# eblerjana/pangenie

Hardware: AMD Instinct MI355X
Metric: genotyped variants/sec (whole node) at H haplotypes; HBM GB/s vs roofline (higher is better)
Workload: dtype f64

## Files before the change

### include/pangenie_hmm.h

```cpp
#ifndef PANGENIE_HMM_H
#define PANGENIE_HMM_H

#include <stddef.h>
#include <stdint.h>

#ifdef __cplusplus
extern "C" {
#endif

#define PG_OK 0
#define PG_ERR_INVALID (-1)
#define PG_ERR_NO_PATHS (-2)
#define PG_ERR_UNSUPPORTED (-3)
#define PG_ERR_DEVICE (-4)
#define PG_ERR_NOMEM (-5)

typedef struct pg_contig_batch {
    uint32_t n_variants;
    uint32_t n_paths;
    const uint64_t* variant_pos;
    const uint16_t* coverage;
    const uint32_t* kmer_off;
    const uint16_t* kmer_count;
    const uint32_t* allele_off;
    const uint16_t* allele_id;
    const uint8_t*  allele_flags;
    const uint16_t* allele_kmer_off;
    const uint32_t* allele_kmer_mask;
    const uint16_t* path_allele;
} pg_contig_batch;

typedef struct pg_hmm_params {
    long double effective_N;
    double recombrate;
    int32_t uniform;
    int32_t run_genotyping;
    int32_t run_phasing;
    int32_t reserved;
} pg_hmm_params;
#define PG_CALL_ANNOUNCED 1

typedef struct pg_contig_result {
    double*   lik;
    int32_t*  lik_exp;
    uint8_t*  kept;
    uint8_t*  allele_present;
    uint16_t* n_kmers;
    uint16_t* coverage;
    uint32_t  n_columns;
    uint32_t  reserved;
    uint16_t* haplotype_1;
    uint16_t* haplotype_2;
} pg_contig_result;

int pg_hmm_geno_offsets(const pg_contig_batch* batch, uint64_t* geno_off);

typedef struct pg_table pg_table;
pg_table* pg_table_create(uint16_t cov_min, uint16_t cov_max, uint16_t count_max,
                          long double regularization);
pg_table* pg_table_create_default(void);
int  pg_table_modify(pg_table* t, uint16_t coverage, uint16_t count,
                     long double p0, long double p1, long double p2);
int  pg_table_get(const pg_table* t, uint16_t coverage, uint16_t count,
                  long double out3[3]);
void pg_table_destroy(pg_table* t);

int pg_hmm_device_count(void);
const char* pg_hmm_version(void);
int pg_hmm_genotype_contig(const pg_contig_batch* batch, const pg_table* table,
                           const pg_hmm_params* params, int device,
                           pg_contig_result* out, char* err, size_t errlen);
void pg_hmm_announce(int device);
void pg_hmm_retract(int device);
int  pg_hmm_coalesce_stats(uint64_t out3[3]);

typedef struct pg_job pg_job;
pg_job* pg_job_create(int device, uint32_t n_contigs, const pg_contig_batch* batches,
                      const pg_table* table, const pg_hmm_params* params,
                      char* err, size_t errlen);
int  pg_job_run(pg_job* job, void* stream, char* err, size_t errlen);
int  pg_job_fetch(pg_job* job, uint32_t contig, pg_contig_result* out, char* err, size_t errlen);
int  pg_job_fetch_all(pg_job* job, pg_contig_result* outs, char* err, size_t errlen);
int  pg_job_device_results(pg_job* job, uint32_t contig, void** d_lik, uint64_t* n_lik,
                           void** d_lik_exp, uint64_t* n_variants);
#define PG_N_KERNEL_CLASSES 6
int  pg_job_kernel_ms(const pg_job* job, double ms[PG_N_KERNEL_CLASSES]);
const char* pg_job_kernel_name(int cls);
int  pg_job_profile_counters(pg_job* job, uint32_t contig, uint64_t out64[64]);
uint64_t pg_job_device_bytes(const pg_job* job);
int  pg_job_sweep_mode(const pg_job* job, uint32_t* chunk_cols);
uint32_t pg_job_triangle_chains(const pg_job* job);
double pg_job_index_ms(const pg_job* job);
size_t pg_job_plan(const pg_job* job, char* out, size_t len);
int pg_sparse_segment(uint32_t n_columns, uint32_t chunk_cols, uint32_t chunk, uint32_t role, uint32_t j, uint32_t out[3]);
int pg_sparse_stored_by_chain(uint32_t n_columns, uint32_t role, uint32_t column);
int pg_sparse_chunk_segment(uint32_t n_columns, uint32_t chunk_cols, uint32_t chunk, uint32_t role, uint32_t j, uint32_t out[3]);
int pg_sparse_chunk_stored_by_chain(uint32_t n_columns, uint32_t role, uint32_t column);
int pg_sparse_piece_range(uint32_t n_columns, uint32_t chunk_cols, uint32_t piece_chunks, uint32_t piece, uint32_t role, uint32_t out[2]);
int pg_prep_parts(uint32_t n_columns, uint32_t chunk_cols, uint32_t piece_chunks, uint32_t n_pieces, uint32_t early,
                  const uint32_t* col_variant, uint32_t n_variants, uint32_t out_cols[2], uint32_t out_vars[2]);
uint32_t pg_prep_part_member(uint32_t part, uint32_t lo, uint32_t hi, uint32_t n, uint32_t u);
double pg_job_viterbi_ms(const pg_job* job);
void pg_job_destroy(pg_job* job);

int  pg_job_panel_sizes(const pg_job* job, uint32_t contig, uint32_t* n_variants, uint32_t* n_paths,
                        uint64_t* sum_kmers, uint64_t* sum_alleles);
int  pg_job_fetch_panel(pg_job* job, uint32_t contig, uint32_t* kmer_off, uint16_t* kmer_count,
                        uint32_t* allele_off, uint16_t* allele_id, uint8_t* allele_flags,
                        uint16_t* allele_kmer_off, uint32_t* allele_kmer_mask, uint16_t* path_allele,
                        char* err, size_t errlen);

int  pg_job_new(int device, uint32_t n_contigs, const pg_contig_batch* batches,
                const pg_table* table, const pg_hmm_params* params,
                pg_job** out, char* err, size_t errlen);
uint32_t pg_job_n_chains(const pg_job* job);

typedef struct pg_sample_counts {
    const uint16_t* const* kmer_count;
    const uint16_t* const* coverage;
} pg_sample_counts;
int  pg_cohort_new(int device, uint32_t n_contigs, const pg_contig_batch* index,
                   uint32_t n_samples, const pg_sample_counts* samples,
                   const pg_table* table, const pg_hmm_params* params,
                   pg_job** out, char* err, size_t errlen);

int  pg_job_upload(pg_job* job, const pg_contig_batch* batches, const pg_sample_counts* samples,
                   char* err, size_t errlen);
int  pg_job_upload_run(pg_job* job, const pg_contig_batch* batches, const pg_sample_counts* samples, char* err, size_t errlen);
int  pg_job_upload_begin(pg_job* job, const pg_sample_counts* samples, char* err, size_t errlen);
int  pg_job_upload_end(pg_job* job, char* err, size_t errlen);
int  pg_job_host_seconds(const pg_job* job, double out4[4]);
int  pg_job_upload_bytes(const pg_job* job, uint64_t out2[2]);
int  pg_job_packed_results(pg_job* job, void** d_lik, void** d_lik_exp, uint64_t* n_lik_total);
void pg_hmm_release_cache(void);

typedef struct pg_comm pg_comm;
int  pg_comm_unique_id(uint8_t id128[128], char* err, size_t errlen);
int  pg_comm_init(const uint8_t id128[128], int world, int rank, int device,
                  pg_comm** out, char* err, size_t errlen);
int  pg_comm_init_all(int n_devices, const int* devices, pg_comm** out_comms, char* err, size_t errlen);
int  pg_comm_rank(const pg_comm* comm);
int  pg_comm_world(const pg_comm* comm);
void pg_comm_destroy(pg_comm* comm);
int  pg_hmm_gather(pg_comm* comm, pg_job* job, int root, const uint64_t* n_lik_per_rank,
                   void* d_lik_all, void* d_exp_all, char* err, size_t errlen);
int  pg_hmm_gather_all(int n_local, pg_comm* const* comms, pg_job* const* jobs, int root,
                       const uint64_t* n_lik_per_rank, void* d_lik_all, void* d_exp_all,
                       char* err, size_t errlen);
int  pg_hmm_gather_to_host(int n_local, pg_comm* const* comms, pg_job* const* jobs, int root,
                           const uint64_t* n_lik_per_rank, double* h_lik_all, int32_t* h_exp_all,
                           char* err, size_t errlen);

int pg_emission_table(const pg_contig_batch* batch, const pg_table* table, uint32_t v,
                      int device, long double* out_AxA, int32_t* all_zeros,
                      char* err, size_t errlen);
int pg_transition_probs(uint64_t from_pos, uint64_t to_pos, double recombrate,
                        uint32_t nr_paths, int uniform, long double effective_N,
                        int device, double out3[3], char* err, size_t errlen);

typedef struct pg_call {
    uint16_t allele_1, allele_2;
    uint16_t gq;
    uint16_t flags;
} pg_call;
#define PG_CALL_OK 0
#define PG_CALL_NONE 1
#define PG_CALL_NOT_UNIQUE 2
#define PG_CALL_DEFERRED 3
int  pg_job_calls(pg_job* job, char* err, size_t errlen);
int  pg_job_fetch_calls(pg_job* job, uint32_t chain, pg_call* out, char* err, size_t errlen);
int  pg_job_fetch_calls_all(pg_job* job, pg_call* const* outs, char* err, size_t errlen);
int  pg_job_device_calls(pg_job* job, uint32_t chain, void** d_calls, uint64_t* n);
double pg_job_calls_ms(const pg_job* job);
int  pg_calls_from_bins(int device, uint32_t n_variants, const uint32_t* allele_off, const uint16_t* allele_id,
                        const uint8_t* kept, const uint8_t* allele_present, const double* lik,
                        const int32_t* lik_exp, pg_call* out);

typedef struct pg_record_plan {
    uint32_t n_variants;
    uint32_t n_records;
    const uint32_t* rec_off;
    const uint32_t* map_off;
    const uint16_t* map;
    const uint16_t* n_alleles;
    const uint32_t* vcf_off;
    const uint16_t* vcf_index;
} pg_record_plan;
#define PG_CALL_EMPTY 0x100
int  pg_job_record_plan(pg_job* job, uint32_t index_contig, const pg_record_plan* plan, char* err, size_t errlen);
int  pg_job_record_plan_strided(pg_job* job, uint32_t contig, uint32_t n_contigs, const pg_record_plan* plan, char* err, size_t errlen);
int  pg_job_record_calls(pg_job* job, char* err, size_t errlen);
int  pg_job_fetch_record_calls(pg_job* job, uint32_t chain, pg_call* out, char* err, size_t errlen);
int  pg_job_fetch_record_calls_all(pg_job* job, pg_call* const* outs, char* err, size_t errlen);
int  pg_job_device_record_calls(pg_job* job, uint32_t chain, void** d_calls, uint64_t* n);
double pg_job_record_calls_ms(const pg_job* job);
int  pg_record_calls_from_bins(int device, uint32_t n_variants, const uint32_t* allele_off, const uint16_t* allele_id,
                               const uint8_t* kept, const uint8_t* allele_present, const double* lik,
                               const int32_t* lik_exp, const pg_record_plan* plan, pg_call* out);

#ifndef PG_GL_DEFINED
#define PG_GL_DEFINED
typedef struct pg_gl { int16_t mant; int16_t exp10; } pg_gl;
#define PG_GL_NEG_INF  (-32768)
#define PG_GL_DEFERRED (-32767)
#endif
int  pg_record_gl_offsets(const pg_record_plan* plan, uint64_t* gl_off);
int  pg_job_record_gl(pg_job* job, char* err, size_t errlen);
int  pg_job_fetch_record_gl(pg_job* job, uint32_t chain, pg_gl* out, char* err, size_t errlen);
int  pg_job_fetch_record_gl_all(pg_job* job, pg_gl* const* outs, char* err, size_t errlen);
int  pg_job_device_record_gl(pg_job* job, uint32_t chain, void** d_gl, uint64_t* n);
double pg_job_record_gl_ms(const pg_job* job);
int  pg_job_record_first(pg_job* job, uint64_t* calls_first, uint64_t* gl_first, char* err, size_t errlen);
int  pg_job_fetch_record_calls_packed(pg_job* job, pg_call* out, uint64_t n, char* err, size_t errlen);
int  pg_job_fetch_record_gl_packed(pg_job* job, pg_gl* out, uint64_t n, char* err, size_t errlen);
int  pg_record_gl_from_bins(int device, uint32_t n_variants, const uint32_t* allele_off, const uint16_t* allele_id,
                            const uint8_t* kept, const uint8_t* allele_present, const double* lik,
                            const int32_t* lik_exp, const pg_record_plan* plan, pg_gl* out);
int  pg_gl_from_values(int device, uint64_t n, const uint64_t* m, const int32_t* e, pg_gl* out);
int  pg_gl_text(pg_gl value, char* buf, size_t len);

#ifdef __cplusplus
}
#endif
#endif
```

### pangenie_amd/_lib.py

```python
from __future__ import annotations

import ctypes as C

import numpy as np
import os
from pathlib import Path

ROOT = Path(__file__).resolve().parent.parent
HIP_LIB_PATH = ROOT / "pangenie_amd" / "csrc" / "libpangenie_hmm.so"

PG_OK = 0
PG_ERR_INVALID = -1
PG_ERR_NO_PATHS = -2
PG_ERR_UNSUPPORTED = -3
PG_ERR_DEVICE = -4
PG_ERR_NOMEM = -5
PG_N_KERNEL_CLASSES = 6

u8p = C.POINTER(C.c_uint8)
u16p = C.POINTER(C.c_uint16)
u32p = C.POINTER(C.c_uint32)
u64p = C.POINTER(C.c_uint64)
i32p = C.POINTER(C.c_int32)
f64p = C.POINTER(C.c_double)
ldp = C.POINTER(C.c_longdouble)


def c_ld(x) -> C.c_longdouble:
    v = np.longdouble(x) if isinstance(x, str) else x
    return C.c_longdouble.from_buffer_copy(np.array([v], dtype=np.longdouble).tobytes())


def ld_out(n: int):
    a = np.zeros(n, dtype=np.longdouble)
    return a, a.ctypes.data_as(ldp)


class PgContigBatch(C.Structure):
    _fields_ = [
        ("n_variants", C.c_uint32),
        ("n_paths", C.c_uint32),
        ("variant_pos", u64p),
        ("coverage", u16p),
        ("kmer_off", u32p),
        ("kmer_count", u16p),
        ("allele_off", u32p),
        ("allele_id", u16p),
        ("allele_flags", u8p),
        ("allele_kmer_off", u16p),
        ("allele_kmer_mask", u32p),
        ("path_allele", u16p),
    ]


class PgHmmParams(C.Structure):
    _fields_ = [
        ("effective_N", C.c_longdouble),
        ("recombrate", C.c_double),
        ("uniform", C.c_int32),
        ("run_genotyping", C.c_int32),
        ("run_phasing", C.c_int32),
        ("reserved", C.c_int32),
    ]


class PgContigResult(C.Structure):
    _fields_ = [
        ("lik", f64p),
        ("lik_exp", i32p),
        ("kept", u8p),
        ("allele_present", u8p),
        ("n_kmers", u16p),
        ("coverage", u16p),
        ("n_columns", C.c_uint32),
        ("reserved", C.c_uint32),
        ("haplotype_1", u16p),
        ("haplotype_2", u16p),
    ]


class PgSampleCounts(C.Structure):
    _fields_ = [
        ("kmer_count", C.POINTER(u16p)),
        ("coverage", C.POINTER(u16p)),
    ]


class PgGl(C.Structure):
    _fields_ = [("mant", C.c_int16), ("exp10", C.c_int16)]


PG_CALL_ANNOUNCED = 1


class HipExtensionMissing(RuntimeError):
    pass


_hip = None


def _bind_hip(lib):
    ld = C.c_longdouble
    lib.pg_hmm_geno_offsets.argtypes = [C.POINTER(PgContigBatch), u64p]
    lib.pg_hmm_geno_offsets.restype = C.c_int
    lib.pg_table_create.argtypes = [C.c_uint16, C.c_uint16, C.c_uint16, ld]
    lib.pg_table_create.restype = C.c_void_p
    lib.pg_table_create_default.argtypes = []
    lib.pg_table_create_default.restype = C.c_void_p
    lib.pg_table_modify.argtypes = [C.c_void_p, C.c_uint16, C.c_uint16, ld, ld, ld]
    lib.pg_table_modify.restype = C.c_int
    lib.pg_table_get.argtypes = [C.c_void_p, C.c_uint16, C.c_uint16, ldp]
    lib.pg_table_get.restype = C.c_int
    lib.pg_table_destroy.argtypes = [C.c_void_p]
    lib.pg_table_destroy.restype = None
    lib.pg_hmm_device_count.argtypes = []
    lib.pg_hmm_device_count.restype = C.c_int
    lib.pg_hmm_version.argtypes = []
    lib.pg_hmm_version.restype = C.c_char_p
    lib.pg_hmm_genotype_contig.argtypes = [
        C.POINTER(PgContigBatch), C.c_void_p, C.POINTER(PgHmmParams), C.c_int,
        C.POINTER(PgContigResult), C.c_char_p, C.c_size_t]
    lib.pg_hmm_genotype_contig.restype = C.c_int
    lib.pg_job_create.argtypes = [
        C.c_int, C.c_uint32, C.POINTER(PgContigBatch), C.c_void_p,
        C.POINTER(PgHmmParams), C.c_char_p, C.c_size_t]
    lib.pg_job_create.restype = C.c_void_p
    lib.pg_job_run.argtypes = [C.c_void_p, C.c_void_p, C.c_char_p, C.c_size_t]
    lib.pg_job_run.restype = C.c_int
    lib.pg_job_fetch.argtypes = [C.c_void_p, C.c_uint32, C.POINTER(PgContigResult),
                                 C.c_char_p, C.c_size_t]
    lib.pg_job_fetch.restype = C.c_int
    lib.pg_job_device_results.argtypes = [C.c_void_p, C.c_uint32, C.POINTER(C.c_void_p),
                                          u64p, C.POINTER(C.c_void_p), u64p]
    lib.pg_job_device_results.restype = C.c_int
    lib.pg_job_index_ms.argtypes = [C.c_void_p]
    lib.pg_job_index_ms.restype = C.c_double
    lib.pg_job_plan.argtypes = [C.c_void_p, C.c_char_p, C.c_size_t]
    lib.pg_job_plan.restype = C.c_size_t
    lib.pg_sparse_segment.argtypes = [C.c_uint32, C.c_uint32, C.c_uint32, C.c_uint32, C.c_uint32, u32p]
    lib.pg_sparse_segment.restype = C.c_int
    lib.pg_sparse_stored_by_chain.argtypes = [C.c_uint32, C.c_uint32, C.c_uint32]
    lib.pg_sparse_stored_by_chain.restype = C.c_int
    lib.pg_sparse_chunk_segment.argtypes = [C.c_uint32, C.c_uint32, C.c_uint32, C.c_uint32, C.c_uint32, u32p]
    lib.pg_sparse_chunk_segment.restype = C.c_int
    lib.pg_sparse_chunk_stored_by_chain.argtypes = [C.c_uint32, C.c_uint32, C.c_uint32]
    lib.pg_sparse_chunk_stored_by_chain.restype = C.c_int
    lib.pg_sparse_piece_range.argtypes = [C.c_uint32, C.c_uint32, C.c_uint32, C.c_uint32, C.c_uint32, u32p]
    lib.pg_sparse_piece_range.restype = C.c_int
    lib.pg_prep_parts.argtypes = [C.c_uint32, C.c_uint32, C.c_uint32, C.c_uint32, C.c_uint32, u32p, C.c_uint32, u32p, u32p]
    lib.pg_prep_parts.restype = C.c_int
    lib.pg_prep_part_member.argtypes = [C.c_uint32] * 5
    lib.pg_prep_part_member.restype = C.c_uint32
    lib.pg_job_kernel_ms.argtypes = [C.c_void_p, f64p]
    lib.pg_job_kernel_ms.restype = C.c_int
    lib.pg_job_kernel_name.argtypes = [C.c_int]
    lib.pg_job_kernel_name.restype = C.c_char_p
    lib.pg_job_profile_counters.argtypes = [C.c_void_p, C.c_uint32, u64p]
    lib.pg_job_profile_counters.restype = C.c_int
    lib.pg_job_viterbi_ms.argtypes = [C.c_void_p]
    lib.pg_job_viterbi_ms.restype = C.c_double
    lib.pg_job_device_bytes.argtypes = [C.c_void_p]
    lib.pg_job_device_bytes.restype = C.c_uint64
    lib.pg_job_sweep_mode.argtypes = [C.c_void_p, C.POINTER(C.c_uint32)]
    lib.pg_job_sweep_mode.restype = C.c_int
    lib.pg_job_triangle_chains.argtypes = [C.c_void_p]
    lib.pg_job_triangle_chains.restype = C.c_uint32
    lib.pg_job_destroy.argtypes = [C.c_void_p]
    lib.pg_job_destroy.restype = None
    lib.pg_job_new.argtypes = [C.c_int, C.c_uint32, C.POINTER(PgContigBatch), C.c_void_p, C.POINTER(PgHmmParams),
                               C.POINTER(C.c_void_p), C.c_char_p, C.c_size_t]
    lib.pg_job_new.restype = C.c_int
    lib.pg_cohort_new.argtypes = [C.c_int, C.c_uint32, C.POINTER(PgContigBatch), C.c_uint32, C.POINTER(PgSampleCounts),
                                  C.c_void_p, C.POINTER(PgHmmParams), C.POINTER(C.c_void_p), C.c_char_p, C.c_size_t]
    lib.pg_cohort_new.restype = C.c_int
    lib.pg_job_n_chains.argtypes = [C.c_void_p]
    lib.pg_job_n_chains.restype = C.c_uint32
    lib.pg_job_upload.argtypes = [C.c_void_p, C.POINTER(PgContigBatch), C.POINTER(PgSampleCounts), C.c_char_p, C.c_size_t]
    lib.pg_job_upload.restype = C.c_int
    lib.pg_job_upload_run.argtypes = [C.c_void_p, C.POINTER(PgContigBatch), C.POINTER(PgSampleCounts), C.c_char_p, C.c_size_t]
    lib.pg_job_upload_run.restype = C.c_int
    lib.pg_job_upload_begin.argtypes = [C.c_void_p, C.POINTER(PgSampleCounts), C.c_char_p, C.c_size_t]
    lib.pg_job_upload_begin.restype = C.c_int
    lib.pg_job_upload_end.argtypes = [C.c_void_p, C.c_char_p, C.c_size_t]
    lib.pg_job_upload_end.restype = C.c_int
    lib.pg_job_host_seconds.argtypes = [C.c_void_p, f64p]
    lib.pg_job_host_seconds.restype = C.c_int
    lib.pg_job_upload_bytes.argtypes = [C.c_void_p, u64p]
    lib.pg_job_upload_bytes.restype = C.c_int
    lib.pg_job_packed_results.argtypes = [C.c_void_p, C.POINTER(C.c_void_p), C.POINTER(C.c_void_p), u64p]
    lib.pg_job_packed_results.restype = C.c_int
    lib.pg_hmm_release_cache.argtypes = []
    lib.pg_hmm_release_cache.restype = None
    lib.pg_comm_unique_id.argtypes = [u8p, C.c_char_p, C.c_size_t]
    lib.pg_comm_unique_id.restype = C.c_int
    lib.pg_comm_init.argtypes = [u8p, C.c_int, C.c_int, C.c_int, C.POINTER(C.c_void_p), C.c_char_p, C.c_size_t]
    lib.pg_comm_init.restype = C.c_int
    lib.pg_comm_init_all.argtypes = [C.c_int, C.POINTER(C.c_int), C.POINTER(C.c_void_p), C.c_char_p, C.c_size_t]
    lib.pg_comm_init_all.restype = C.c_int
    lib.pg_comm_rank.argtypes = [C.c_void_p]
    lib.pg_comm_rank.restype = C.c_int
    lib.pg_comm_world.argtypes = [C.c_void_p]
    lib.pg_comm_world.restype = C.c_int
    lib.pg_comm_destroy.argtypes = [C.c_void_p]
    lib.pg_comm_destroy.restype = None
    lib.pg_hmm_gather.argtypes = [C.c_void_p, C.c_void_p, C.c_int, u64p, C.c_void_p, C.c_void_p, C.c_char_p, C.c_size_t]
    lib.pg_hmm_gather.restype = C.c_int
    lib.pg_hmm_gather_all.argtypes = [C.c_int, C.POINTER(C.c_void_p), C.POINTER(C.c_void_p), C.c_int, u64p, C.c_void_p, C.c_void_p,
                                      C.c_char_p, C.c_size_t]
    lib.pg_hmm_gather_all.restype = C.c_int
    lib.pg_emission_table.argtypes = [C.POINTER(PgContigBatch), C.c_void_p, C.c_uint32, C.c_int,
                                      ldp, i32p, C.c_char_p, C.c_size_t]
    lib.pg_emission_table.restype = C.c_int
    lib.pg_transition_probs.argtypes = [C.c_uint64, C.c_uint64, C.c_double, C.c_uint32, C.c_int,
                                        ld, C.c_int, f64p, C.c_char_p, C.c_size_t]
    lib.pg_transition_probs.restype = C.c_int
    lib.pg_job_fetch_all.argtypes = [C.c_void_p, C.POINTER(PgContigResult), C.c_char_p, C.c_size_t]
    lib.pg_job_fetch_all.restype = C.c_int
    lib.pg_job_panel_sizes.argtypes = [C.c_void_p, C.c_uint32, C.POINTER(C.c_uint32), C.POINTER(C.c_uint32), u64p, u64p]
    lib.pg_job_panel_sizes.restype = C.c_int
    lib.pg_job_fetch_panel.argtypes = [C.c_void_p, C.c_uint32, u32p, u16p, u32p, u16p, u8p, u16p, u32p, u16p, C.c_char_p, C.c_size_t]
    lib.pg_job_fetch_panel.restype = C.c_int
    lib.pg_hmm_announce.argtypes = [C.c_int]
    lib.pg_hmm_announce.restype = None
    lib.pg_hmm_retract.argtypes = [C.c_int]
    lib.pg_hmm_retract.restype = None
    lib.pg_hmm_coalesce_stats.argtypes = [u64p]
    lib.pg_hmm_coalesce_stats.restype = C.c_int
    lib.pg_job_calls.argtypes = [C.c_void_p, C.c_char_p, C.c_size_t]
    lib.pg_job_calls.restype = C.c_int
    lib.pg_job_fetch_calls.argtypes = [C.c_void_p, C.c_uint32, C.c_void_p, C.c_char_p, C.c_size_t]
    lib.pg_job_fetch_calls.restype = C.c_int
    lib.pg_job_fetch_calls_all.argtypes = [C.c_void_p, C.POINTER(C.c_void_p), C.c_char_p, C.c_size_t]
    lib.pg_job_fetch_calls_all.restype = C.c_int
    lib.pg_job_device_calls.argtypes = [C.c_void_p, C.c_uint32, C.POINTER(C.c_void_p), u64p]
    lib.pg_job_device_calls.restype = C.c_int
    lib.pg_job_calls_ms.argtypes = [C.c_void_p]
    lib.pg_job_calls_ms.restype = C.c_double
    lib.pg_calls_from_bins.argtypes = [C.c_int, C.c_uint32, u32p, u16p, u8p, u8p, f64p, i32p, C.c_void_p]
    lib.pg_calls_from_bins.restype = C.c_int
    lib.pg_job_record_plan.argtypes = [C.c_void_p, C.c_uint32, C.c_void_p, C.c_char_p, C.c_size_t]
    lib.pg_job_record_plan.restype = C.c_int
    lib.pg_job_record_calls.argtypes = [C.c_void_p, C.c_char_p, C.c_size_t]
    lib.pg_job_record_calls.restype = C.c_int
    lib.pg_job_fetch_record_calls.argtypes = [C.c_void_p, C.c_uint32, C.c_void_p, C.c_char_p, C.c_size_t]
    lib.pg_job_fetch_record_calls.restype = C.c_int
    lib.pg_job_fetch_record_calls_all.argtypes = [C.c_void_p, C.POINTER(C.c_void_p), C.c_char_p, C.c_size_t]
    lib.pg_job_fetch_record_calls_all.restype = C.c_int
    lib.pg_job_device_record_calls.argtypes = [C.c_void_p, C.c_uint32, C.POINTER(C.c_void_p), u64p]
    lib.pg_job_device_record_calls.restype = C.c_int
    lib.pg_job_record_calls_ms.argtypes = [C.c_void_p]
    lib.pg_job_record_calls_ms.restype = C.c_double
    lib.pg_record_calls_from_bins.argtypes = [C.c_int, C.c_uint32, u32p, u16p, u8p, u8p, f64p, i32p, C.c_void_p, C.c_void_p]
    lib.pg_record_calls_from_bins.restype = C.c_int
    lib.pg_record_gl_offsets.argtypes = [C.c_void_p, u64p]
    lib.pg_record_gl_offsets.restype = C.c_int
    lib.pg_job_record_gl.argtypes = [C.c_void_p, C.c_char_p, C.c_size_t]
    lib.pg_job_record_gl.restype = C.c_int
    lib.pg_job_fetch_record_gl.argtypes = [C.c_void_p, C.c_uint32, C.c_void_p, C.c_char_p, C.c_size_t]
    lib.pg_job_fetch_record_gl.restype = C.c_int
    lib.pg_job_fetch_record_gl_all.argtypes = [C.c_void_p, C.POINTER(C.c_void_p), C.c_char_p, C.c_size_t]
    lib.pg_job_fetch_record_gl_all.restype = C.c_int
    lib.pg_job_device_record_gl.argtypes = [C.c_void_p, C.c_uint32, C.POINTER(C.c_void_p), u64p]
    lib.pg_job_device_record_gl.restype = C.c_int
    lib.pg_job_record_gl_ms.argtypes = [C.c_void_p]
    lib.pg_job_record_gl_ms.restype = C.c_double
    lib.pg_record_gl_from_bins.argtypes = [C.c_int, C.c_uint32, u32p, u16p, u8p, u8p, f64p, i32p, C.c_void_p, C.c_void_p]
    lib.pg_record_gl_from_bins.restype = C.c_int
    lib.pg_job_record_plan_strided.argtypes = [C.c_void_p, C.c_uint32, C.c_uint32, C.c_void_p, C.c_char_p, C.c_size_t]
    lib.pg_job_record_plan_strided.restype = C.c_int
    lib.pg_job_record_first.argtypes = [C.c_void_p, u64p, u64p, C.c_char_p, C.c_size_t]
    lib.pg_job_record_first.restype = C.c_int
    lib.pg_job_fetch_record_calls_packed.argtypes = [C.c_void_p, C.c_void_p, C.c_uint64, C.c_char_p, C.c_size_t]
    lib.pg_job_fetch_record_calls_packed.restype = C.c_int
    lib.pg_job_fetch_record_gl_packed.argtypes = [C.c_void_p, C.c_void_p, C.c_uint64, C.c_char_p, C.c_size_t]
    lib.pg_job_fetch_record_gl_packed.restype = C.c_int
    lib.pg_gl_from_values.argtypes = [C.c_int, C.c_uint64, u64p, i32p, C.c_void_p]
    lib.pg_gl_from_values.restype = C.c_int
    lib.pg_gl_text.argtypes = [PgGl, C.c_char_p, C.c_size_t]
    lib.pg_gl_text.restype = C.c_int
    return lib


HIP_ABI_SYMBOLS = [
    "pg_hmm_geno_offsets", "pg_table_create", "pg_table_create_default", "pg_table_modify",
    "pg_table_get", "pg_table_destroy", "pg_hmm_device_count", "pg_hmm_version",
    "pg_hmm_genotype_contig", "pg_job_create", "pg_job_run", "pg_job_fetch",
    "pg_job_device_results", "pg_job_profile_counters", "pg_job_kernel_ms", "pg_job_index_ms", "pg_job_plan", "pg_job_kernel_name", "pg_job_device_bytes", "pg_job_sweep_mode",
    "pg_job_destroy", "pg_emission_table", "pg_transition_probs",
    "pg_job_new", "pg_cohort_new", "pg_job_n_chains", "pg_job_upload", "pg_job_upload_run", "pg_job_upload_begin", "pg_job_upload_end", "pg_job_host_seconds", "pg_job_upload_bytes",
    "pg_job_packed_results", "pg_hmm_release_cache", "pg_job_triangle_chains", "pg_job_viterbi_ms",
    "pg_comm_unique_id", "pg_comm_init", "pg_comm_init_all", "pg_comm_rank", "pg_comm_world", "pg_comm_destroy",
    "pg_hmm_gather", "pg_hmm_gather_all", "pg_hmm_gather_to_host",
    "pg_hmm_announce", "pg_hmm_retract", "pg_hmm_coalesce_stats", "pg_job_fetch_all", "pg_job_panel_sizes", "pg_job_fetch_panel",
    "pg_job_calls", "pg_job_fetch_calls", "pg_job_fetch_calls_all", "pg_job_device_calls", "pg_job_calls_ms", "pg_calls_from_bins",
    "pg_job_record_plan", "pg_job_record_calls", "pg_job_fetch_record_calls", "pg_job_fetch_record_calls_all", "pg_job_device_record_calls",
    "pg_job_record_calls_ms", "pg_record_calls_from_bins",
    "pg_record_gl_offsets", "pg_job_record_gl", "pg_job_fetch_record_gl", "pg_job_fetch_record_gl_all", "pg_job_device_record_gl",
    "pg_job_record_gl_ms", "pg_record_gl_from_bins", "pg_gl_from_values", "pg_gl_text",
    "pg_job_record_plan_strided", "pg_job_record_first", "pg_job_fetch_record_calls_packed", "pg_job_fetch_record_gl_packed",
    "pg_sparse_segment", "pg_sparse_stored_by_chain", "pg_sparse_chunk_segment", "pg_sparse_chunk_stored_by_chain", "pg_sparse_piece_range",
    "pg_prep_parts", "pg_prep_part_member",
]


def load_hip():
    global _hip
    if _hip is None:
        path = Path(os.environ.get("PANGENIE_HMM_LIB", HIP_LIB_PATH))
        if not path.exists():
            raise HipExtensionMissing(
                f"{path} is missing: run `python -c 'import __graft_entry__ as g; g.build()'` "
                "(hipcc --offload-arch=gfx950). There is no CPU fallback.")
        _hip = _bind_hip(C.CDLL(str(path), mode=os.RTLD_GLOBAL if hasattr(os, "RTLD_GLOBAL") else 0))
    return _hip
```

### pangenie_amd/csrc/pg_device.h

```cpp
#pragma once
#include <stddef.h>
#include <stdint.h>

#define PG_AMAX 5
#define PG_ESTRIDE (PG_AMAX + 1)
#define PG_ETAB (PG_ESTRIDE * PG_ESTRIDE)
#define PG_MAX_ALLELES_PER_VARIANT 256
#define PG_MAX_PATHS 1024
#define PG_PHANTOM 255

#define PG_REC_C0 0
#define PG_REC_C1 8
#define PG_REC_C2 16
#define PG_REC_KAPPA 24
#define PG_REC_VARIANT 32
#define PG_REC_EXP 36
#define PG_REC_NLOCAL 40
#define PG_REC_FLAGS 41
#define PG_REC_LOCAL_SLOT 48
#define PG_REC_BITS1 64
#define PG_REC_E 80
#define PG_REC_ALLELES (80 + 8 * PG_ETAB)
#define PG_REC_FLAG_ALLZERO 1
#define PG_REC_FLAG_WIDE 2
#define PG_REC_WIDE_IDX 44
#define PG_REC_AUX 60

#define PG_WIDE_MAX 254
#define PG_WIDE_NONE 0xFFFFFFFFu
static inline uint64_t pg_wide_entry_bytes(uint32_t n_local) {
    const uint64_t s = (uint64_t)n_local + 1;
    return (s * s * 20 + (uint64_t)n_local * 2 + 15) & ~(uint64_t)15;
}
#define PG_WIDE_OFF_PM(S) ((size_t)(S) * (S) * 8)
#define PG_WIDE_OFF_PE(S) ((size_t)(S) * (S) * 16)
#define PG_WIDE_OFF_SLOT(S) ((size_t)(S) * (S) * 20)

#ifndef PG_SCRATCH_BUFS
#define PG_SCRATCH_BUFS 3u
#endif
#define PG_SCR_BUF(c) ((c) % PG_SCRATCH_BUFS)
#define PG_SYNC_NEXT 16u
#define PG_SYNC_DONE 17u
#define PG_SYNC_READY 32u
#define PG_SYNC_WORDS 48u

#define PG_BIAS_F 400
#define PG_BIAS_B 400

static inline uint32_t pg_pair_count(uint32_t pair_n) { return ((pair_n * (pair_n + 1) / 2) + 1u) & ~1u; }
static inline uint32_t pg_pair_bytes(uint32_t pair_n) { return pg_pair_count(pair_n) * 12u; }

static inline uint32_t pg_rec_bytes(uint32_t hp) { return (PG_REC_ALLELES + hp + 63u) & ~63u; }

#define PG_DEVERR_ALLELE_NOT_FOUND 1u
#define PG_DEVERR_TOO_MANY_ALLELES 2u
#define PG_DEVERR_TOO_MANY_LOCAL 4u
#define PG_DEVERR_SYNC_TIMEOUT 16u
#define PG_DEVERR_WIDE_FUSED 8u

struct DevTable {
    uint32_t cov_min, cov_max, count_max;
    uint32_t pad;
    double reg;
    const double* mant;
    const int32_t* expo;
    const unsigned char* packed;
};

#define PG_IXPD_BYTES 32u
#define PG_IXREC_BYTES 64u
#define PG_IXBIN_BYTES 32u
#define PG_SREC1_BYTES 64u
#define PG_SREC2_BYTES 128u
#define PG_CPREC_BYTES 192u
#define PG_COL_NONE 0xFFFFFFFFu
#define PG_IXPD_U0 0x100u
#define PG_IXPD_U1 0x200u
#define PG_IXPD_HAS0 0x400u
#define PG_IXPD_HAS1 0x800u
#define PG_SREC_FLAG_ALLZERO 1u
#define PG_SREC_FLAG_WIDE 2u
#define PG_SREC_FLAG_PRECISE 4u
struct IxBin {
    uint32_t g0, v, aux;
    uint16_t A;
    uint8_t nl, flags;
    uint16_t ls[5];
    uint8_t cnt[5];
    uint8_t pad;
};

struct DevContig {
    uint32_t V, H, HP, RB;
    uint32_t T;
    uint32_t pad0;
    double dist_scale;
    int32_t uniform;
    uint32_t debug;
    uint32_t part_slots;
    uint32_t pair_n;
    const uint64_t* pos;
    const uint16_t* cov;
    const uint32_t* kmer_off;
    const uint16_t* kmer_count;
    const uint32_t* allele_off;
    const uint16_t* allele_id;
    const uint8_t*  allele_flags;
    const uint16_t* allele_koff;
    const uint32_t* allele_kmask;
    const uint16_t* path_allele;
    const uint64_t* geno_off;
    uint8_t*  vrec;
    uint8_t*  kept;
    uint8_t*  allele_present;
    uint32_t* n_cols;
    uint32_t* col_variant;
    uint8_t*  colrec;
    double*   fwd;
    double*   part;
    double*   fscale;
    double*   bscale;
    double*   bsum;
    uint8_t*  fwd_fallback;
    double*   scratch;
    uint32_t* sync;
    uint32_t  chunk_cols;
    uint32_t  col_stride;
    uint8_t*  wide;
    const uint32_t* wide_idx;
    uint8_t*  vpair;
    double*   frec;
    uint32_t  prep_fast;
    uint32_t  n_prep_m4, n_prep_w;
    uint32_t  n_prep_b;
    const uint32_t* prep_m4;
    const uint32_t* prep_w;
    const uint32_t* prep_b;
    uint32_t  lean;
    uint32_t  tri;
    uint32_t  leanx2;
    uint32_t  widef;
    uint32_t  small;
    uint32_t  leanx;
    uint32_t  cls4;
    uint32_t  smallx;
    uint32_t  split;
    const uint32_t* col_of;
    const unsigned char* ix_pd;
    const unsigned char* ix_rec;
    const unsigned char* ix_bin;
    unsigned char* cprec;
    uint32_t* ix_err;
    const uint32_t* ix_big;
    uint32_t n_ix_big;
    uint32_t sparse;
    uint32_t sparse2;
    uint32_t ckpt_slots;
    double*  ckpt;
    uint32_t* wcols;
    uint32_t* n_wcols;
    unsigned char* aux;
    const uint32_t* aux_idx;
    uint32_t  live;
    double*   xbuf;
    uint32_t* err;
    unsigned long long* prof;
    double*   vit_tq;
    uint16_t* vit_back;
    uint32_t* vit_best;
    uint16_t* hap1;
    uint16_t* hap2;
    double*   lik;
    int32_t*  lik_exp;
};

#define PG_LEAN_SPARSE 64u
#ifdef __HIP__
#define PG_HD __attribute__((host)) __attribute__((device))
#else
#define PG_HD
#endif
PG_HD inline uint32_t pg_sparse_segments(uint32_t C, uint32_t role) {
    const uint32_t mid = C / 2u;
    if (role == 0u) return mid ? (mid - 1u) / PG_LEAN_SPARSE : 0u;
    return C ? (C - 1u - mid) / PG_LEAN_SPARSE : 0u;
}
PG_HD inline uint32_t pg_sparse_checkpoint(uint32_t C, uint32_t role, uint32_t m) {
    const uint32_t mid = C / 2u;
    return role == 0u ? mid - 1u - m * PG_LEAN_SPARSE : mid + m * PG_LEAN_SPARSE;
}
PG_HD inline bool pg_sparse_stored(uint32_t C, uint32_t role, uint32_t c) {
    const uint32_t mid = C / 2u;
    if (role == 0u) return c >= mid || (mid - 1u - c) % PG_LEAN_SPARSE == 0u || c < (mid - 1u) % PG_LEAN_SPARSE;
    return c < mid || (c - mid) % PG_LEAN_SPARSE == 0u || c > mid + pg_sparse_segments(C, 1u) * PG_LEAN_SPARSE;
}
#define PG_PIECE_CHUNKS_DEFAULT 4u
PG_HD inline bool pg_sparse_piece(uint32_t C, uint32_t role, uint32_t piece_cols, uint32_t g, uint32_t out[2]) {
    const unsigned long long mid = C / 2u, half = role == 0u ? mid : C - mid;
    const unsigned long long d0 = (unsigned long long)g * piece_cols;
    if (piece_cols == 0u || piece_cols % PG_LEAN_SPARSE != 0u || d0 >= half) return false;
    const unsigned long long d1 = half - d0 > piece_cols ? d0 + piece_cols : half;
    if (role == 0u) { out[0] = (uint32_t)(mid - d1); out[1] = (uint32_t)(mid - 1u - d0); }
    else { out[0] = (uint32_t)(mid + d0); out[1] = (uint32_t)(mid + d1 - 1u); }
    return true;
}
#define PG_PREP_EARLY_PIECES_DEFAULT 2u
PG_HD inline uint32_t pg_prep_band(uint32_t n_pieces, uint32_t E, uint32_t piece_cols) {
    const unsigned long long W = (unsigned long long)(n_pieces - E) * piece_cols;
    return W > 0xFFFFFFC0ull ? 0xFFFFFFC0u : (uint32_t)W;
}
PG_HD inline void pg_prep_middle(uint32_t C, uint32_t W, uint32_t out[2]) {
    const uint32_t mid = C / 2u;
    out[0] = mid - (mid < W ? mid : W);
    out[1] = mid + (C - mid < W ? C - mid : W);
}
PG_HD inline void pg_prep_middle_variants(const uint32_t* col_variant, uint32_t C, uint32_t V, uint32_t W, uint32_t out[2]) {
    uint32_t cr[2];
    pg_prep_middle(C, W, cr);
    out[0] = cr[0] == 0u ? 0u : col_variant[cr[0]];
    out[1] = cr[1] >= C ? V : col_variant[cr[1]];
}
PG_HD inline uint32_t pg_prep_part_item(uint32_t part, uint32_t lo, uint32_t hi, uint32_t N, uint32_t u) {
    if (part == 2u) return u < hi - lo ? lo + u : N;
    return u < lo ? u : (u < N - (hi - lo) ? u + (hi - lo) : N);
}

PG_HD inline uint32_t pg_sparse2_slots(uint32_t V) { return (V / 2u + 1u) / PG_LEAN_SPARSE + 2u; }
PG_HD inline bool pg_sparse2_segment(uint32_t C, uint32_t role, unsigned long long m, uint32_t out[3]) {
    if (C < 2u) return false;
    const unsigned long long mid = C / 2u, d = m * PG_LEAN_SPARSE;
    if (role == 0u) {
        const unsigned long long ck = mid - 1u + d;
        if (ck + 1u >= C) return false;
        out[0] = (uint32_t)ck; out[1] = (uint32_t)ck + 1u; out[2] = (uint32_t)(C - 1u - ck > PG_LEAN_SPARSE ? ck + PG_LEAN_SPARSE : C - 1u);
    } else {
        if (d >= mid) return false;
        const unsigned long long ck = mid - d;
        out[0] = (uint32_t)ck; out[1] = (uint32_t)(ck > PG_LEAN_SPARSE ? ck - PG_LEAN_SPARSE : 0u); out[2] = (uint32_t)ck - 1u;
    }
    return true;
}
PG_HD inline bool pg_sparse2_stored(uint32_t C, uint32_t role, uint32_t c) {
    const uint32_t mid = C / 2u;
    if (C < 2u) return false;
    if (role == 0u) return c >= mid && c < C && (c - (mid - 1u)) % PG_LEAN_SPARSE == 0u;
    return c < mid && (mid - c) % PG_LEAN_SPARSE == 0u;
}

struct pg_job;
extern "C" {
__attribute__((visibility("hidden"))) int pgi_job_fill_begin(struct pg_job* job, uint32_t sample, int device, uint32_t n_contigs, const uint32_t* n_variants,
                                                            const uint32_t* const* kmer_off, void* stream, uint16_t** d_kmer_count, uint16_t** d_coverage,
                                                            char* err, size_t errlen);
__attribute__((visibility("hidden"))) int pgi_job_fill_end(struct pg_job* job, uint32_t sample, uint32_t n_contigs, const uint16_t* const* coverage, void* stream,
                                                          char* err, size_t errlen);
}
```

### pangenie_amd/csrc/pg_experiments.h

```cpp
#pragma once

#ifndef PG_EXP
#define PG_EXP 0
#endif
static constexpr unsigned kExp = PG_EXP;
#ifdef PG_CHAIN_PROF
static constexpr bool kChainProf = true;
#else
static constexpr bool kChainProf = false;
#endif

#ifndef PG_LEAN_EXP
#define PG_LEAN_EXP 0
#endif
static constexpr unsigned kLeanExp = PG_LEAN_EXP;
#ifdef PG_LEAN_DPPSUM
static constexpr bool kLeanDppSum = true;
#else
static constexpr bool kLeanDppSum = false;
#endif

#ifdef PG_POST_GENERIC
static constexpr bool kPostGeneric = true;
#else
static constexpr bool kPostGeneric = false;
#endif

#ifndef PG_PERSIST_EXP
#define PG_PERSIST_EXP 0
#endif
static constexpr unsigned kPersistExp = PG_PERSIST_EXP;

#ifndef PG_LEAN_PRETOTAL
#define PG_LEAN_PRETOTAL 0
#endif
static constexpr bool kLeanPreTotal = PG_LEAN_PRETOTAL != 0;

#ifdef PG_NT_STORES
static constexpr bool kNtStores = true;
#else
static constexpr bool kNtStores = false;
#endif
#ifdef PG_NT_POST
static constexpr bool kNtPost = true;
#else
static constexpr bool kNtPost = false;
#endif

#ifndef PG_LX_EXP
#define PG_LX_EXP 0
#endif
static constexpr unsigned kLxExp = PG_LX_EXP;

#ifndef PG_LEANP_EXP
#define PG_LEANP_EXP 0
#endif
static constexpr unsigned kLeanpExp = PG_LEANP_EXP;

#ifdef PG_LEAN_TIMELINE
static constexpr bool kLeanTimeline = true;
#else
static constexpr bool kLeanTimeline = false;
#endif
struct LeanTimeline {
    unsigned long long t[10], acc[10];
    DEVI void init() { if constexpr (kLeanTimeline) { for (int i = 0; i < 10; ++i) { t[i] = 0; acc[i] = 0; } } }
    template <int I>
    DEVI void mark(double dep) {
        if constexpr (kLeanTimeline) {
            __builtin_amdgcn_sched_barrier(0);
            asm volatile("" :: "v"(dep));
            t[I] = __builtin_amdgcn_s_memtime();
            __builtin_amdgcn_sched_barrier(0);
        }
    }
    template <int N>
    DEVI void fold() {
        if constexpr (kLeanTimeline) {
#pragma unroll
            for (int i = 0; i < N; ++i) acc[i] += t[i + 1] - t[i];
            acc[9] += 1;
        }
    }
    DEVI void write(unsigned long long* o) const {
        if constexpr (kLeanTimeline) { for (int i = 0; i < 9; ++i) o[i] = acc[i]; o[15] = acc[9]; }
    }
};

#ifndef PG_X_EXP
#define PG_X_EXP 0
#endif
static constexpr unsigned kXExp = PG_X_EXP;

#ifdef PG_VIT_TIMELINE
static constexpr bool kVitTimeline = true;
#else
static constexpr bool kVitTimeline = false;
#endif
#ifndef PG_VIT_EXP
#define PG_VIT_EXP 0
#endif
static constexpr unsigned kVitExp = PG_VIT_EXP;
struct VitTimeline {
    unsigned long long t[13], acc[13];
    DEVI void init() { if constexpr (kVitTimeline) { for (int i = 0; i < 13; ++i) { t[i] = 0; acc[i] = 0; } } }
    template <int I>
    DEVI void mark(double dep) {
        if constexpr (kVitTimeline) {
            __builtin_amdgcn_sched_barrier(0);
            asm volatile("" :: "v"(dep));
            t[I] = __builtin_amdgcn_s_memtime();
            __builtin_amdgcn_sched_barrier(0);
        }
    }
    template <int I>
    DEVI void mark_u(unsigned dep) {
        if constexpr (kVitTimeline) {
            __builtin_amdgcn_sched_barrier(0);
            asm volatile("" :: "v"(dep));
            t[I] = __builtin_amdgcn_s_memtime();
            __builtin_amdgcn_sched_barrier(0);
        }
    }
    template <int N>
    DEVI void fold() {
        if constexpr (kVitTimeline) {
#pragma unroll
            for (int i = 0; i < N; ++i) acc[i] += t[i + 1] - t[i];
            acc[12] += 1;
        }
    }
    DEVI void write(unsigned long long* o) const {
        if constexpr (kVitTimeline) { for (int i = 0; i < 12; ++i) o[i] = acc[i]; o[15] = acc[12]; }
    }
};
```

### pangenie_amd/csrc/pg_kernels.hip

```cpp
#include <hip/hip_runtime.h>
#include <math.h>
#include <stdint.h>
#include <stdlib.h>

#include <type_traits>

#include "pg_device.h"
#include "pg_devmath.h"
#include "pg_launch.h"

#define DEVI __device__ __forceinline__
typedef double v2f64 __attribute__((ext_vector_type(2)));
#include "pg_experiments.h"

template <int CTRL, int ROW_MASK, bool BOUND>
DEVI double dpp_f64(double v) {
    int lo = __double2loint(v), hi = __double2hiint(v);
    lo = __builtin_amdgcn_update_dpp(0, lo, CTRL, ROW_MASK, 0xF, BOUND);
    hi = __builtin_amdgcn_update_dpp(0, hi, CTRL, ROW_MASK, 0xF, BOUND);
    return __hiloint2double(hi, lo);
}

DEVI double readlane_f64(double v, int src_lane ) {
    int lo = __builtin_amdgcn_readlane(__double2loint(v), src_lane);
// ... 2132 lines not shown
    constexpr int KP = (PHASE == 2 && !RING) ? R - Cfg::PARK : R;
    v2f64* const park = (v2f64*)ring + p.tid;
    auto y_get = [&](int k, v2f64& q) __attribute__((always_inline)) -> double {
        if (k < KP) return y[k < KP ? k : 0];
        if (!(k & 1)) q = park[(size_t)((k - KP) >> 1) * Cfg::T];
        return (k & 1) ? q.y : q.x;
    };
    auto y_put = [&](int k, v2f64& q, double val) __attribute__((always_inline)) {
        if (k < KP) y[k < KP ? k : 0] = val;
        else if (k & 1) { q.y = val; park[(size_t)((k - KP) >> 1) * Cfg::T] = q; }
        else q.x = val;
    };
    double Sy = 0.0;
    unsigned long long tq = 0;
    if (!Cfg::LOADER && p.wave == 0) {
        rec_stage(t0 + 1, rec_load(t0 + 1));
        rec_stage(t0, rec_load(t0));
        rec_stage(t0 - 1, rec_load(t0 - 1));
        tq = rec_load(t0 - 2);
    }
    if constexpr (PHASE == 1) {
        const double B0 = ldexp(1.0, PG_BIAS_B);
#pragma unroll
        for (int k = 0; k < R; ++k) y[k] = (p.j < H && p.i0 + k < H) ? B0 : 0.0;
        Sy = (double)H * (double)H * B0;
        store_col(top, y);
        if (p.tid == 0) { bscale[top] = 1.0; bsum[top] = Sy; }
    } else {
        if (tri) load_col_tri(resume, y);
        else load_col(top + 1, y);
        Sy = bsum[top + 1];
        if constexpr (PHASE == 2 && !RING) {
            load_col(top, vA);
            if constexpr (VBUF == 2) load_col(top - 1, vB);
        }
    }
    if constexpr (KP < R) {
#pragma unroll
        for (int k = KP; k < R; k += 2) park[(size_t)((k - KP) >> 1) * Cfg::T] = v2f64{y[k], y[k + 1]};
    }
    lds_barrier();
    RecInfo cur = decode_record<Cfg::UNI>(sh.rec[(uint32_t)(t0 + 1) & 7u], p.j, p.i0, full, dc.wide);
    const bool prof = kChainProf && (dc.debug & 8u) != 0;
    const unsigned long long t_begin = prof ? __builtin_amdgcn_s_memtime() : 0;

    auto step = [&](int64_t t, double (&v)[NV]) {
        if (__builtin_expect(!(Sy > 0.0) || !(Sy < INFINITY), 0)) {
            v2f64 uq = v2f64{0.0, 0.0};
#pragma unroll
            for (int k = 0; k < R; ++k) y_put(k, uq, (p.j < H && p.i0 + k < H) ? unif : 0.0);
            Sy = 1.0;
        }
        double vt[RING ? R : 1];
        if constexpr (RING) ring_get(t, vt);
        const RecInfo nxt = decode_record<Cfg::UNI>(sh.rec[(uint32_t)t & 7u], p.j, p.i0, full, dc.wide);
        const unsigned char* rec1 = sh.rec[(uint32_t)(t + 1) & 7u];
        int es = exponent_of(Sy) - PG_BIAS_B;
        es = es < -900 ? -900 : es;
        const double m = ldexp(Sy, -es - PG_BIAS_B);
        if (p.tid == 0) bscale[t] = m;
        const double k0 = ldexp(cur.c0, -es), k1 = ldexp(cur.c1, -es), k2 = ldexp(cur.c2, -es);
        const double kap = ldexp(cur.kappa, -es);
        const bool fast = cur.fast;
        FastE fe = cur.fe;
        if (Cfg::UNI) fe.rowbits = __builtin_amdgcn_readfirstlane(fe.rowbits);
        const double feA = fe.eA, feB = fe.eB;
        double w[KEEPW ? R : 1];
        double part = 0.0;
        v2f64 yq = v2f64{0.0, 0.0};
        if (fast) {
#pragma unroll
            for (int k = 0; k < R; ++k) {
                const double yk = y_get(k, yq);
                const double wk = (kExp & 16u) ? yk : yk * (((fe.rowbits >> k) & 1u) ? +feB : +feA);
                if constexpr (KEEPW) w[k] = wk;
                part += (kExp & 16u) ? (k == 0 ? wk : 0.0) : wk;
            }
        } else if (cur.em.wide) {
#pragma unroll
            for (int k = 0; k < R; ++k) {
                const double wk = y_get(k, yq) * emission_wide(rec1, p.i0 + k, cur.em);
                if constexpr (KEEPW) w[k] = wk;
                part += wk;
                if constexpr (R > 16) { if ((k & 7) == 7) __builtin_amdgcn_sched_barrier(0); }
            }
        } else {
#pragma unroll
            for (int k = 0; k < R; ++k) {
                const double wk = y_get(k, yq) * emission_narrow(rec1, p.i0 + k, cur.em);
                if constexpr (KEEPW) w[k] = wk;
                part += wk;
                if constexpr (R > 16) { if ((k & 7) == 7) __builtin_amdgcn_sched_barrier(0); }
            }
        }
        const uint32_t pb = (uint32_t)t & 1u;
        write_colsums<HP, R>(sh, pb, p, part);
        if (!Cfg::LOADER && p.wave == 0) {
            rec_stage(t - 2, tq);
            tq = rec_load(t - 3);
        }
        lds_barrier();
        double Cj, Crow, Call;
        read_colsums<HP, R>(sh, pb, p, Cj, Crow, Call);
        const double urow = k1 * Crow, ucol = k1 * Cj;
        double ui[R > 16 ? 1 : R];
        if constexpr (R <= 16) { publish_u<HP, R>(sh, p, urow, ucol); fetch_u<HP, R>(sh, p, urow, ui); }
        constexpr bool UDPP = R > 16 && PHASE != 2;
        double urep[2] = {0.0, 0.0};
        if constexpr (UDPP) u_rows_setup<HP, R>(sh, pb, p, k1, urep);
        __builtin_amdgcn_sched_barrier(0);
        const double Sw = total_sum<HP>(Call);
        const double uj = fma(k2, Sw, ucol);
        auto beta_loop = [&](auto kind_c) {
            constexpr int KIND = decltype(kind_c)::value;
#pragma unroll
            for (int k = 0; k < R; ++k) {
                double wk;
                if constexpr (KEEPW) wk = w[k];
                else {
                    const double yk = y_get(k, yq);
                    if constexpr (KIND == 1) wk = yk * (((fe.rowbits >> k) & 1u) ? +feB : +feA);
                    else if constexpr (KIND == 2) wk = yk * emission_wide(rec1, p.i0 + k, cur.em);
                    else wk = yk * emission_narrow(rec1, p.i0 + k, cur.em);
                }
                double uik;
                if constexpr (R <= 16) uik = ui[k];
                else if constexpr (UDPP) uik = u_of_row(urep, k);
                else uik = readlane_f64(urow, __builtin_amdgcn_readfirstlane((int)((p.i0 + k) & 63u)));
                const double yn = (kExp & 16u) ? (k == 0 ? wk + uik + uj : wk) : fma(k0, wk, uik + uj);
                y_put(k, yq, yn);
                if constexpr (PHASE == 2 && !RING) v[k] *= yn;
                if constexpr (STORE) { if (k & 1) { store_pair(t, k, y[k - 1], y[k]); __builtin_amdgcn_sched_barrier(0); } }
                else if constexpr (R > 16) { if ((k & 7) == 7) __builtin_amdgcn_sched_barrier(0); }
            }
        };
        if (KEEPW || fast) beta_loop(std::integral_constant<int, 1>{});
        else if (cur.em.wide) beta_loop(std::integral_constant<int, 2>{});
        else beta_loop(std::integral_constant<int, 0>{});
        Sy = kap * Sw;
        if constexpr (STORE) {
            if (p.tid == 0) bsum[t] = Sy;
        } else {
            if constexpr (RING) {
#pragma unroll
                for (int k = 0; k < R; ++k) vt[k] *= y[k];
                posterior<HP, R>(sh, part_out, part_slots, nxt, (uint32_t)t, p, vt);
            } else {
                posterior<HP, R>(sh, part_out, part_slots, nxt, (uint32_t)t, p, v);
                load_col(t - VBUF, v);
            }
        }
        cur = nxt;
    };

    if constexpr (R <= 16) {
        static_assert(PHASE != 2 || RING, "loader configurations read partner columns from the LDS ring");
        double w[R];
        auto rowbits_of = [&](const RecInfo& ri) -> uint32_t {
            return Cfg::UNI ? (uint32_t)__builtin_amdgcn_readfirstlane(ri.fe.rowbits) : ri.fe.rowbits;
        };
        {
            if (!(Sy > 0.0)) {
#pragma unroll
                for (int k = 0; k < R; ++k) y[k] = (p.j < H && p.i0 + k < H) ? unif : 0.0;
                Sy = 1.0;
            }
            const unsigned char* rec1 = sh.rec[(uint32_t)(t0 + 1) & 7u];
            const uint32_t rb1 = rowbits_of(cur);
            double part = 0.0;
            if (cur.fast) {
#pragma unroll
                for (int k = 0; k < R; ++k) { w[k] = y[k] * (((rb1 >> k) & 1u) ? cur.fe.eB : cur.fe.eA); part += w[k]; }
            } else {
#pragma unroll
                for (int k = 0; k < R; ++k) { w[k] = y[k] * emission_at(rec1, p.i0 + k, cur.em); part += w[k]; }
            }
            write_colsums<HP, R>(sh, (uint32_t)t0 & 1u, p, part);
        }
        for (int64_t t = t0; t >= bot; --t) {
            int es = exponent_of(Sy) - PG_BIAS_B;
            es = es < -900 ? -900 : es;
            const double m = ldexp(Sy, -es - PG_BIAS_B);
            if (Cfg::NW == 1 || p.tid == 0) bscale[t] = m;
            const double k0 = ldexp(cur.c0, -es), k1 = ldexp(cur.c1, -es), k2 = ldexp(cur.c2, -es);
            const double kap = ldexp(cur.kappa, -es);
            double vt[RING ? R : 1];
            if constexpr (RING) ring_get(t, vt);
            const RecInfo nxt = decode_record<Cfg::UNI>(sh.rec[(uint32_t)t & 7u], p.j, p.i0, full, dc.wide);
            const unsigned char* rec0 = sh.rec[(uint32_t)t & 7u];
            const uint32_t rb0 = rowbits_of(nxt);
            if (!Cfg::LOADER && p.wave == 0) {
                rec_stage(t - 2, tq);
                tq = rec_load(t - 3);
            }
            lds_barrier();
            double Cj, Crow, Call;
            read_colsums<HP, R>(sh, (uint32_t)t & 1u, p, Cj, Crow, Call);
            const double urow = k1 * Crow, ucol = k1 * Cj;
            publish_u<HP, R>(sh, p, urow, ucol);
            double ui[R];
            fetch_u<HP, R>(sh, p, urow, ui);
            __builtin_amdgcn_sched_barrier(0);
            const double Sw = total_sum<HP>(Call);
            const double uj = fma(k2, Sw, ucol);
            const double Snew = kap * Sw;
            double part = 0.0;
            if (__builtin_expect(!(Snew > 0.0), 0)) {
#pragma unroll
                for (int k = 0; k < R; ++k) {
                    y[k] = 0.0;
                    const double bu = (p.j < H && p.i0 + k < H) ? unif : 0.0;
                    w[k] = bu * (nxt.fast ? (((rb0 >> k) & 1u) ? nxt.fe.eB : nxt.fe.eA) : emission_at(rec0, p.i0 + k, nxt.em));
                    part += w[k];
                }
                if constexpr (STORE) store_col(t, y);
            } else if (nxt.fast) {
#pragma unroll
                for (int k = 0; k < R; ++k) {
                    y[k] = (kExp & 16u) ? w[k] : fma(k0, w[k], ui[k] + uj);
                    if constexpr (STORE) { if (k & 1) { store_pair(t, k, y[k - 1], y[k]); __builtin_amdgcn_sched_barrier(0); } }
                    w[k] = (kExp & 16u) ? y[k] : y[k] * (((rb0 >> k) & 1u) ? nxt.fe.eB : nxt.fe.eA);
                    part += (kExp & 16u) ? (k == 0 ? w[0] + ui[k] + uj : 0.0) : w[k];
                }
            } else {
#pragma unroll
                for (int k = 0; k < R; ++k) {
                    y[k] = fma(k0, w[k], ui[k] + uj);
                    if constexpr (STORE) { if (k & 1) { store_pair(t, k, y[k - 1], y[k]); __builtin_amdgcn_sched_barrier(0); } }
                    w[k] = y[k] * emission_at(rec0, p.i0 + k, nxt.em);
                    part += w[k];
                }
            }
            write_colsums<HP, R>(sh, (uint32_t)(t - 1) & 1u, p, part);
            if constexpr (STORE) { if (Cfg::NW == 1 || p.tid == 0) bsum[t] = Snew; }
            else if (widef_col(rec0, nxt)) store_aux(rec0, y);
            else {
#pragma unroll
                for (int k = 0; k < R; ++k) vt[k] *= y[k];
                posterior<HP, R>(sh, part_out, part_slots, nxt, (uint32_t)t, p, vt);
            }
            Sy = Snew > 0.0 ? Snew : 1.0;
            cur = nxt;
        }
    } else
    for (int64_t t = t0; t >= bot; t -= 2) {
        if constexpr (PHASE == 2 && VBUF == 2 && !RING) {
            step(t, vA);
            if (t - 1 >= bot) step(t - 1, vB);
        } else {
            step(t, vA);
            if (t - 1 >= bot) step(t - 1, vA);
        }
    }
    if (prof && p.tid == 0) {
        unsigned long long* o = dc.prof + (PHASE == 1 ? 16 : 24);
        o[0] = __builtin_amdgcn_s_memtime() - t_begin; o[1] = 0; o[2] = (unsigned long long)(t0 - bot + 1);
    }
    if constexpr (PHASE == 2) lds_barrier();
}

template <int HP, int R, int VBUF, bool KEEPW, int PHASE>
#ifndef PG_HP32_WAVES
#define PG_HP32_WAVES 4
#endif
#ifndef PG_HP32_WAVES_P2
#define PG_HP32_WAVES_P2 3
#endif
__global__ __launch_bounds__((ChainCfg<HP, R, sweep_has_loader<HP, PHASE>()>::TT), (HP == 32 ? (PHASE == 2 ? PG_HP32_WAVES_P2 : PG_HP32_WAVES) : 1)) void k_sweep(const DevContig* __restrict__ contigs, uint32_t chunk) {
    __shared__ ChainShared<HP, R> sh;
    extern __shared__ __attribute__((aligned(16))) unsigned char dyn_ring[];
    const DevContig& dc = contigs[blockIdx.x];
    if (dc.HP != (uint32_t)HP) return;
    if (dc.split) return;
    if (PHASE != 2 && (dc.lean || dc.small || dc.smallx || dc.leanx)) return;
    if (PHASE == 2 && dc.leanx2) return;
    const uint32_t C = (uint32_t)__builtin_amdgcn_readfirstlane((int)*dc.n_cols);
    if (C == 0) return;
    if (PHASE == 2 && dc.tri == 2u && C >= 2) return;
    if (PHASE == 2 && (dc.small == 2u || dc.smallx == 2u) && C >= 2) return;
    if constexpr (PHASE == 2 && HP == 64 && ChainCfg<HP, R>::LOADER) {
        if (threadIdx.x == 0) *(v2f64*)(dyn_ring + (uint32_t)kTriSlots * kTriSlotB) = v2f64{0.0, 0.0};
    }
    if (PHASE == 1 && HP == 64 && dc.tri) return;
    if (blockIdx.y == 0) forward_body<HP, R, PHASE>(dc, sh, C, dyn_ring, chunk);
    else backward_body<HP, R, VBUF, KEEPW, PHASE>(dc, sh, C, dyn_ring, chunk);
}
__global__ __launch_bounds__((ChainCfg<64, 16, sweep_has_loader<64, 1>()>::TT), 1) void k_sweep_tri1(const DevContig* __restrict__ contigs) {
    __shared__ ChainShared<64, 16> sh;
    const DevContig& dc = contigs[blockIdx.x];
    if (dc.HP != 64u || dc.split || dc.lean || dc.leanx || !dc.tri) return;
    const uint32_t C = (uint32_t)__builtin_amdgcn_readfirstlane((int)*dc.n_cols);
    if (C == 0) return;
    if (blockIdx.y == 0) forward_body<64, 16, 1, true>(dc, sh, C, nullptr, 0);
    else backward_body<64, 16, 1, true, 1, true>(dc, sh, C, nullptr, 0);
}

#define PG_LEAN_BLOCK 64
template <int R>
struct LeanShared {
    static constexpr int NW = 64 / R;
    double psum[2][NW][64];
    double ptot[2][NW] __attribute__((aligned(32)));
    double u[NW][64] __attribute__((aligned(16)));
    double rec[2][PG_LEAN_BLOCK][8] __attribute__((aligned(16)));
    double scal[2][64];
    v2f64 tab[2][PG_LEAN_BLOCK][4][2];
    unsigned char comb[2][PG_LEAN_BLOCK][NW][R / 2] __attribute__((aligned(8)));
};
struct FRec {
    double c0, c1, c2, kappa, E00, E01, E11;
    unsigned long long bits1;
};
typedef double v4f64 __attribute__((ext_vector_type(4)));
struct LeanRecs {
    const GAS char* base;
    int64_t origin, C;
    int dir;
    uint32_t tid;
    DEVI v2f64 fetch(uint32_t block) const {
        int64_t c = origin + (int64_t)dir * ((int64_t)block * PG_LEAN_BLOCK + ((tid & 255u) >> 2));
        c = c < 0 ? 0 : (c >= C ? C - 1 : c);
        return *(const GAS v2f64*)(base + (size_t)c * 64u + (tid & 3u) * 16u);
    }
    template <class SH>
    DEVI void park(SH& sh, uint32_t block, v2f64 piece) const {
        if (tid < 256u) ((v2f64*)&sh.rec[block & 1u][0][0])[tid] = piece;
    }
};
template <class SH>
DEVI FRec read_frec(const SH& sh, uint32_t rel ) {
    const double* q = sh.rec[(rel / PG_LEAN_BLOCK) & 1u][rel % PG_LEAN_BLOCK];
    FRec r;
    r.c0 = q[0]; r.c1 = q[1]; r.c2 = q[2]; r.kappa = q[3]; r.E00 = q[4]; r.E01 = q[5]; r.E11 = q[6];
    r.bits1 = (unsigned long long)__double_as_longlong(q[7]);
    return r;
}

DEVI double wave_total_mfma(double v) {
    const v4f64 z = {0.0, 0.0, 0.0, 0.0};
    const v4f64 a = __builtin_amdgcn_mfma_f64_16x16x4f64(v, 1.0, z, 0, 0, 0);
    const double u = (a[0] + a[1]) + (a[2] + a[3]);
    const v4f64 b = __builtin_amdgcn_mfma_f64_16x16x4f64(u, 1.0, z, 0, 0, 0);
    return b[0];
}
DEVI double sel_by_bit(uint32_t bits , int k, double if0, double if1) {
    const uint32_t m = (uint32_t)(((int32_t)(bits << (31 - k))) >> 31);
    const uint32_t lo = ((uint32_t)__double2loint(if1) & m) | ((uint32_t)__double2loint(if0) & ~m);
    const uint32_t hi = ((uint32_t)__double2hiint(if1) & m) | ((uint32_t)__double2hiint(if0) & ~m);
    return __hiloint2double((int)hi, (int)lo);
}

struct ColScalars {
    double* row;
    unsigned long long valid = 0ull;
    DEVI void put(uint32_t , uint64_t t , double v ) {
        row[t & 63u] = v;
        valid |= 1ull << (t & 63u);
    }
    DEVI void flush(gdouble* arr, uint32_t lane, uint64_t t_any ) {
        if ((valid >> lane) & 1ull) arr[(t_any & ~(uint64_t)63u) + lane] = row[lane];
        valid = 0ull;
    }
};

template <int R>
DEVI void lean_u_rows(double urep, double (&ui)[R]) {
    static_assert(R == 16, "one DPP row of 16 lanes = the wave's 16 rows");
    ui[0] = row_bcast_f64<0>(urep);   ui[1] = row_bcast_f64<1>(urep);   ui[2] = row_bcast_f64<2>(urep);   ui[3] = row_bcast_f64<3>(urep);
    ui[4] = row_bcast_f64<4>(urep);   ui[5] = row_bcast_f64<5>(urep);   ui[6] = row_bcast_f64<6>(urep);   ui[7] = row_bcast_f64<7>(urep);
    ui[8] = row_bcast_f64<8>(urep);   ui[9] = row_bcast_f64<9>(urep);   ui[10] = row_bcast_f64<10>(urep); ui[11] = row_bcast_f64<11>(urep);
    ui[12] = row_bcast_f64<12>(urep); ui[13] = row_bcast_f64<13>(urep); ui[14] = row_bcast_f64<14>(urep); ui[15] = row_bcast_f64<15>(urep);
}
template <int K>
DEVI double fmac_row_bcast(double acc, double u, double s) {
    asm("v_fmac_f64_dpp %0, %1, %2 row_newbcast:%3 row_mask:0xf bank_mask:0xf" : "+v"(acc) : "v"(u), "v"(s), "n"(K));
    return acc;
}
DEVI void pin_here(double& v) { asm volatile("" : "+v"(v)); }
DEVI void lean_fence() { __builtin_amdgcn_sched_barrier(0); }
DEVI double dpp_source(double v) {
    double r;
    asm("v_mov_b64 %0, %1\n\ts_nop 1" : "=v"(r) : "v"(v));
    return r;
}
template <int K>
DEVI unsigned long long row_mask64(unsigned long long bits ) {
    unsigned long long m;
    asm("s_bfe_i64 %0, %1, %2" : "=s"(m) : "s"(bits), "n"((1 << 16) | K) : "scc");
    return m;
}
DEVI double sel_by_mask(double if0, double if1, unsigned long long m ) {
    uint32_t lo, hi;
    asm("v_cndmask_b32_e64 %0, %1, %2, %3" : "=v"(lo) : "v"(__double2loint(if0)), "v"(__double2loint(if1)), "s"(m));
    asm("v_cndmask_b32_e64 %0, %1, %2, %3" : "=v"(hi) : "v"(__double2hiint(if0)), "v"(__double2hiint(if1)), "s"(m));
    return __hiloint2double((int)hi, (int)lo);
}
template <int K, int N, class F>
DEVI void static_for(F&& f) {
    if constexpr (K < N) { f(std::integral_constant<int, K>{}); static_for<K + 1, N>(f); }
}
template <int SEL>
DEVI uint32_t add_byte(uint32_t bytes, uint32_t base) {
    uint32_t r;
    if constexpr (SEL == 0) asm("v_add_u32_sdwa %0, %1, %2 dst_sel:DWORD dst_unused:UNUSED_PAD src0_sel:BYTE_0 src1_sel:DWORD" : "=v"(r) : "v"(bytes), "v"(base));
    else if constexpr (SEL == 1) asm("v_add_u32_sdwa %0, %1, %2 dst_sel:DWORD dst_unused:UNUSED_PAD src0_sel:BYTE_1 src1_sel:DWORD" : "=v"(r) : "v"(bytes), "v"(base));
    else if constexpr (SEL == 2) asm("v_add_u32_sdwa %0, %1, %2 dst_sel:DWORD dst_unused:UNUSED_PAD src0_sel:BYTE_2 src1_sel:DWORD" : "=v"(r) : "v"(bytes), "v"(base));
    else asm("v_add_u32_sdwa %0, %1, %2 dst_sel:DWORD dst_unused:UNUSED_PAD src0_sel:BYTE_3 src1_sel:DWORD" : "=v"(r) : "v"(bytes), "v"(base));
    return r;
}
template <class SH>
DEVI void lean_expand(SH& sh, uint32_t block , uint32_t tid) {
    static_assert(sizeof(sh.comb[0][0]) == 32, "four waves of eight row pairs");
    if (tid >= 256u) return;
    const uint32_t b = block & 1u;
    {
        const uint32_t r = tid >> 2, c = tid & 3u;
        const double* rc = sh.rec[b][r];
        const double E00 = rc[4], E01 = rc[5], E11 = rc[6];
        sh.tab[b][r][c][0] = v2f64{(c & 1u) ? E01 : E00, (c & 2u) ? E01 : E00};
        sh.tab[b][r][c][1] = v2f64{(c & 1u) ? E11 : E01, (c & 2u) ? E11 : E01};
    }
    {
        const uint32_t r = tid >> 2, w = tid & 3u;
        const unsigned long long bits = (unsigned long long)__double_as_longlong(sh.rec[b][r][7]);
        const uint32_t b16 = (uint32_t)(bits >> (16u * w)) & 0xFFFFu;
        auto spread = [](uint32_t v8) { return ((v8 & 3u) | (((v8 >> 2) & 3u) << 8) | (((v8 >> 4) & 3u) << 16) | (((v8 >> 6) & 3u) << 24)) << 5; };
        typedef uint32_t u32x2 __attribute__((ext_vector_type(2)));
        *(u32x2*)&sh.comb[b][r][w][0] = u32x2{spread(b16 & 0xFFu), spread(b16 >> 8)};
    }
}
struct LeanPairs { uint32_t tbase, cd0, cd1; };
typedef uint32_t u32x2 __attribute__((ext_vector_type(2)));
template <class SH>
DEVI u32x2 lean_pair_bytes(const SH& sh, uint32_t rel , uint32_t wave ) {
    return *(const u32x2*)&sh.comb[(rel / PG_LEAN_BLOCK) & 1u][rel % PG_LEAN_BLOCK][wave][0];
}
template <class SH>
DEVI LeanPairs lean_pairs(const SH& sh, uint32_t rel , u32x2 cd, uint32_t aj ) {
    return LeanPairs{(uint32_t)(uintptr_t)(LAS const unsigned char*)&sh.tab[(rel / PG_LEAN_BLOCK) & 1u][rel % PG_LEAN_BLOCK][0][0] + aj * 16u, cd.x, cd.y};
}
template <class SH>
DEVI LeanPairs lean_pairs(const SH& sh, uint32_t rel, uint32_t wave, uint32_t aj) { return lean_pairs(sh, rel, lean_pair_bytes(sh, rel, wave), aj); }
template <int P>
DEVI v2f64 lean_pair(const LeanPairs& lp) {
    return *(LAS const v2f64*)(uintptr_t)add_byte<(P & 3)>(P < 4 ? lp.cd0 : lp.cd1, lp.tbase);
}
template <int R>
DEVI void lean_pairs_all(const LeanPairs& lp, double (&e)[R]) {
    static_for<0, R / 2>([&](auto pc) __attribute__((always_inline)) { constexpr int q = decltype(pc)::value; const v2f64 t = lean_pair<q>(lp); e[2 * q] = t.x; e[2 * q + 1] = t.y; });
}
template <int R>
DEVI double lean_colsum(const LeanShared<R>& sh, uint32_t pb, uint32_t lane) {
    if constexpr (R == 16)
        return (sh.psum[pb][0][lane] + sh.psum[pb][1][lane]) + (sh.psum[pb][2][lane] + sh.psum[pb][3][lane]);
    else
        return ((sh.psum[pb][0][lane] + sh.psum[pb][1][lane]) + (sh.psum[pb][2][lane] + sh.psum[pb][3][lane])) +
               ((sh.psum[pb][4][lane] + sh.psum[pb][5][lane]) + (sh.psum[pb][6][lane] + sh.psum[pb][7][lane]));
}



#define PG_SYNC_TIMEOUT_TICKS 1000000000ull
#ifndef PG_POLL_SLEEPS
#define PG_POLL_SLEEPS 2
#endif
DEVI bool chunk_spin(uint32_t* flag, uint32_t want, uint32_t* err) {
    bool ok = __hip_atomic_load(flag, __ATOMIC_RELAXED, __HIP_MEMORY_SCOPE_AGENT) >= want;
    if (!ok) {
        const unsigned long long t0 = wall_clock64();
        for (uint32_t it = 0;; ++it) {
#pragma unroll
            for (int z = 0; z < PG_POLL_SLEEPS; ++z) __builtin_amdgcn_s_sleep(127);
            if (__hip_atomic_load(flag, __ATOMIC_RELAXED, __HIP_MEMORY_SCOPE_AGENT) >= want) { ok = true; break; }
            if ((it & 63u) == 63u) {
                if (__hip_atomic_load(err, __ATOMIC_RELAXED, __HIP_MEMORY_SCOPE_AGENT) & PG_DEVERR_SYNC_TIMEOUT) break;
                if (wall_clock64() - t0 > PG_SYNC_TIMEOUT_TICKS) { atomicOr(err, PG_DEVERR_SYNC_TIMEOUT); break; }
            }
        }
    }
    if (ok) __builtin_amdgcn_fence(__ATOMIC_ACQUIRE, "agent");
    return ok;
}
DEVI void chunk_publish(uint32_t* flag, uint32_t value) {
    __builtin_amdgcn_fence(__ATOMIC_RELEASE, "agent");
    __syncthreads();
    if (threadIdx.x == 0) __hip_atomic_store(flag, value, __ATOMIC_RELEASE, __HIP_MEMORY_SCOPE_AGENT);
}
DEVI void chunk_wait_buffer(uint32_t* flag, uint32_t want, uint32_t* err) {
    if (threadIdx.x == 0 && !(kPersistExp & 2u)) (void)chunk_spin(flag, want, err);
    __syncthreads();
}

DEVI void lean_store(gdouble2* p, v2f64 v) {
    if constexpr (kNtStores) __builtin_nontemporal_store(v, p);
    else *p = v;
}
template <int R>
DEVI void lean_put_sums(LeanShared<R>& sh, uint32_t pb, uint32_t wave, uint32_t lane, double part) {
    sh.psum[pb][wave][lane] = part;
    if constexpr (kLeanPreTotal) {
        double v = part;
        v += dpp_f64<0x111, 0xF, true>(v);
        v += dpp_f64<0x112, 0xF, true>(v);
        v += dpp_f64<0x114, 0xF, true>(v);
        v += dpp_f64<0x118, 0xF, true>(v);
        v += dpp_f64<0x142, 0xA, false>(v);
        v += dpp_f64<0x143, 0xC, false>(v);
        if (lane == 63u) sh.ptot[pb][wave] = v;
    }
}
template <int R>
DEVI double lean_total(const LeanShared<R>& sh, uint32_t pb) {
    static_assert(R == 16, "four waves");
    const v2f64 a = *(const v2f64*)&sh.ptot[pb][0], b = *(const v2f64*)&sh.ptot[pb][2];
    return (a.x + a.y) + (b.x + b.y);
}

template <int PHASE, int R, bool TRI, bool SPARSE = false>
DEVI void lean_forward(const DevContig& dc, LeanShared<R>& sh, uint32_t C, uint32_t chunk) {
    static_assert(!SPARSE || ((PHASE == 1 || PHASE == 3) && !TRI), "sparse stores: phases 1 and 3 of full-column lean chains");
    constexpr int HP = 64;
    constexpr uint32_t RMASK = (1u << R) - 1u;
    const uint32_t mid = C / 2, K = dc.chunk_cols;
    uint32_t lo = PHASE == 1 ? 0u : mid, hi = PHASE == 1 ? mid : C;
    if constexpr (PHASE == 3) {
        const unsigned long long l = (unsigned long long)mid + (unsigned long long)chunk * K;
        if (l >= C) return;
        lo = (uint32_t)l;
        hi = C - lo > K ? lo + K : C;
    }
    if constexpr (SPARSE && PHASE == 1) if (chunk) {
        uint32_t pc[2];
        if (!pg_sparse_piece(C, 0u, (chunk >> 16) * K, chunk & 0xFFFFu, pc)) return;
        lo = pc[0]; hi = pc[1] + 1u;
    }
    bool seg2 = false;
    if constexpr (PHASE == 5) {
        lo = chunk + 1u; hi = chunk + PG_LEAN_SPARSE;
        seg2 = lo >= mid;
        if (seg2) hi = C - lo > PG_LEAN_SPARSE ? lo + PG_LEAN_SPARSE : C;
    }
    if (lo >= hi) return;
    const uint32_t first = lo == 0 ? 1u : lo;
    const uint32_t tid = threadIdx.x, lane = tid & 63u;
    const uint32_t wave = __builtin_amdgcn_readfirstlane(tid >> 6);
    const uint32_t i0 = wave * R;
    const size_t colsz = TRI ? (size_t)dc.col_stride : (size_t)HP * HP;
    const double unif = 1.0 / 4096.0;
    LeanRecs recs{(const GAS char*)dc.frec, (int64_t)first - 1, (int64_t)C, +1, tid};
    recs.park(sh, 0, recs.fetch(0));
    v2f64 piece = recs.fetch(1);
    lds_barrier();
    lean_expand(sh, 0, tid);
    lds_barrier();
    gdouble* fwd = (gdouble*)dc.fwd;
    gdouble* fscale = (gdouble*)dc.fscale;
    gu8* fallback = (gu8*)dc.fwd_fallback;
    gdouble* wr = fwd;
    gcdouble* resume = (gcdouble*)(fwd + (size_t)(lo > 0 ? lo - 1 : 0) * colsz);
    if constexpr (PHASE == 3) {
        gdouble* scr = (gdouble*)dc.scratch;
        wr = scr + (size_t)(PG_SCR_BUF(chunk) * 2u) * K * colsz - (size_t)lo * colsz;
        if constexpr (SPARSE) { if (chunk > 0) resume = (gcdouble*)dc.ckpt + (size_t)(lo - mid) / PG_LEAN_SPARSE * colsz; }
        else if (chunk > 0) resume = (gcdouble*)(scr + ((size_t)(PG_SCR_BUF(chunk - 1u) * 2u) * K + (K - 1u)) * colsz);
    }
    if constexpr (PHASE == 4) wr = (gdouble*)dc.scratch - (size_t)lo * colsz;
    bool boundary = false;
    if constexpr (PHASE == 5) if (seg2) {
        const uint32_t m = (lo - mid) / PG_LEAN_SPARSE, ci = (lo - mid) / K;
        if (m) resume = (gcdouble*)dc.ckpt + (size_t)m * colsz;
        wr = (gdouble*)dc.scratch + (size_t)(PG_SCR_BUF(ci) * 2u) * K * colsz - ((size_t)mid + (size_t)ci * K) * colsz;
        boundary = (lo - mid) % K == 0u;
    }
    const size_t toff = (size_t)(i0 >> 1) * HP + lane;
    auto emis = [&](const FRec& r, double& eA, double& eB) {
        const bool aj = (r.bits1 >> lane) & 1ull;
        eA = aj ? r.E01 : r.E00;
        eB = aj ? r.E11 : r.E01;
    };
    double tfa[TRI ? R / 2 : 1], tfb[TRI ? R / 2 : 1];
    uint32_t tskip = 0, tunit[TRI ? R / 2 : 1];
    uint32_t rskip = 0;
    if constexpr (PHASE == 5) {
#pragma unroll
        for (int q = 0; q < R / 2; ++q) rskip |= (lane < ((i0 + 2u * (uint32_t)q) & ~7u) ? 1u : 0u) << q;
    }
    if constexpr (TRI) {
#pragma unroll
        for (int q = 0; q < R / 2; ++q) {
            const uint32_t r0 = i0 + 2u * (uint32_t)q;
            tfa[q] = lane < r0 ? 0.0 : (lane == r0 ? 0.5 : 1.0);
            tfb[q] = lane <= r0 ? 0.0 : (lane == r0 + 1u ? 0.5 : 1.0);
            const bool off_q = lane < (r0 & ~7u);
            tskip |= (off_q ? 1u : 0u) << q;
            tunit[q] = off_q ? 0u : tri_unit_of(r0 >> 1, lane);
        }
    }
    auto put_pair = [&](gdouble2* dst, int q, double a, double b) __attribute__((always_inline)) {
        if constexpr (TRI) {
            if (!((tskip >> q) & 1u)) lean_store((dst - toff) + tunit[q], v2f64{a * tfa[q], b * tfb[q]});
        } else if constexpr (PHASE == 5) {
            if (!((rskip >> q) & 1u)) lean_store(dst + (size_t)q * HP, v2f64{a, b});
        } else {
            lean_store(dst + (size_t)q * HP, v2f64{a, b});
        }
    };
    auto col_at = [&](uint32_t c) __attribute__((always_inline)) -> gdouble* {
        if constexpr (SPARSE && PHASE == 3) return (gdouble*)dc.ckpt + (size_t)((c - (mid - 1u)) / PG_LEAN_SPARSE) * colsz;
        else return wr + (size_t)c * colsz;
    };
    auto store_col = [&](uint32_t c, const double (&v)[R]) {
        gdouble2* dst = (gdouble2*)col_at(c) + toff;
#pragma unroll
        for (int k = 0; k < R; k += 2) put_pair(dst, k >> 1, v[k], v[k + 1]);
    };
    auto flag_uniform = [&](uint32_t cprev) {
        bool stored = cprev >= lo;
        if constexpr (SPARSE && PHASE == 1) stored = pg_sparse_stored(C, 0u, cprev);
        if constexpr (SPARSE && PHASE == 3) stored = stored && pg_sparse2_stored(C, 0u, cprev);
        if (stored) {
            double xu[R];
#pragma unroll
            for (int k = 0; k < R; ++k) xu[k] = unif;
            store_col(cprev, xu);
        }
        if constexpr (PHASE != 5) if (wave == 0) fallback[cprev] = 1;
    };

    uint32_t noscal = ~0u;
    if constexpr (PHASE == 5) if (seg2 && pg_sparse2_stored(C, 0u, hi - 1u)) noscal = hi - 1u;
    ColScalars fsc{&sh.scal[0][0]};
    double x[R];
    {
        const FRec r0 = read_frec(sh, 0);
        double eA, eB;
        emis(r0, eA, eB);
        const uint32_t rb = (uint32_t)__builtin_amdgcn_readfirstlane((int)((uint32_t)(r0.bits1 >> i0) & RMASK));
        double part = 0.0;
        if (lo == 0) {
            const double P0 = ldexp(1.0, PG_BIAS_F);
            double pz[R];
#pragma unroll
            for (int k = 0; k < R; ++k) { pz[k] = P0; x[k] = sel_by_bit(rb, k, eA, eB) * P0; part += x[k]; }
            store_col(0, pz);
            if (wave == 0) fscale[0] = 1.0;
        } else {
            gcdouble2* src = (gcdouble2*)resume + toff;
#pragma unroll
            for (int k = 0; k < R; k += 2) { const v2f64 t = src[(size_t)(k >> 1) * HP]; x[k] = t.x; x[k + 1] = t.y; }
            if (!fallback[lo - 1]) {
#pragma unroll
                for (int k = 0; k < R; ++k) { const double e = sel_by_bit(rb, k, eA, eB); part = fma(e, x[k], part); x[k] *= e; }
            } else if ((PHASE == 5 && !boundary) || (SPARSE && PHASE == 1)) {
#pragma unroll
                for (int k = 0; k < R; ++k) x[k] = 0.0;
            } else {
#pragma unroll
                for (int k = 0; k < R; ++k) part += x[k];
            }
        }
        lean_put_sums<R>(sh, (first - 1) & 1u, wave, lane, part);
    }
    double ec[R];
    {
        const FRec r1 = read_frec(sh, 1);
        lean_pairs_all<R>(lean_pairs(sh, 1, wave, (uint32_t)((r1.bits1 >> lane) & 1ull)), ec);
    }
    LeanTimeline tl;
    tl.init();
    auto step = [&](auto store_c, uint32_t t, const FRec& cur, FRec& nxt) __attribute__((always_inline)) {
        constexpr bool STORE = decltype(store_c)::value;
        const uint32_t n = t - first;
        tl.template mark<0>(0.0);
        nxt = read_frec(sh, n + 2u);
        const u32x2 cdn = lean_pair_bytes(sh, n + 2u, wave);
        if (((n + 4u) % PG_LEAN_BLOCK) == 0u) {
            const uint32_t blk = (n + 4u) / PG_LEAN_BLOCK;
            recs.park(sh, blk, piece);
            piece = recs.fetch(blk + 1u);
        } else if (((n + 3u) % PG_LEAN_BLOCK) == 0u) {
            lean_expand(sh, (n + 3u) / PG_LEAN_BLOCK, tid);
        }
        const uint32_t pb = (t - 1) & 1u;
        double pc[64 / R], pr[64 / R];
#pragma unroll
        for (int q = 0; q < 64 / R; ++q) { pc[q] = sh.psum[pb][q][lane]; pr[q] = sh.psum[pb][q][i0 + (lane & 15u)]; }
        const double Spre = kLeanPreTotal ? lean_total<R>(sh, pb) : 0.0;
        const double Cj = (pc[0] + pc[1]) + (pc[2] + pc[3]);
        tl.template mark<1>(Cj);
        const v4f64 zz = {0.0, 0.0, 0.0, 0.0};
        const v4f64 ma = (kLeanDppSum || kLeanPreTotal) ? zz : __builtin_amdgcn_mfma_f64_16x16x4f64(Cj, 1.0, zz, 0, 0, 0);
        lean_fence();
        const double ucol = cur.c1 * Cj;
        const double urep = dpp_source(cur.c1 * ((pr[0] + pr[1]) + (pr[2] + pr[3])));
        const LeanPairs lp = lean_pairs(sh, n + 2u, cdn, (uint32_t)((nxt.bits1 >> lane) & 1ull));
        const double msum = (ma[0] + ma[1]) + (ma[2] + ma[3]);
        tl.template mark<2>(msum);
        lean_fence();
        const v4f64 mb = (kLeanDppSum || kLeanPreTotal) ? zz : __builtin_amdgcn_mfma_f64_16x16x4f64(msum, 1.0, zz, 0, 0, 0);
        if constexpr (!kLeanPreTotal) asm volatile("" :: "v"(mb));
        lean_fence();
        double S = (kLeanExp & 4) ? 64.0 * Cj : (kLeanPreTotal ? Spre : (kLeanDppSum ? wave_sum(Cj) : mb[0]));
        tl.template mark<3>(S);
        double uj = fma(cur.c2, S, ucol);
        double c0 = cur.c0;
        if (__builtin_expect(!(S > 0.0), 0)) {
            flag_uniform(t - 1);
            const double Cu = 64.0 * unif;
            S = 1.0;
            uj = fma(cur.c0, unif, fma(cur.c2, 1.0, 2.0 * cur.c1 * Cu));
            c0 = 0.0;
        }
        int es = exponent_of(S) - PG_BIAS_F;
        es = es < -900 ? -900 : es;
        const double m = ldexp(S, -es - PG_BIAS_F);
        const double sc = ldexp(1.0, -es), c0s = ldexp(c0, -es), ujs = ldexp(uj, -es);
        tl.template mark<4>(c0s + ujs + sc);
        gdouble2* dst = (gdouble2*)col_at(t) + toff;
        double part = 0.0, pprev = 0.0;
        static_for<0, R>([&](auto kc) __attribute__((always_inline)) {
            constexpr int k = decltype(kc)::value;
            const double pk = fmac_row_bcast<k>(fma(c0s, x[k], ujs), urep, sc);
            part = fma(ec[k], pk, part);
            x[k] = ec[k] * pk;
            pin_here(x[k]);
            if constexpr (k == 1) tl.template mark<5>(x[1]);
            if constexpr (k & 1) {
                if constexpr (STORE) { if (!(kLeanExp & 1)) put_pair(dst, k >> 1, pprev, pk); }
                const v2f64 t2 = (kLeanExp & 2) ? v2f64{0.5, 0.5} : lean_pair<(k >> 1)>(lp);
                ec[k - 1] = t2.x; ec[k] = t2.y;
                __builtin_amdgcn_sched_barrier(0);
            } else pprev = pk;
        });
        tl.template mark<6>(part);
        lean_put_sums<R>(sh, t & 1u, wave, lane, part);
        if constexpr (SPARSE) {
            if constexpr (STORE) if (wave == 0) fscale[t] = m;
        } else if (wave == 0) {
            if (PHASE != 5 || t != noscal) fsc.put(lane, t, m);
            if ((t & 63u) == 63u) fsc.flush(fscale, lane, t);
        }
        tl.template mark<7>(0.0);
        lds_barrier();
        tl.template mark<8>(0.0);
        tl.template fold<8>();
    };
    FRec ra = read_frec(sh, 1), rb2;
    constexpr std::true_type kStore{};
    constexpr std::false_type kNoStore{};
    __builtin_amdgcn_s_waitcnt(0x0F70);
    lds_barrier();
    uint32_t t = first;
    if constexpr (PHASE == 4) {
        const uint32_t post_groups = 2u * (uint32_t)K;
        gdouble* scr = (gdouble*)dc.scratch;
        uint32_t q = 0, cend = hi - lo > K ? lo + K : hi;
        for (;;) {
            for (; t + 1 < cend; t += 2) {
                step(kStore, t, ra, rb2);
                step(kStore, t + 1, rb2, ra);
            }
            if (t < cend) { step(kStore, t, ra, rb2); ++t; }
            if (wave == 0 && fsc.valid) fsc.flush(fscale, lane, cend - 1);
            {
                const double Cj = lean_colsum<R>(sh, (cend - 1) & 1u, lane);
                if (!(wave_total_mfma(Cj) > 0.0)) flag_uniform(cend - 1);
            }
            chunk_publish(dc.sync + 0, q + 1u);
            if (cend >= hi) break;
            ++q;
            lo = cend;
            cend = hi - lo > K ? lo + K : hi;
            wr = scr + (size_t)(PG_SCR_BUF(q) * 2u) * K * colsz - (size_t)lo * colsz;
            if (q >= PG_SCRATCH_BUFS) chunk_wait_buffer(dc.sync + PG_SYNC_DONE + PG_SCR_BUF(q), (q / PG_SCRATCH_BUFS) * post_groups, dc.err);
        }
        return;
    }
    if constexpr (SPARSE) {
        if constexpr (PHASE == 1) {
            const uint32_t ck0 = (hi - 1u) % PG_LEAN_SPARSE;
            for (; t + 1 <= ck0; t += 2) {
                step(kStore, t, ra, rb2);
                step(kStore, t + 1, rb2, ra);
            }
            if (t <= ck0) { step(kStore, t, ra, rb2); ra = rb2; ++t; }
        }
        while (hi - t >= PG_LEAN_SPARSE) {
            for (uint32_t g = 0; g + 1u < PG_LEAN_SPARSE / 2u; ++g, t += 2) {
                step(kNoStore, t, ra, rb2);
                step(kNoStore, t + 1, rb2, ra);
            }
            step(kNoStore, t, ra, rb2);
            step(kStore, t + 1, rb2, ra);
            t += 2;
        }
        if constexpr (PHASE == 3) {
            for (; t + 1 < hi; t += 2) {
                step(kNoStore, t, ra, rb2);
                step(kNoStore, t + 1, rb2, ra);
            }
            if (t < hi) step(kNoStore, t, ra, rb2);
        }
    } else {
        for (; t + 1 < hi; t += 2) {
            step(kStore, t, ra, rb2);
            step(kStore, t + 1, rb2, ra);
        }
        if (t < hi) step(kStore, t, ra, rb2);
    }
    if constexpr (!SPARSE) if (wave == 0 && fsc.valid) fsc.flush(fscale, lane, hi - 1);
    if (kLeanTimeline && tid == 0) tl.write(dc.prof + 32);
    {
        const uint32_t pb = (hi - 1) & 1u;
        const double Cj = lean_colsum<R>(sh, pb, lane);
        if (!(wave_total_mfma(Cj) > 0.0)) flag_uniform(hi - 1);
    }
}

template <int PHASE, int R, bool TRI, bool SPARSE = false>
DEVI void lean_backward(const DevContig& dc, LeanShared<R>& sh, uint32_t C, uint32_t chunk) {
    static_assert(!SPARSE || ((PHASE == 1 || PHASE == 3) && !TRI), "sparse stores: phases 1 and 3 of full-column lean chains");
    constexpr int HP = 64;
    constexpr uint32_t RMASK = (1u << R) - 1u;
    const int64_t mid = C / 2, K = dc.chunk_cols;
    int64_t top = PHASE == 1 ? (int64_t)C - 1 : mid - 1;
    int64_t bot = PHASE == 1 ? mid : 0;
    if constexpr (PHASE == 3) {
        top = mid - 1 - (int64_t)chunk * K;
        if (top < 0) return;
        bot = top - K + 1 > 0 ? top - K + 1 : 0;
    }
    bool seg2 = false;
    if constexpr (PHASE == 5) {
        top = (int64_t)chunk - 1; bot = (int64_t)chunk - (int64_t)(PG_LEAN_SPARSE - 1u);
        seg2 = (int64_t)chunk <= mid;
        if (seg2) bot = top + 1 > (int64_t)PG_LEAN_SPARSE ? top + 1 - (int64_t)PG_LEAN_SPARSE : 0;
    }
    bool resumed = PHASE != 1;
    if constexpr (SPARSE && PHASE == 1) if (chunk) {
        uint32_t pc[2];
        if (!pg_sparse_piece(C, 1u, (chunk >> 16) * dc.chunk_cols, chunk & 0xFFFFu, pc)) return;
        bot = pc[0]; top = pc[1];
        resumed = top != (int64_t)C - 1;
    }
    if (top < bot) return;
    const int64_t t0 = resumed ? top : top - 1;
    const uint32_t tid = threadIdx.x, lane = tid & 63u;
    const uint32_t wave = __builtin_amdgcn_readfirstlane(tid >> 6);
    const uint32_t i0 = wave * R;
    const size_t colsz = TRI ? (size_t)dc.col_stride : (size_t)HP * HP;
    const double unif = 1.0 / 4096.0;
    LeanRecs recs{(const GAS char*)dc.frec, t0 + 1, (int64_t)C, -1, tid};
    recs.park(sh, 0, recs.fetch(0));
    v2f64 piece = recs.fetch(1);
    lds_barrier();
    lean_expand(sh, 0, tid);
    lds_barrier();
    gdouble* cols = (gdouble*)dc.fwd;
    gdouble* bscale = (gdouble*)dc.bscale;
    gdouble* bsum = (gdouble*)dc.bsum;
    gdouble* wr = cols;
    gcdouble* resume = (gcdouble*)(cols + (size_t)(top + 1 < (int64_t)C ? top + 1 : top) * colsz);
    if constexpr (PHASE == 3) {
        gdouble* scr = (gdouble*)dc.scratch;
        wr = scr + (size_t)(PG_SCR_BUF(chunk) * 2u + 1u) * (size_t)K * colsz - (size_t)bot * colsz;
        if constexpr (SPARSE) { if (chunk > 0) resume = (gcdouble*)dc.ckpt + ((size_t)dc.ckpt_slots + (size_t)(mid - 1 - top) / PG_LEAN_SPARSE) * colsz; }
        else if (chunk > 0) resume = (gcdouble*)(scr + (size_t)(PG_SCR_BUF(chunk - 1u) * 2u + 1u) * (size_t)K * colsz);
    }
    if constexpr (PHASE == 5) if (seg2) {
        const size_t m = (size_t)(mid - 1 - top) / PG_LEAN_SPARSE;
        const int64_t ci = (mid - 1 - top) / K, ctop = mid - 1 - ci * K;
        if (m) resume = (gcdouble*)dc.ckpt + ((size_t)dc.ckpt_slots + m) * colsz;
        wr = (gdouble*)dc.scratch + (size_t)(PG_SCR_BUF((uint32_t)ci) * 2u + 1u) * (size_t)K * colsz - (size_t)(ctop - K + 1 > 0 ? ctop - K + 1 : 0) * colsz;
    }
    int64_t cbot = bot;
    if constexpr (PHASE == 4) {
        cbot = top - K + 1 > 0 ? top - K + 1 : 0;
        wr = (gdouble*)dc.scratch + (size_t)K * colsz - (size_t)cbot * colsz;
    }
    const size_t toff = (size_t)(i0 >> 1) * HP + lane;
    auto emis = [&](const FRec& r, double& eA, double& eB) {
        const bool aj = (r.bits1 >> lane) & 1ull;
        eA = aj ? r.E01 : r.E00;
        eB = aj ? r.E11 : r.E01;
    };
    double tfa[TRI ? R / 2 : 1], tfb[TRI ? R / 2 : 1];
    uint32_t tskip = 0, tunit[TRI ? R / 2 : 1];
    uint32_t rskip = 0;
    if constexpr (PHASE == 5) {
#pragma unroll
        for (int q = 0; q < R / 2; ++q) rskip |= (lane < ((i0 + 2u * (uint32_t)q) & ~7u) ? 1u : 0u) << q;
    }
    if constexpr (TRI) {
#pragma unroll
        for (int q = 0; q < R / 2; ++q) {
            const uint32_t r0 = i0 + 2u * (uint32_t)q;
            tfa[q] = lane < r0 ? 0.0 : (lane == r0 ? 0.5 : 1.0);
            tfb[q] = lane <= r0 ? 0.0 : (lane == r0 + 1u ? 0.5 : 1.0);
            const bool off_q = lane < (r0 & ~7u);
            tskip |= (off_q ? 1u : 0u) << q;
            tunit[q] = off_q ? 0u : tri_unit_of(r0 >> 1, lane);
        }
    }
    auto put_pair = [&](gdouble2* dst, int q, double a, double b) __attribute__((always_inline)) {
        if constexpr (TRI) {
            if (!((tskip >> q) & 1u)) lean_store((dst - toff) + tunit[q], v2f64{a * tfa[q], b * tfb[q]});
        } else if constexpr (PHASE == 5) {
            if (!((rskip >> q) & 1u)) lean_store(dst + (size_t)q * HP, v2f64{a, b});
        } else {
            lean_store(dst + (size_t)q * HP, v2f64{a, b});
        }
    };
    auto col_at = [&](int64_t c) __attribute__((always_inline)) -> gdouble* {
        if constexpr (SPARSE && PHASE == 3) return (gdouble*)dc.ckpt + ((size_t)dc.ckpt_slots + (size_t)(mid - c) / PG_LEAN_SPARSE) * colsz;
        else return wr + (size_t)c * colsz;
    };
    auto store_col = [&](int64_t c, const double (&v)[R]) {
        gdouble2* dst = (gdouble2*)col_at(c) + toff;
#pragma unroll
        for (int k = 0; k < R; k += 2) put_pair(dst, k >> 1, v[k], v[k + 1]);
    };

    int64_t noscal = -1;
    if constexpr (PHASE == 5) if (seg2 && pg_sparse2_stored(C, 1u, (uint32_t)bot)) noscal = bot;
    ColScalars bsc{&sh.scal[0][0]}, bsm{&sh.scal[1][0]};
    double w[R], Sy;
    FRec cur = read_frec(sh, 0);
    {
        double y[R];
        if (!resumed) {
            const double B0 = ldexp(1.0, PG_BIAS_B);
#pragma unroll
            for (int k = 0; k < R; ++k) y[k] = B0;
            Sy = 4096.0 * B0;
            store_col(top, y);
            if (wave == 0) { bscale[top] = 1.0; bsum[top] = Sy; }
        } else {
            gcdouble2* src = (gcdouble2*)resume + toff;
#pragma unroll
            for (int k = 0; k < R; k += 2) { const v2f64 t = src[(size_t)(k >> 1) * HP]; y[k] = t.x; y[k + 1] = t.y; }
            Sy = bsum[top + 1];
            if (!(Sy > 0.0)) {
#pragma unroll
                for (int k = 0; k < R; ++k) y[k] = unif;
                Sy = 1.0;
            }
        }
        double eA, eB;
        emis(cur, eA, eB);
        const uint32_t rb = (uint32_t)__builtin_amdgcn_readfirstlane((int)((uint32_t)(cur.bits1 >> i0) & RMASK));
        double part = 0.0;
#pragma unroll
        for (int k = 0; k < R; ++k) { const double e = sel_by_bit(rb, k, eA, eB); part = fma(e, y[k], part); w[k] = y[k] * e; }
        lean_put_sums<R>(sh, (uint32_t)t0 & 1u, wave, lane, part);
    }
    double ec[R];
    {
        const FRec r1 = read_frec(sh, 1);
        lean_pairs_all<R>(lean_pairs(sh, 1, wave, (uint32_t)((r1.bits1 >> lane) & 1ull)), ec);
    }
    double one = 1.0;
    asm volatile("" : "+v"(one));
    LeanTimeline tl;
    tl.init();
    auto step = [&](auto store_c, int64_t t, const FRec& cur, FRec& nxt) __attribute__((always_inline)) {
        constexpr bool STORE = decltype(store_c)::value;
        const uint32_t n = (uint32_t)(t0 - t);
        tl.template mark<0>(0.0);
        if (((n + 4u) % PG_LEAN_BLOCK) == 0u) {
            const uint32_t blk = (n + 4u) / PG_LEAN_BLOCK;
            recs.park(sh, blk, piece);
            piece = recs.fetch(blk + 1u);
        } else if (((n + 3u) % PG_LEAN_BLOCK) == 0u) {
            lean_expand(sh, (n + 3u) / PG_LEAN_BLOCK, tid);
        }
        int es = exponent_of(Sy) - PG_BIAS_B;
        es = es < -900 ? -900 : es;
        const double m = ldexp(Sy, -es - PG_BIAS_B);
        if constexpr (SPARSE) {
            if constexpr (STORE) if (wave == 1) { asm volatile("" ::: "memory"); bscale[t] = m; }
        } else if (wave == 1 && (PHASE != 5 || t != noscal)) { asm volatile("" ::: "memory"); bsc.put(lane, (uint64_t)t, m); }
        double k0 = ldexp(cur.c0, -es), k1 = ldexp(cur.c1, -es), k2 = ldexp(cur.c2, -es), kap = ldexp(cur.kappa, -es);
        pin_here(k0); pin_here(k1); pin_here(k2); pin_here(kap);
        tl.template mark<1>(k0 + kap);
        lds_barrier();
        tl.template mark<2>(0.0);
        const uint32_t pb = (uint32_t)t & 1u;
        double pc[64 / R], pr[64 / R];
#pragma unroll
        for (int q = 0; q < 64 / R; ++q) { pc[q] = sh.psum[pb][q][lane]; pr[q] = sh.psum[pb][q][i0 + (lane & 15u)]; }
        const double Spre = kLeanPreTotal ? lean_total<R>(sh, pb) : 0.0;
        lean_fence();
        nxt = read_frec(sh, n + 1u);
        const unsigned long long bits_n = (unsigned long long)__double_as_longlong(sh.rec[((n + 2u) / PG_LEAN_BLOCK) & 1u][(n + 2u) % PG_LEAN_BLOCK][7]);
        const u32x2 cdn = lean_pair_bytes(sh, n + 2u, wave);
        lean_fence();
        const double Cj = (pc[0] + pc[1]) + (pc[2] + pc[3]);
        tl.template mark<3>(Cj);
        const v4f64 zz = {0.0, 0.0, 0.0, 0.0};
        const v4f64 ma = (kLeanDppSum || kLeanPreTotal) ? zz : __builtin_amdgcn_mfma_f64_16x16x4f64(Cj, 1.0, zz, 0, 0, 0);
        lean_fence();
        const double ucol = k1 * Cj;
        const double urep = dpp_source(k1 * ((pr[0] + pr[1]) + (pr[2] + pr[3])));
        const LeanPairs lp = lean_pairs(sh, n + 2u, cdn, (uint32_t)((bits_n >> lane) & 1ull));
        const double msum = (ma[0] + ma[1]) + (ma[2] + ma[3]);
        tl.template mark<4>(msum);
        lean_fence();
        const v4f64 mb = (kLeanDppSum || kLeanPreTotal) ? zz : __builtin_amdgcn_mfma_f64_16x16x4f64(msum, 1.0, zz, 0, 0, 0);
        if constexpr (!kLeanPreTotal) asm volatile("" :: "v"(mb));
        lean_fence();
        const double Sw = (kLeanExp & 4) ? 64.0 * Cj : (kLeanPreTotal ? Spre : (kLeanDppSum ? wave_sum(Cj) : mb[0]));
        tl.template mark<5>(Sw);
        const double uj = fma(k2, Sw, ucol);
        const double Snew = kap * Sw;
        Sy = Snew;
        gdouble2* dst = (gdouble2*)col_at(t) + toff;
        double part = 0.0, yprev = 0.0;
        const bool zero = !(Snew > 0.0);
        static_for<0, R>([&](auto kc) __attribute__((always_inline)) {
            constexpr int k = decltype(kc)::value;
            const double yk = fmac_row_bcast<k>(fma(k0, w[k], uj), urep, one);
            part = fma(ec[k], yk, part);
            w[k] = ec[k] * yk;
            pin_here(w[k]);
            if constexpr (k == 1) tl.template mark<6>(w[1]);
            if constexpr (k & 1) {
                if constexpr (STORE) { if (!(kLeanExp & 1)) put_pair(dst, k >> 1, yprev, yk); }
                const v2f64 t2 = (kLeanExp & 2) ? v2f64{0.5, 0.5} : lean_pair<(k >> 1)>(lp);
                ec[k - 1] = t2.x; ec[k] = t2.y;
                __builtin_amdgcn_sched_barrier(0);
            } else yprev = yk;
        });
        if (__builtin_expect(zero, 0)) {
            double et[R];
            lean_pairs_all<R>(lean_pairs(sh, n + 1u, wave, (uint32_t)((nxt.bits1 >> lane) & 1ull)), et);
            part = 0.0;
#pragma unroll
            for (int k = 0; k < R; ++k) { w[k] = unif * et[k]; part += w[k]; }
            Sy = 1.0;
        }
        tl.template mark<7>(part);
        lean_put_sums<R>(sh, (uint32_t)(t - 1) & 1u, wave, lane, part);
        if constexpr (SPARSE) {
            if constexpr (STORE) if (wave == 2) { asm volatile("" ::: "memory"); bsum[t] = Snew; }
        } else if constexpr (PHASE != 5) {
            if (wave == 2) { asm volatile("" ::: "memory"); bsm.put(lane, (uint64_t)t, Snew); }
            if (((uint64_t)t & 63u) == 0u) {
                if (wave == 1) bsc.flush(bscale, lane, (uint64_t)t);
                if (wave == 2) bsm.flush(bsum, lane, (uint64_t)t);
            }
        } else {
            if (wave == 1 && ((uint64_t)t & 63u) == 0u) bsc.flush(bscale, lane, (uint64_t)t);
        }
        tl.template mark<8>(0.0);
        tl.template fold<8>();
    };
    FRec rb2;
    constexpr std::true_type kStore{};
    constexpr std::false_type kNoStore{};
    int64_t t = t0;
    __builtin_amdgcn_s_waitcnt(0x0F70);
    if constexpr (PHASE == 4) {
        const uint32_t post_groups = 2u * (uint32_t)K;
        gdouble* scr = (gdouble*)dc.scratch;
        uint32_t q = 0;
        for (;;) {
            for (; t - 1 >= cbot; t -= 2) {
                step(kStore, t, cur, rb2);
                step(kStore, t - 1, rb2, cur);
            }
            if (t >= cbot) { step(kStore, t, cur, rb2); --t; }
            if (wave == 1 && bsc.valid) bsc.flush(bscale, lane, (uint64_t)cbot);
            if (wave == 2 && bsm.valid) bsm.flush(bsum, lane, (uint64_t)cbot);
            chunk_publish(dc.sync + 1, q + 1u);
            if (cbot == 0) break;
            ++q;
            const int64_t ntop = cbot - 1;
            cbot = ntop - K + 1 > 0 ? ntop - K + 1 : 0;
            wr = scr + (size_t)(PG_SCR_BUF(q) * 2u + 1u) * (size_t)K * colsz - (size_t)cbot * colsz;
            if (q >= PG_SCRATCH_BUFS) chunk_wait_buffer(dc.sync + PG_SYNC_DONE + PG_SCR_BUF(q), (q / PG_SCRATCH_BUFS) * post_groups, dc.err);
        }
        return;
    }
    if constexpr (SPARSE) {
        if constexpr (PHASE == 1) {
            const int64_t ckh = mid + (int64_t)pg_sparse_segments(C, 1u) * (int64_t)PG_LEAN_SPARSE;
            for (; t - 1 >= ckh; t -= 2) {
                step(kStore, t, cur, rb2);
                step(kStore, t - 1, rb2, cur);
            }
            if (t >= ckh) { step(kStore, t, cur, rb2); cur = rb2; --t; }
        }
        while (t - bot >= (int64_t)PG_LEAN_SPARSE - 1) {
            for (uint32_t g = 0; g + 1u < PG_LEAN_SPARSE / 2u; ++g, t -= 2) {
                step(kNoStore, t, cur, rb2);
                step(kNoStore, t - 1, rb2, cur);
            }
            step(kNoStore, t, cur, rb2);
            step(kStore, t - 1, rb2, cur);
            t -= 2;
        }
        if constexpr (PHASE == 3) {
            for (; t - 1 >= bot; t -= 2) {
                step(kNoStore, t, cur, rb2);
                step(kNoStore, t - 1, rb2, cur);
            }
            if (t >= bot) step(kNoStore, t, cur, rb2);
        }
    } else {
        for (; t - 1 >= bot; t -= 2) {
            step(kStore, t, cur, rb2);
            step(kStore, t - 1, rb2, cur);
        }
        if (t >= bot) step(kStore, t, cur, rb2);
    }
    if constexpr (!SPARSE) {
        if (wave == 1 && bsc.valid) bsc.flush(bscale, lane, (uint64_t)bot);
        if (PHASE != 5 && wave == 2 && bsm.valid) bsm.flush(bsum, lane, (uint64_t)bot);
    }
    if (kLeanTimeline && tid == 0) tl.write(dc.prof + 48);
}

template <int R>
struct LeanShared2 {
    LeanShared<R> a;
    v2f64 ppart[2][64 / R][64];
};
template <int R>
struct LeanTri {
    uint32_t sbase[R / 2];
    uint32_t lane16, valid;
    DEVI void setup(uint32_t i0 , uint32_t lane) {
        valid = 0;
        lane16 = lane * 16u;
#pragma unroll
        for (int q = 0; q < R / 2; ++q) {
            const uint32_t rp = (i0 >> 1) + (uint32_t)q, g = rp >> 2;
            sbase[q] = (uint32_t)__builtin_amdgcn_readfirstlane((int)((256u * g - 16u * g * (g - 1u) + (rp & 3u) * (64u - 8u * g) - 8u * g) * 16u));
            valid |= (lane >= 8u * g ? 1u : 0u) << q;
        }
    }
    DEVI void load(gcdouble* col , double (&v)[R]) const {
#pragma unroll
        for (int q = 0; q < R / 2; ++q)
            if ((valid >> q) & 1u) {
                const GAS char* cb = (const GAS char*)col + (int32_t)sbase[q];
                const v2f64 t = *(const GAS v2f64*)(cb + lane16);
                v[2 * q] = t.x; v[2 * q + 1] = t.y;
            }
    }
};
template <int R>
DEVI void lean_load_mirrored(gcdouble* col, uint32_t i0, uint32_t lane, double (&v)[R]) {
#pragma unroll
    for (int k = 0; k < R; ++k) {
        const uint32_t i = i0 + (uint32_t)k, a = i <= lane ? i : lane, b = i <= lane ? lane : i;
        const double val = col[(size_t)tri_unit_of(a >> 1, b) * 2 + (a & 1u)];
        v[k] = a == b ? 2.0 * val : val;
    }
}
template <int R>
DEVI void lean2_flush_partials(const LeanShared2<R>& sh, uint32_t pb, gdouble* part, size_t c, uint32_t wave, uint32_t lane,
                               unsigned long long bits1 ) {
    static_assert(64 / R == 4, "one class per wave");
    v2f64 t = sh.ppart[pb][0][lane];
#pragma unroll
    for (int w = 1; w < 64 / R; ++w) { const v2f64 o = sh.ppart[pb][w][lane]; t.x += o.x; t.y += o.y; }
    const bool aj = (bits1 >> lane) & 1ull;
    const double mine = (wave & 2u) ? t.y : t.x;
    const double s = wave_sum(aj == ((wave & 1u) != 0u) ? mine : 0.0);
    if (lane == 0) part[c * 4u + wave] = s;
}

template <int R>
DEVI void lean2_forward(const DevContig& dc, LeanShared2<R>& sh2, uint32_t C) {
    constexpr int HP = 64;
    constexpr uint32_t RMASK = (1u << R) - 1u;
    LeanShared<R>& sh = sh2.a;
    const uint32_t mid = C / 2, lo = mid, hi = C, first = lo;
    const uint32_t tid = threadIdx.x, lane = tid & 63u;
    const uint32_t wave = __builtin_amdgcn_readfirstlane(tid >> 6);
    const uint32_t i0 = wave * R;
    const size_t colsz = dc.col_stride;
    const double unif = 1.0 / 4096.0;
    LeanRecs recs{(const GAS char*)dc.frec, (int64_t)first - 1, (int64_t)C, +1, tid};
    recs.park(sh, 0, recs.fetch(0));
    v2f64 piece = recs.fetch(1);
    lds_barrier();
    lean_expand(sh, 0, tid);
    gcdouble* cols = (gcdouble*)dc.fwd;
    gdouble* fscale = (gdouble*)dc.fscale;
    gu8* fallback = (gu8*)dc.fwd_fallback;
    gdouble* part = (gdouble*)dc.part;
    auto emis = [&](const FRec& r, double& eA, double& eB) {
        const bool aj = (r.bits1 >> lane) & 1ull;
        eA = aj ? r.E01 : r.E00;
        eB = aj ? r.E11 : r.E01;
    };
    LeanTri<R> tri;
    tri.setup(i0, lane);
    double b0[R], b1[R], b2[R];
#pragma unroll
    for (int k = 0; k < R; ++k) { b0[k] = 0.0; b1[k] = 0.0; b2[k] = 0.0; }
    tri.load(cols + (size_t)lo * colsz, b0);
    if (lo + 1 < C) tri.load(cols + (size_t)(lo + 1) * colsz, b1);

    ColScalars fsc{&sh.scal[0][0]};
    double x[R];
    {
        const FRec r0 = read_frec(sh, 0);
        double eA, eB;
        emis(r0, eA, eB);
        const uint32_t rb = (uint32_t)__builtin_amdgcn_readfirstlane((int)((uint32_t)(r0.bits1 >> i0) & RMASK));
        lean_load_mirrored<R>(cols + (size_t)(lo - 1) * colsz, i0, lane, x);
        if (!fallback[lo - 1]) {
#pragma unroll
            for (int k = 0; k < R; ++k) x[k] *= sel_by_bit(rb, k, eA, eB);
        }
        double part0 = 0.0;
#pragma unroll
        for (int k = 0; k < R; ++k) part0 += x[k];
        sh.psum[(first - 1) & 1u][wave][lane] = part0;
    }
    unsigned long long pbits = 0;
    lds_barrier();
    unsigned long long cbits = read_frec(sh, 1).bits1;
    u32x2 ccd = lean_pair_bytes(sh, 1, wave);
    auto step = [&](uint32_t t, const double (&ba)[R], double (&bc)[R]) __attribute__((always_inline)) {
        const uint32_t n = t - first;
        const double* rq = sh.rec[((n + 1u) / PG_LEAN_BLOCK) & 1u][(n + 1u) % PG_LEAN_BLOCK];
        const double rc0 = rq[0], rc1 = rq[1], rc2 = rq[2];
        const unsigned long long nbits = (unsigned long long)__double_as_longlong(sh.rec[((n + 2u) / PG_LEAN_BLOCK) & 1u][(n + 2u) % PG_LEAN_BLOCK][7]);
        const u32x2 ncd = lean_pair_bytes(sh, n + 2u, wave);
        if (((n + 4u) % PG_LEAN_BLOCK) == 0u) {
            const uint32_t blk = (n + 4u) / PG_LEAN_BLOCK;
            recs.park(sh, blk, piece);
            piece = recs.fetch(blk + 1u);
        } else if (((n + 3u) % PG_LEAN_BLOCK) == 0u) {
            lean_expand(sh, (n + 3u) / PG_LEAN_BLOCK, tid);
        }
        if (t + 2 < C) tri.load(cols + (size_t)(t + 2) * colsz, bc);
        if (t > first) lean2_flush_partials<R>(sh2, (t - 1) & 1u, part, (size_t)(t - 1), wave, lane, pbits);
        const uint32_t pb = (t - 1) & 1u;
        const double Cj = lean_colsum<R>(sh, pb, lane);
        const double ucol = rc1 * Cj;
        const double urep = dpp_source(rc1 * lean_colsum<R>(sh, pb, i0 + (lane & 15u)));
        const LeanPairs lp = lean_pairs(sh, n + 1u, ccd, (uint32_t)((cbits >> lane) & 1ull));
        const v4f64 zz = {0.0, 0.0, 0.0, 0.0};
        const v4f64 ma = __builtin_amdgcn_mfma_f64_16x16x4f64(Cj, 1.0, zz, 0, 0, 0);
        double S = __builtin_amdgcn_mfma_f64_16x16x4f64((ma[0] + ma[1]) + (ma[2] + ma[3]), 1.0, zz, 0, 0, 0)[0];
        double uj = fma(rc2, S, ucol);
        double c0 = rc0;
        if (__builtin_expect(!(S > 0.0), 0)) {
            if (wave == 0) fallback[t - 1] = 1;
            const double Cu = 64.0 * unif;
            S = 1.0;
            uj = fma(rc0, unif, fma(rc2, 1.0, 2.0 * rc1 * Cu));
            c0 = 0.0;
        }
        int es = exponent_of(S) - PG_BIAS_F;
        es = es < -900 ? -900 : es;
        const double m = ldexp(S, -es - PG_BIAS_F);
        const double sc = ldexp(1.0, -es), c0s = ldexp(c0, -es), ujs = ldexp(uj, -es);
        double part0 = 0.0, acc0 = 0.0, acc1 = 0.0;
        const uint32_t rb = (uint32_t)__builtin_amdgcn_readfirstlane((int)((uint32_t)(cbits >> i0) & RMASK));
        v2f64 en = lean_pair<0>(lp);
        static_for<0, R / 2>([&](auto pc) __attribute__((always_inline)) {
            constexpr int q = decltype(pc)::value, k = 2 * q;
            const v2f64 e = en;
            if constexpr (q + 1 < R / 2) en = lean_pair<q + 1>(lp);
            const double pa = fmac_row_bcast<k>(fma(c0s, x[k], ujs), urep, sc);
            const double pb2 = fmac_row_bcast<k + 1>(fma(c0s, x[k + 1], ujs), urep, sc);
            x[k] = pa * e.x;
            part0 += x[k];
            x[k + 1] = pb2 * e.y;
            part0 += x[k + 1];
            const double pra = pa * ba[k], prb = pb2 * ba[k + 1];
            const bool bita = (rb >> k) & 1u, bitb = (rb >> (k + 1)) & 1u;
            acc1 = fma(pra, bita ? 1.0 : 0.0, acc1);
            acc0 = fma(pra, bita ? 0.0 : 1.0, acc0);
            acc1 = fma(prb, bitb ? 1.0 : 0.0, acc1);
            acc0 = fma(prb, bitb ? 0.0 : 1.0, acc0);
        });
        sh.psum[t & 1u][wave][lane] = part0;
        sh2.ppart[t & 1u][wave][lane] = v2f64{acc0, acc1};
        if (wave == 0) {
            fsc.put(lane, t, m);
            if ((t & 63u) == 63u) fsc.flush(fscale, lane, t);
        }
        pbits = cbits; cbits = nbits; ccd = ncd;
        lds_barrier();
    };
    {
        uint32_t t = first;
        for (; t + 2 < hi; t += 3) {
            step(t, b0, b2);
            step(t + 1, b1, b0);
            step(t + 2, b2, b1);
        }
        if (t < hi) step(t, b0, b2);
        if (t + 1 < hi) step(t + 1, b1, b0);
    }
    lean2_flush_partials<R>(sh2, (hi - 1) & 1u, part, (size_t)(hi - 1), wave, lane, pbits);
    if (wave == 0 && fsc.valid) fsc.flush(fscale, lane, hi - 1);
    {
        const double Cj = lean_colsum<R>(sh, (hi - 1) & 1u, lane);
        if (!(wave_total_mfma(Cj) > 0.0) && wave == 0) fallback[hi - 1] = 1;
    }
}

template <int R>
DEVI void lean2_backward(const DevContig& dc, LeanShared2<R>& sh2, uint32_t C) {
    constexpr int HP = 64;
    constexpr uint32_t RMASK = (1u << R) - 1u;
    LeanShared<R>& sh = sh2.a;
    const int64_t mid = C / 2, top = mid - 1, bot = 0, t0 = top;
    const uint32_t tid = threadIdx.x, lane = tid & 63u;
    const uint32_t wave = __builtin_amdgcn_readfirstlane(tid >> 6);
    const uint32_t i0 = wave * R;
    const size_t colsz = dc.col_stride;
    const double unif = 1.0 / 4096.0;
    LeanRecs recs{(const GAS char*)dc.frec, t0 + 1, (int64_t)C, -1, tid};
    recs.park(sh, 0, recs.fetch(0));
    v2f64 piece = recs.fetch(1);
    lds_barrier();
    lean_expand(sh, 0, tid);
    gcdouble* cols = (gcdouble*)dc.fwd;
    gdouble* bscale = (gdouble*)dc.bscale;
    gcdouble* bsum = (gcdouble*)dc.bsum;
    gdouble* part = (gdouble*)dc.part;
    auto emis = [&](const FRec& r, double& eA, double& eB) {
        const bool aj = (r.bits1 >> lane) & 1ull;
        eA = aj ? r.E01 : r.E00;
        eB = aj ? r.E11 : r.E01;
    };
    LeanTri<R> tri;
    tri.setup(i0, lane);
    double b0[R], b1[R], b2[R];
#pragma unroll
    for (int k = 0; k < R; ++k) { b0[k] = 0.0; b1[k] = 0.0; b2[k] = 0.0; }
    tri.load(cols + (size_t)t0 * colsz, b0);
    if (t0 - 1 >= 0) tri.load(cols + (size_t)(t0 - 1) * colsz, b1);

    ColScalars bsc{&sh.scal[0][0]};
    double w[R], Sy;
    FRec cur = read_frec(sh, 0);
    {
        double y[R];
        lean_load_mirrored<R>(cols + (size_t)(top + 1) * colsz, i0, lane, y);
        Sy = bsum[top + 1];
        if (!(Sy > 0.0)) {
#pragma unroll
            for (int k = 0; k < R; ++k) y[k] = unif;
            Sy = 1.0;
        }
        double eA, eB;
        emis(cur, eA, eB);
        const uint32_t rb = (uint32_t)__builtin_amdgcn_readfirstlane((int)((uint32_t)(cur.bits1 >> i0) & RMASK));
        double part0 = 0.0;
#pragma unroll
        for (int k = 0; k < R; ++k) { w[k] = y[k] * sel_by_bit(rb, k, eA, eB); part0 += w[k]; }
        sh.psum[(uint32_t)t0 & 1u][wave][lane] = part0;
    }
    double one = 1.0;
    asm volatile("" : "+v"(one));
    lds_barrier();
    double kc0 = cur.c0, kc1 = cur.c1, kc2 = cur.c2, kck = cur.kappa;
    unsigned long long pbits = cur.bits1;
    unsigned long long cbits = read_frec(sh, 1).bits1;
    u32x2 ccd = lean_pair_bytes(sh, 1, wave);
    auto step = [&](int64_t t, const double (&ba)[R], double (&bc)[R]) __attribute__((always_inline)) {
        const uint32_t n = (uint32_t)(t0 - t);
        if (((n + 4u) % PG_LEAN_BLOCK) == 0u) {
            const uint32_t blk = (n + 4u) / PG_LEAN_BLOCK;
            recs.park(sh, blk, piece);
            piece = recs.fetch(blk + 1u);
        } else if (((n + 3u) % PG_LEAN_BLOCK) == 0u) {
            lean_expand(sh, (n + 3u) / PG_LEAN_BLOCK, tid);
        }
        if (t - 2 >= 0) tri.load(cols + (size_t)(t - 2) * colsz, bc);
        int es = exponent_of(Sy) - PG_BIAS_B;
        es = es < -900 ? -900 : es;
        const double m = ldexp(Sy, -es - PG_BIAS_B);
        if (wave == 0) bsc.put(lane, (uint64_t)t, m);
        const double k0 = ldexp(kc0, -es), k1 = ldexp(kc1, -es), k2 = ldexp(kc2, -es), kap = ldexp(kck, -es);
        lds_barrier();
        const double* rq = sh.rec[((n + 1u) / PG_LEAN_BLOCK) & 1u][(n + 1u) % PG_LEAN_BLOCK];
        const double nc0 = rq[0], nc1 = rq[1], nc2 = rq[2], nck = rq[3];
        const unsigned long long nbits = (unsigned long long)__double_as_longlong(sh.rec[((n + 2u) / PG_LEAN_BLOCK) & 1u][(n + 2u) % PG_LEAN_BLOCK][7]);
        const u32x2 ncd = lean_pair_bytes(sh, n + 2u, wave);
        if (t < t0) lean2_flush_partials<R>(sh2, (uint32_t)(t + 1) & 1u, part, (size_t)(t + 1), wave, lane, pbits);
        const double Cj = lean_colsum<R>(sh, (uint32_t)t & 1u, lane);
        const double ucol = k1 * Cj;
        const double urep = dpp_source(k1 * lean_colsum<R>(sh, (uint32_t)t & 1u, i0 + (lane & 15u)));
        const LeanPairs lp = lean_pairs(sh, n + 1u, ccd, (uint32_t)((cbits >> lane) & 1ull));
        const v4f64 zz = {0.0, 0.0, 0.0, 0.0};
        const v4f64 ma = __builtin_amdgcn_mfma_f64_16x16x4f64(Cj, 1.0, zz, 0, 0, 0);
        const double Sw = __builtin_amdgcn_mfma_f64_16x16x4f64((ma[0] + ma[1]) + (ma[2] + ma[3]), 1.0, zz, 0, 0, 0)[0];
        const double uj = fma(k2, Sw, ucol);
        const double Snew = kap * Sw;
        double part0 = 0.0, acc0 = 0.0, acc1 = 0.0;
        if (__builtin_expect(!(Snew > 0.0), 0)) {
            double et[R];
            lean_pairs_all<R>(lp, et);
#pragma unroll
            for (int k = 0; k < R; ++k) { w[k] = unif * et[k]; part0 += w[k]; }
        } else {
            const uint32_t rb = (uint32_t)__builtin_amdgcn_readfirstlane((int)((uint32_t)(cbits >> i0) & RMASK));
            v2f64 en = lean_pair<0>(lp);
            static_for<0, R / 2>([&](auto pc) __attribute__((always_inline)) {
                constexpr int q = decltype(pc)::value, k = 2 * q;
                const v2f64 e = en;
                if constexpr (q + 1 < R / 2) en = lean_pair<q + 1>(lp);
                const double ya = fmac_row_bcast<k>(fma(k0, w[k], uj), urep, one);
                const double yb = fmac_row_bcast<k + 1>(fma(k0, w[k + 1], uj), urep, one);
                w[k] = ya * e.x;
                part0 += w[k];
                w[k + 1] = yb * e.y;
                part0 += w[k + 1];
                const double pra = ba[k] * ya, prb = ba[k + 1] * yb;
                const bool bita = (rb >> k) & 1u, bitb = (rb >> (k + 1)) & 1u;
                acc1 = fma(pra, bita ? 1.0 : 0.0, acc1);
                acc0 = fma(pra, bita ? 0.0 : 1.0, acc0);
                acc1 = fma(prb, bitb ? 1.0 : 0.0, acc1);
                acc0 = fma(prb, bitb ? 0.0 : 1.0, acc0);
            });
        }
        sh.psum[(uint32_t)(t - 1) & 1u][wave][lane] = part0;
        sh2.ppart[(uint32_t)t & 1u][wave][lane] = v2f64{acc0, acc1};
        if (wave == 0 && ((uint64_t)t & 63u) == 0u) bsc.flush(bscale, lane, (uint64_t)t);
        Sy = Snew > 0.0 ? Snew : 1.0;
        kc0 = nc0; kc1 = nc1; kc2 = nc2; kck = nck;
        pbits = cbits; cbits = nbits; ccd = ncd;
    };
    {
        int64_t t = t0;
        for (; t - 2 >= bot; t -= 3) {
            step(t, b0, b2);
            step(t - 1, b1, b0);
            step(t - 2, b2, b1);
        }
        if (t >= bot) step(t, b0, b2);
        if (t - 1 >= bot) step(t - 1, b1, b0);
    }
    lds_barrier();
    lean2_flush_partials<R>(sh2, (uint32_t)bot & 1u, part, (size_t)bot, wave, lane, pbits);
    if (wave == 0 && bsc.valid) bsc.flush(bscale, lane, (uint64_t)bot);
}

template <int R>
__global__ __launch_bounds__((64 * 64 / R)) __attribute__((amdgpu_waves_per_eu(2, 2)))
void k_sweep_lean2(const DevContig* __restrict__ contigs) {
    __shared__ LeanShared2<R> sh;
    const DevContig& dc = contigs[blockIdx.x];
    if (!dc.lean || dc.tri != 2u) return;
    const uint32_t C = (uint32_t)__builtin_amdgcn_readfirstlane((int)*dc.n_cols);
    if (C < 2) return;
    if (blockIdx.y == 0) lean2_forward<R>(dc, sh, C);
    else lean2_backward<R>(dc, sh, C);
}

template <int PHASE, int R, bool TRI>
DEVI void sweep_lean_body(const DevContig* __restrict__ contigs, uint32_t chunk, LeanShared<R>& sh);

template <int PHASE, int R>
__global__ __launch_bounds__((64 * 64 / R)) __attribute__((amdgpu_waves_per_eu(2, 2)))
void k_sweep_lean_tri(const DevContig* __restrict__ contigs, uint32_t chunk) {
    __shared__ LeanShared<R> sh;
    sweep_lean_body<PHASE, R, true>(contigs, chunk, sh);
}

template <int PHASE, int R, bool TRI = false>
__global__ __launch_bounds__((64 * 64 / R)) void k_sweep_lean(const DevContig* __restrict__ contigs, uint32_t chunk) {
    __shared__ LeanShared<R> sh;
    sweep_lean_body<PHASE, R, TRI>(contigs, chunk, sh);
}

template <int PHASE, int R, bool TRI>
DEVI void sweep_lean_body(const DevContig* __restrict__ contigs, uint32_t chunk, LeanShared<R>& sh) {
    const DevContig& dc = contigs[blockIdx.x];
    if (dc.lean != 1u) return;
    if ((dc.tri != 0u) != TRI) return;
    const uint32_t C = (uint32_t)__builtin_amdgcn_readfirstlane((int)*dc.n_cols);
    if (C == 0) return;
    const unsigned long long t_begin = kChainProf ? __builtin_amdgcn_s_memtime() : 0ull;
    if constexpr ((PHASE == 1 || PHASE == 3) && !TRI) {
        if (PHASE == 1 ? dc.sparse != 0u : (dc.sparse2 != 0u && C >= 2u)) {
            if (blockIdx.y == 0) lean_forward<PHASE, R, TRI, true>(dc, sh, C, chunk);
            else lean_backward<PHASE, R, TRI, true>(dc, sh, C, chunk);
        } else {
            if (blockIdx.y == 0) lean_forward<PHASE, R, TRI>(dc, sh, C, chunk);
            else lean_backward<PHASE, R, TRI>(dc, sh, C, chunk);
        }
    } else {
        if (blockIdx.y == 0) lean_forward<PHASE, R, TRI>(dc, sh, C, chunk);
        else lean_backward<PHASE, R, TRI>(dc, sh, C, chunk);
    }
    if (kChainProf && threadIdx.x == 0) {
        unsigned long long* o = dc.prof + (blockIdx.y == 0 ? 0 : 16) + (PHASE == 1 ? 0 : 8);
        o[0] = __builtin_amdgcn_s_memtime() - t_begin;
    }
}

#define PG_REFILL_PLACEMENT_LDS (100 * 1024)
template <int R>
__global__ __launch_bounds__((64 * 64 / R)) void k_refill_lean(const DevContig* __restrict__ contigs, uint32_t n_contigs, uint32_t chunk, uint32_t q, uint32_t phase2) {
    __shared__ LeanShared<R> sh;
    static_assert(sizeof(LeanShared<R>) + PG_REFILL_PLACEMENT_LDS <= 160 * 1024 && 2 * sizeof(LeanShared<R>) + PG_REFILL_PLACEMENT_LDS > 160 * 1024,
                  "a refill block fits a CU of its own and none that runs a sweep workgroup");
    const uint32_t total = 2u * q * n_contigs;
    for (uint32_t w = blockIdx.x; w < total; w += gridDim.x) {
        const uint32_t chain = w % n_contigs, role = (w / n_contigs) & 1u, j = w / (2u * n_contigs);
        const DevContig& dc = contigs[chain];
        if (dc.lean != 1u || dc.tri != 0u || !(phase2 ? dc.sparse2 : dc.sparse)) continue;
        const uint32_t C = (uint32_t)__builtin_amdgcn_readfirstlane((int)*dc.n_cols);
        const unsigned long long m = (unsigned long long)chunk * q + j + (phase2 ? 0u : 1u);
        uint32_t ck;
        if (phase2) {
            uint32_t seg[3];
            if (!pg_sparse2_segment(C, role, m, seg)) continue;
            ck = seg[0];
        } else {
            if (m > pg_sparse_segments(C, role)) continue;
            ck = pg_sparse_checkpoint(C, role, (uint32_t)m);
        }
        __syncthreads();
        if (role == 0u) lean_forward<5, R, false>(dc, sh, C, ck);
        else lean_backward<5, R, false>(dc, sh, C, ck);
    }
}


template <int HP>
struct LxCfg {
    static constexpr int R = HP / 4;
    static constexpr int NCH = HP / 64;
    static constexpr int NW = 4 * NCH;
    static constexpr int T = 64 * NW;
    static constexpr int NS = R / 16;
    static constexpr int RB = (PG_REC_ALLELES + HP + 63) & ~63;
    static constexpr int BLK = 16;
    static constexpr int PIECES = BLK * RB / 16;
    static constexpr int PPT = (PIECES + T - 1) / T;
    static_assert(R % 16 == 0 && (BLK * HP / 4) % T == 0, "bad lean-x geometry");
};
template <int HP>
struct LxShared {
    using Cfg = LxCfg<HP>;
    double psum[2][4][HP];
    double scal[2][64];
    unsigned char rec[2][Cfg::BLK][Cfg::RB] __attribute__((aligned(16)));
};
template <int HP>
struct LxRecs {
    using Cfg = LxCfg<HP>;
    const GAS char* base;
    int64_t origin, C;
    int dir;
    uint32_t tid;
    DEVI v2f64 fetch(uint32_t block, int p) const {
        uint32_t piece = tid + (uint32_t)p * Cfg::T;
        if constexpr (Cfg::PIECES % Cfg::T != 0) piece = piece < (uint32_t)Cfg::PIECES ? piece : (uint32_t)Cfg::PIECES - 1u;
        const uint32_t q = piece / (uint32_t)(Cfg::RB / 16), w = piece % (uint32_t)(Cfg::RB / 16);
        int64_t c = origin + (int64_t)dir * ((int64_t)block * Cfg::BLK + q);
        c = c < 0 ? 0 : (c >= C ? C - 1 : c);
        return *(const GAS v2f64*)(base + (size_t)c * Cfg::RB + w * 16u);
    }
    DEVI void park(LxShared<HP>& sh, uint32_t block, int p, v2f64 v) const {
        const uint32_t piece = tid + (uint32_t)p * Cfg::T;
        if (Cfg::PIECES % Cfg::T == 0 || piece < (uint32_t)Cfg::PIECES) ((v2f64*)&sh.rec[block & 1u][0][0])[piece] = v;
    }
};
template <int HP>
DEVI void lx_transform(LxShared<HP>& sh, uint32_t block, uint32_t tid) {
    using Cfg = LxCfg<HP>;
    auto f = [](uint32_t v) {
        uint32_t a = v & 0xFFFFu, b = v >> 16;
        a = a > (uint32_t)PG_AMAX ? (uint32_t)PG_AMAX : a;
        b = b > (uint32_t)PG_AMAX ? (uint32_t)PG_AMAX : b;
        return (a * (uint32_t)(PG_ESTRIDE * 8)) | ((b * (uint32_t)(PG_ESTRIDE * 8)) << 16);
    };
#pragma unroll
    for (uint32_t d = tid; d < (uint32_t)(Cfg::BLK * HP / 4); d += (uint32_t)Cfg::T) {
        uint32_t* ptr = (uint32_t*)(&sh.rec[block & 1u][d / (uint32_t)(HP / 4)][PG_REC_ALLELES]) + d % (uint32_t)(HP / 4);
        const uint32_t v = *ptr;
        *ptr = f(v & 0x00FF00FFu) | (f((v >> 8) & 0x00FF00FFu) << 8);
    }
}
template <int HP>
DEVI const unsigned char* lx_rec(const LxShared<HP>& sh, uint32_t rel ) {
    return sh.rec[(rel / (uint32_t)LxCfg<HP>::BLK) & 1u][rel % (uint32_t)LxCfg<HP>::BLK];
}
struct LxConsts { double c0, c1, c2, kappa; };
template <int HP>
DEVI LxConsts lx_consts(const LxShared<HP>& sh, uint32_t rel) {
    const double* q = (const double*)lx_rec(sh, rel);
    return LxConsts{q[0], q[1], q[2], q[3]};
}
template <int R>
struct LxAlleles { uint32_t col8; uint32_t rows[R / 4]; };
template <int HP>
DEVI LxAlleles<LxCfg<HP>::R> lx_alleles(const LxShared<HP>& sh, uint32_t rel, uint32_t j, uint32_t i0) {
    constexpr int R = LxCfg<HP>::R;
    const unsigned char* al = lx_rec(sh, rel) + PG_REC_ALLELES;
    LxAlleles<R> a;
    a.col8 = ((uint32_t)al[j] * 171u) >> 10;
#pragma unroll
    for (int q = 0; q < R / 4; ++q) a.rows[q] = ((const uint32_t*)(al + i0))[q];
    return a;
}
template <int HP>
DEVI uint32_t lx_ecol(const LxShared<HP>& sh, uint32_t rel, uint32_t col8) {
    return (uint32_t)(uintptr_t)(LAS const unsigned char*)(lx_rec(sh, rel) + PG_REC_E) + col8;
}
template <int HP, int K>
DEVI double lx_emission(uint32_t ecol, const LxAlleles<LxCfg<HP>::R>& a) {
    return *(LAS const double*)(uintptr_t)add_byte<(K & 3)>(a.rows[K >> 2], ecol);
}

template <int R>
struct LxTri {
    double fa[R / 2], fb[R / 2];
    uint32_t off[R / 2];
    uint32_t skip;
    DEVI void setup(uint32_t i0, uint32_t j) {
        skip = 0;
#pragma unroll
        for (int q = 0; q < R / 2; ++q) {
            const uint32_t r0 = i0 + 2u * (uint32_t)q;
            fa[q] = j < r0 ? 0.0 : (j == r0 ? 0.5 : 1.0);
            fb[q] = j <= r0 ? 0.0 : (j == r0 + 1u ? 0.5 : 1.0);
            const bool off_q = j < (r0 & ~7u);
            skip |= (off_q ? 1u : 0u) << q;
            off[q] = off_q ? 0u : tri_unit_of(r0 >> 1, j) * 16u;
        }
    }
    DEVI void put(GAS char* col, int q, double a, double b) const {
        if (!((skip >> q) & 1u)) *(gdouble2*)(col + off[q]) = v2f64{a * fa[q], b * fb[q]};
    }
};
template <int PHASE, int HP, bool TRI = false, bool WIDE = false>
DEVI void leanx_forward(const DevContig& dc, LxShared<HP>& sh, uint32_t C, uint32_t chunk) {
    static_assert(!TRI || (PHASE == 1 && HP == 64), "triangle stores: phase 1 at 64 paths");
    using Cfg = LxCfg<HP>;
    constexpr int R = Cfg::R, NS = Cfg::NS, BLK = Cfg::BLK, PPT = Cfg::PPT;
    const uint32_t mid = C / 2, K = dc.chunk_cols;
    uint32_t lo = PHASE == 1 ? 0u : mid, hi = PHASE == 1 ? mid : C;
    if constexpr (PHASE == 3) {
        const unsigned long long l = (unsigned long long)mid + (unsigned long long)chunk * K;
        if (l >= C) return;
        lo = (uint32_t)l;
        hi = C - lo > K ? lo + K : C;
    }
    if (lo >= hi) return;
    const uint32_t first = lo == 0 ? 1u : lo;
    const uint32_t tid = threadIdx.x, lane = tid & 63u;
    const uint32_t wave = __builtin_amdgcn_readfirstlane(tid >> 6);
    const uint32_t rg = wave / (uint32_t)Cfg::NCH, i0 = rg * R, j = (wave % (uint32_t)Cfg::NCH) * 64u + lane;
    const uint32_t H = dc.H;
    const size_t colsz = TRI ? (size_t)dc.col_stride : (size_t)HP * HP;
    const double unif = 1.0 / ((double)H * (double)H);
    LxRecs<HP> recs{(const GAS char*)dc.colrec, (int64_t)first - 1, (int64_t)C, +1, tid};
    v2f64 piece[PPT];
#pragma unroll
    for (int p = 0; p < PPT; ++p) recs.park(sh, 0, p, recs.fetch(0, p));
#pragma unroll
    for (int p = 0; p < PPT; ++p) piece[p] = recs.fetch(1, p);
    lds_barrier();
    lx_transform<HP>(sh, 0, tid);
    lds_barrier();
    gdouble* fwd = (gdouble*)dc.fwd;
    gdouble* fscale = (gdouble*)dc.fscale;
    gu8* fallback = (gu8*)dc.fwd_fallback;
    gdouble* wr = fwd;
    gcdouble* resume = (gcdouble*)(fwd + (size_t)(lo > 0 ? lo - 1 : 0) * colsz);
    if constexpr (PHASE == 3) {
        gdouble* scr = (gdouble*)dc.scratch;
        wr = scr + (size_t)(PG_SCR_BUF(chunk) * 2u) * K * colsz - (size_t)lo * colsz;
        if (chunk > 0) resume = (gcdouble*)(scr + ((size_t)(PG_SCR_BUF(chunk - 1u) * 2u) * K + (K - 1u)) * colsz);
    }
    const size_t toff = (size_t)(i0 >> 1) * HP + j;
    GAS char* sp[R / 8];
#pragma unroll
    for (int g = 0; g < R / 8; ++g) sp[g] = (GAS char*)(wr + (size_t)first * colsz) + toff * 16u + (size_t)(4 * g + 2) * (size_t)(HP * 16);
    LxTri<TRI ? R : 2> ltri;
    if constexpr (TRI) ltri.setup(i0, j);
    auto store_col = [&](uint32_t c, const double (&v)[R]) {
        if constexpr (TRI) {
            GAS char* col = (GAS char*)(wr + (size_t)c * colsz);
#pragma unroll
            for (int k = 0; k < R; k += 2) ltri.put(col, k >> 1, v[k], v[k + 1]);
            return;
// ... 2515 lines not shown
```

### pangenie_amd/csrc/pg_shim.cpp

```cpp
#include <hip/hip_runtime_api.h>

#include <math.h>
#include <stdarg.h>
#include <stdio.h>
#include <stdlib.h>
#include <string.h>

#include <algorithm>
#include <atomic>
#include <chrono>
#include <condition_variable>
#include <map>
#include <memory>
#include <mutex>
#include <string>
#include <thread>
#include <vector>

#include "../../include/pangenie_hmm.h"
#include "pg_device.h"
#include "pg_job.h"
#include "pg_launch.h"

using namespace pgj;
// ... 1417 lines not shown
        if (!batches) { set_err(err, errlen, "batches must be given"); return PG_ERR_INVALID; }
        for (uint32_t i = 0; i < n; ++i) specs[i] = {i, batches[i].kmer_count, batches[i].coverage};
    }
    const int rc = check_chain_arrays(job, specs, err, errlen);
    if (rc != PG_OK) return rc;
    return upload_inputs(job, batches, specs, batches != nullptr, err, errlen);
}

extern "C" int pg_job_upload_begin(pg_job* job, const pg_sample_counts* samples, char* err, size_t errlen) {
    if (!job) { set_err(err, errlen, "null job"); return PG_ERR_INVALID; }
    if (job->upload_pending) { set_err(err, errlen, "an upload is already in flight: call pg_job_upload_end first"); return PG_ERR_INVALID; }
    HIP_TRY(hipSetDevice(job->device));
    if (!job->cohort) { set_err(err, errlen, "not a cohort job"); return PG_ERR_INVALID; }
    if (!samples) { set_err(err, errlen, "cohort job: samples must be given"); return PG_ERR_INVALID; }
    auto specs = std::make_shared<std::vector<ChainSpec>>();
    int rc = cohort_chain_specs(job->n_samples, job->n_contigs, samples, *specs, err, errlen);
    if (rc == PG_OK) rc = check_chain_arrays(job, *specs, err, errlen);
    if (rc != PG_OK) return rc;
    const size_t n = job->chains.size();
    if (!job->copy_stream) HIP_TRY(hipStreamCreateWithFlags(&job->copy_stream, hipStreamNonBlocking));
    if (!job->alt_samples) {
        hipError_t he = hipMalloc((void**)&job->alt_samples, job->sample_bytes ? job->sample_bytes : 8);
        if (he != hipSuccess) {
            (void)hipGetLastError();
            job->alt_samples = nullptr;
            pg_hmm_release_cache();
            hipSetDevice(job->device);
            he = hipMalloc((void**)&job->alt_samples, job->sample_bytes ? job->sample_bytes : 8);
        }
        if (he == hipSuccess) he = hipMalloc((void**)&job->d_contigs_owned, sizeof(DevContig) * n);
        job->d_contigs_alt = job->d_contigs_owned;
        if (he != hipSuccess) {
            if (job->alt_samples) { hipFree(job->alt_samples); job->alt_samples = nullptr; }
            job->d_contigs_alt = job->d_contigs_owned = nullptr;
            set_err(err, errlen, "hipMalloc (second sample set, %zu bytes) failed: %s", job->sample_bytes, hipGetErrorString(he));
            return PG_ERR_NOMEM;
        }
    }
    unsigned char* other = job->cur_samples == job->alt_samples ? job->arena + job->sample_lo : job->alt_samples;
    DevContig* d_other = job->d_contigs_alt;
    job->next_coverage.assign(n, {});
    job->upload_pending = true;
    job->upload_rc = PG_OK;
    job->upload_err.clear();
    if (job->uploader.joinable()) job->uploader.join();
    job->uploader = std::thread([job, specs, other, d_other, n]() {
        char e[256] = {0};
        uint64_t bytes = 0;
        int r = hipSetDevice(job->device) == hipSuccess ? PG_OK : PG_ERR_DEVICE;
        if (r == PG_OK) r = sample_upload(job, *specs, other, job->copy_stream, &job->next_coverage, &bytes, e, sizeof(e));
        if (r == PG_OK) {
            std::vector<DevContig> hd = job->h_contigs;
            for (size_t c = 0; c < n; ++c) {
                hd[c].cov = (const uint16_t*)(other + (job->chains[c].o_cov - job->sample_lo));
                hd[c].kmer_count = (const uint16_t*)(other + (job->chains[c].o_kcnt - job->sample_lo));
            }
            if (hipMemcpyAsync(d_other, hd.data(), sizeof(DevContig) * n, hipMemcpyHostToDevice, job->copy_stream) != hipSuccess ||
                hipStreamSynchronize(job->copy_stream) != hipSuccess) { r = PG_ERR_DEVICE; snprintf(e, sizeof(e), "descriptor upload failed"); }
            else job->h_contigs.swap(hd);
        }
        job->up_bytes[0] = 0; job->up_bytes[1] = bytes;
        job->upload_rc = r;
        job->upload_err = e;
    });
    return PG_OK;
}

extern "C" int pg_job_upload_end(pg_job* job, char* err, size_t errlen) {
    if (!job) { set_err(err, errlen, "null job"); return PG_ERR_INVALID; }
    if (!job->upload_pending) { set_err(err, errlen, "no upload in flight"); return PG_ERR_INVALID; }
    const double t0 = now_s();
    if (job->uploader.joinable()) job->uploader.join();
    job->upload_pending = false;
    job->host_s[1] = now_s() - t0;
    if (job->upload_rc != PG_OK) { set_err(err, errlen, "%s", job->upload_err.c_str()); return job->upload_rc; }
    std::swap(job->d_contigs, job->d_contigs_alt);
    job->cur_samples = job->cur_samples == job->alt_samples ? job->arena + job->sample_lo : job->alt_samples;
    for (size_t c = 0; c < job->chains.size(); ++c) {
        job->chains[c].coverage.swap(job->next_coverage[c]);
        job->chains[c].d = job->h_contigs[c];
    }
    job->ran = false;
    return PG_OK;
}

extern "C" int pgi_job_fill_begin(pg_job* job, uint32_t sample, int device, uint32_t n_contigs, const uint32_t* n_variants,
                                  const uint32_t* const* kmer_off, void* stream, uint16_t** d_kmer_count, uint16_t** d_coverage,
                                  char* err, size_t errlen) {
    if (!job) { set_err(err, errlen, "null job"); return PG_ERR_INVALID; }
    if (!job->cohort) { set_err(err, errlen, "not a cohort job"); return PG_ERR_INVALID; }
    if (job->upload_pending) { set_err(err, errlen, "an asynchronous upload is in flight: call pg_job_upload_end first"); return PG_ERR_INVALID; }
    if (job->device != device) { set_err(err, errlen, "the job is on device %d, the counter on device %d", job->device, device); return PG_ERR_INVALID; }
    if (sample >= job->n_samples) { set_err(err, errlen, "sample %u of %u", sample, job->n_samples); return PG_ERR_INVALID; }
    if (n_contigs != job->n_contigs) { set_err(err, errlen, "the plan has %u contigs, the job %u", n_contigs, job->n_contigs); return PG_ERR_INVALID; }
    for (uint32_t c = 0; c < n_contigs; ++c) {
        const IndexHost& x = job->index[c];
        if (n_variants[c] != x.V || (x.V && memcmp(kmer_off[c], x.koff.data(), ((size_t)x.V + 1) * 4) != 0)) {
            set_err(err, errlen, "contig %u: variants or k-mers per variant of the plan differ from the resident job", c);
            return PG_ERR_INVALID;
        }
    }
    HIP_TRY(hipSetDevice(job->device));
    if (!job->ev_fill) HIP_TRY(hipEventCreateWithFlags(&job->ev_fill, hipEventDisableTiming));
    HIP_TRY(hipEventRecord(job->ev_fill, job->stream));
    HIP_TRY(hipStreamWaitEvent((hipStream_t)stream, job->ev_fill, 0));
    job->ran = false;
    for (uint32_t c = 0; c < n_contigs; ++c) {
        const ChainHost& ch = job->chains[(size_t)sample * n_contigs + c];
        d_kmer_count[c] = (uint16_t*)(job->cur_samples + (ch.o_kcnt - job->sample_lo));
        d_coverage[c] = (uint16_t*)(job->cur_samples + (ch.o_cov - job->sample_lo));
    }
    return PG_OK;
}

extern "C" int pgi_job_fill_end(pg_job* job, uint32_t sample, uint32_t n_contigs, const uint16_t* const* coverage, void* stream,
                                char* err, size_t errlen) {
    HIP_TRY(hipEventRecord(job->ev_fill, (hipStream_t)stream));
    HIP_TRY(hipStreamWaitEvent(job->stream, job->ev_fill, 0));
    for (uint32_t c = 0; c < n_contigs; ++c) {
        const uint32_t V = job->index[c].V;
        if (V) job->chains[(size_t)sample * n_contigs + c].coverage.assign(coverage[c], coverage[c] + V);
    }
    job->ran = false;
    return PG_OK;
}

extern "C" int pg_job_fetch(pg_job* job, uint32_t ci, pg_contig_result* out, char* err, size_t errlen) {
    if (!job || !out || ci >= job->chains.size()) { set_err(err, errlen, "bad argument"); return PG_ERR_INVALID; }
    if (!job->ran) { set_err(err, errlen, "pg_job_run has not been called"); return PG_ERR_INVALID; }
    const double t0 = now_s();
    HIP_TRY(hipSetDevice(job->device));
    const ChainHost& c = job->chains[ci];
    const IndexHost& x = job->index[c.index];
    out->n_columns = c.n_cols_host;
    if (x.V == 0) return PG_OK;
    if (out->lik && x.n_lik) HIP_TRY(hipMemcpy(out->lik, c.d.lik, x.n_lik * sizeof(double), hipMemcpyDeviceToHost));
    if (out->lik_exp && x.n_lik) HIP_TRY(hipMemcpy(out->lik_exp, c.d.lik_exp, x.n_lik * sizeof(int32_t), hipMemcpyDeviceToHost));
    if (out->kept) HIP_TRY(hipMemcpy(out->kept, c.d.kept, x.V, hipMemcpyDeviceToHost));
    if (out->allele_present && x.sumA) HIP_TRY(hipMemcpy(out->allele_present, c.d.allele_present, x.sumA, hipMemcpyDeviceToHost));
    const bool fill = job->params.run_genotyping && c.n_cols_host > 0;
    const size_t nvit = job->params.run_phasing ? c.n_cols_host : 0;
    if (out->n_kmers) {
        if (fill) memcpy(out->n_kmers, x.n_kmers.data(), (size_t)x.V * 2);
        else { memset(out->n_kmers, 0, (size_t)x.V * 2); memcpy(out->n_kmers, x.n_kmers.data(), nvit * 2); }
    }
    if (out->coverage) {
        if (fill) memcpy(out->coverage, c.coverage.data(), (size_t)x.V * 2);
        else { memset(out->coverage, 0, (size_t)x.V * 2); memcpy(out->coverage, c.coverage.data(), nvit * 2); }
    }
    if (job->params.run_phasing) {
        if (out->haplotype_1) HIP_TRY(hipMemcpy(out->haplotype_1, c.d.hap1, (size_t)x.V * 2, hipMemcpyDeviceToHost));
        if (out->haplotype_2) HIP_TRY(hipMemcpy(out->haplotype_2, c.d.hap2, (size_t)x.V * 2, hipMemcpyDeviceToHost));
    }
    job->host_s[3] += now_s() - t0;
    return PG_OK;
}

extern "C" int pg_job_fetch_all(pg_job* job, pg_contig_result* outs, char* err, size_t errlen) {
    if (!job || !outs) { set_err(err, errlen, "bad argument"); return PG_ERR_INVALID; }
    if (!job->ran) { set_err(err, errlen, "pg_job_run has not been called"); return PG_ERR_INVALID; }
    const double t0 = now_s();
    HIP_TRY(hipSetDevice(job->device));
    hipStream_t s = job->stream;
    for (size_t ci = 0; ci < job->chains.size(); ++ci) {
        const ChainHost& c = job->chains[ci];
        const IndexHost& x = job->index[c.index];
        pg_contig_result* out = &outs[ci];
        out->n_columns = c.n_cols_host;
        if (x.V == 0) continue;
        if (out->lik && x.n_lik) HIP_TRY(hipMemcpyAsync(out->lik, c.d.lik, x.n_lik * sizeof(double), hipMemcpyDeviceToHost, s));
        if (out->lik_exp && x.n_lik) HIP_TRY(hipMemcpyAsync(out->lik_exp, c.d.lik_exp, x.n_lik * sizeof(int32_t), hipMemcpyDeviceToHost, s));
        if (out->kept) HIP_TRY(hipMemcpyAsync(out->kept, c.d.kept, x.V, hipMemcpyDeviceToHost, s));
        if (out->allele_present && x.sumA) HIP_TRY(hipMemcpyAsync(out->allele_present, c.d.allele_present, x.sumA, hipMemcpyDeviceToHost, s));
        if (job->params.run_phasing) {
            if (out->haplotype_1) HIP_TRY(hipMemcpyAsync(out->haplotype_1, c.d.hap1, (size_t)x.V * 2, hipMemcpyDeviceToHost, s));
            if (out->haplotype_2) HIP_TRY(hipMemcpyAsync(out->haplotype_2, c.d.hap2, (size_t)x.V * 2, hipMemcpyDeviceToHost, s));
        }
        const bool fill = job->params.run_genotyping && c.n_cols_host > 0;
        const size_t nvit = job->params.run_phasing ? c.n_cols_host : 0;
        if (out->n_kmers) {
            if (fill) memcpy(out->n_kmers, x.n_kmers.data(), (size_t)x.V * 2);
            else { memset(out->n_kmers, 0, (size_t)x.V * 2); memcpy(out->n_kmers, x.n_kmers.data(), nvit * 2); }
        }
        if (out->coverage) {
            if (fill) memcpy(out->coverage, c.coverage.data(), (size_t)x.V * 2);
            else { memset(out->coverage, 0, (size_t)x.V * 2); memcpy(out->coverage, c.coverage.data(), nvit * 2); }
        }
    }
    HIP_TRY(hipStreamSynchronize(s));
    job->host_s[3] += now_s() - t0;
    return PG_OK;
}

extern "C" int pg_job_panel_sizes(const pg_job* job, uint32_t ci, uint32_t* n_variants, uint32_t* n_paths, uint64_t* sum_kmers, uint64_t* sum_alleles) {
    if (!job || ci >= job->chains.size()) return PG_ERR_INVALID;
    const IndexHost& x = job->index[job->chains[ci].index];
    if (n_variants) *n_variants = x.V;
    if (n_paths) *n_paths = x.H;
    if (sum_kmers) *sum_kmers = x.sumK;
    if (sum_alleles) *sum_alleles = x.sumA;
    return PG_OK;
}
extern "C" int pg_job_fetch_panel(pg_job* job, uint32_t ci, uint32_t* kmer_off, uint16_t* kmer_count, uint32_t* allele_off, uint16_t* allele_id,
                                  uint8_t* allele_flags, uint16_t* allele_kmer_off, uint32_t* allele_kmer_mask, uint16_t* path_allele,
                                  char* err, size_t errlen) {
    if (!job || ci >= job->chains.size()) { set_err(err, errlen, "bad argument"); return PG_ERR_INVALID; }
    HIP_TRY(hipSetDevice(job->device));
    const ChainHost& c = job->chains[ci];
    const IndexHost& x = job->index[c.index];
    if (x.V == 0) return PG_OK;
    const unsigned char* A = job->arena;
    if (kmer_off) HIP_TRY(hipMemcpy(kmer_off, A + x.o_koff, ((size_t)x.V + 1) * 4, hipMemcpyDeviceToHost));
    if (kmer_count && x.sumK) HIP_TRY(hipMemcpy(kmer_count, job->cur_samples + (c.o_kcnt - job->sample_lo), (size_t)x.sumK * 2, hipMemcpyDeviceToHost));
    if (allele_off) HIP_TRY(hipMemcpy(allele_off, A + x.o_aoff, ((size_t)x.V + 1) * 4, hipMemcpyDeviceToHost));
    if (allele_id) HIP_TRY(hipMemcpy(allele_id, A + x.o_aid, (size_t)x.sumA * 2, hipMemcpyDeviceToHost));
    if (allele_flags) HIP_TRY(hipMemcpy(allele_flags, A + x.o_aflag, (size_t)x.sumA, hipMemcpyDeviceToHost));
    if (allele_kmer_off) HIP_TRY(hipMemcpy(allele_kmer_off, A + x.o_akoff, (size_t)x.sumA * 2, hipMemcpyDeviceToHost));
    if (allele_kmer_mask) HIP_TRY(hipMemcpy(allele_kmer_mask, A + x.o_akmask, (size_t)x.sumA * 4, hipMemcpyDeviceToHost));
    if (path_allele) HIP_TRY(hipMemcpy(path_allele, A + x.o_pa, (size_t)x.V * x.H * 2, hipMemcpyDeviceToHost));
    return PG_OK;
}

extern "C" int pg_job_device_results(pg_job* job, uint32_t ci, void** d_lik, uint64_t* n_lik, void** d_lik_exp, uint64_t* n_variants) {
    if (!job || ci >= job->chains.size()) return PG_ERR_INVALID;
    const ChainHost& c = job->chains[ci];
    const IndexHost& x = job->index[c.index];
    if (d_lik) *d_lik = c.d.lik;
    if (n_lik) *n_lik = x.n_lik;
    if (d_lik_exp) *d_lik_exp = c.d.lik_exp;
    if (n_variants) *n_variants = x.V;
    return PG_OK;
}

extern "C" int pg_job_packed_results(pg_job* job, void** d_lik, void** d_lik_exp, uint64_t* n_lik_total) {
    if (!job) return PG_ERR_INVALID;
    if (d_lik) *d_lik = job->d_lik;
    if (d_lik_exp) *d_lik_exp = job->d_likexp;
    if (n_lik_total) *n_lik_total = job->n_lik_total;
    return PG_OK;
}

extern "C" uint32_t pg_job_n_chains(const pg_job* job) { return job ? (uint32_t)job->chains.size() : 0; }

extern "C" int pg_job_host_seconds(const pg_job* job, double out4[4]) {
    if (!job || !out4) return PG_ERR_INVALID;
    for (int i = 0; i < 4; ++i) out4[i] = job->host_s[i];
    return PG_OK;
}
extern "C" int pg_job_upload_bytes(const pg_job* job, uint64_t out2[2]) {
    if (!job || !out2) return PG_ERR_INVALID;
    out2[0] = job->up_bytes[0]; out2[1] = job->up_bytes[1];
    return PG_OK;
}

extern "C" int pg_job_profile_counters(pg_job* job, uint32_t ci, uint64_t out64[64]) {
    if (!job || !out64 || ci >= job->chains.size()) return PG_ERR_INVALID;
    if (hipSetDevice(job->device) != hipSuccess) return PG_ERR_DEVICE;
    if (hipMemcpy(out64, job->chains[ci].d.prof, 64 * sizeof(uint64_t), hipMemcpyDeviceToHost) != hipSuccess) return PG_ERR_DEVICE;
    return PG_OK;
}

extern "C" int pg_job_kernel_ms(const pg_job* job, double ms[PG_N_KERNEL_CLASSES]) {
    if (!job || !ms) return PG_ERR_INVALID;
    for (int i = 0; i < PG_N_KERNEL_CLASSES; ++i) ms[i] = job->ms[i];
    return PG_OK;
}
extern "C" const char* pg_job_kernel_name(int cls) { return (cls >= 0 && cls < PG_N_KERNEL_CLASSES) ? kKernelNames[cls] : ""; }
extern "C" uint64_t pg_job_device_bytes(const pg_job* job) { return job ? job->arena_bytes : 0; }
extern "C" int pg_job_sweep_mode(const pg_job* job, uint32_t* chunk_cols) {
    if (!job) return PG_ERR_INVALID;
    if (chunk_cols) *chunk_cols = job->chunk_cols;
    return job->chunked ? 1 : 0;
}

extern "C" double pg_job_viterbi_ms(const pg_job* job) { return job ? job->vit_ms : 0.0; }

extern "C" double pg_job_index_ms(const pg_job* job) { return job ? job->index_ms : 0.0; }
extern "C" size_t pg_job_plan(const pg_job* job, char* out, size_t len) {
    if (!job) return 0;
    std::string t = job->plan_text;
    if (job->persist) {
        char line[160];
        snprintf(line, sizeof(line), "  persistent phase 2: %u run(s), %u more fell back to a launch per chunk\n", job->persist_runs, job->persist_fallbacks);
        t += line;
    }
    if (out && len) { const size_t n = t.size() < len - 1 ? t.size() : len - 1; memcpy(out, t.data(), n); out[n] = 0; }
    return t.size() + 1;
}
extern "C" int pg_sparse_segment(uint32_t n_columns, uint32_t chunk_cols, uint32_t chunk, uint32_t role, uint32_t j, uint32_t out[3]) {
    if (role > 1u || chunk_cols == 0u || chunk_cols % PG_LEAN_SPARSE != 0u || j >= chunk_cols / PG_LEAN_SPARSE) return -1;
    const unsigned long long m = (unsigned long long)chunk * (chunk_cols / PG_LEAN_SPARSE) + j + 1u;
    if (m > pg_sparse_segments(n_columns, role)) return 0;
    const uint32_t ck = pg_sparse_checkpoint(n_columns, role, (uint32_t)m);
    if (out) { out[0] = ck; out[1] = role == 0u ? ck + 1u : ck - (PG_LEAN_SPARSE - 1u); out[2] = role == 0u ? ck + (PG_LEAN_SPARSE - 1u) : ck - 1u; }
    return 1;
}
extern "C" int pg_sparse_piece_range(uint32_t n_columns, uint32_t chunk_cols, uint32_t piece_chunks, uint32_t piece, uint32_t role, uint32_t out[2]) {
    if (role > 1u || chunk_cols == 0u || chunk_cols % PG_LEAN_SPARSE != 0u || piece_chunks == 0u || (unsigned long long)piece_chunks * chunk_cols > 0xFFFFFFFFull) return -1;
    uint32_t r[2];
    if (!pg_sparse_piece(n_columns, role, piece_chunks * chunk_cols, piece, r)) return 0;
    if (out) { out[0] = r[0]; out[1] = r[1]; }
    return 1;
}
extern "C" int pg_prep_parts(uint32_t n_columns, uint32_t chunk_cols, uint32_t piece_chunks, uint32_t n_pieces, uint32_t early,
                             const uint32_t* col_variant, uint32_t n_variants, uint32_t out_cols[2], uint32_t out_vars[2]) {
    if (chunk_cols == 0u || chunk_cols % PG_LEAN_SPARSE != 0u || piece_chunks == 0u || (unsigned long long)piece_chunks * chunk_cols > 0xFFFFFFFFull) return -1;
    if (early == 0u || n_pieces == 0u || n_columns > n_variants) return -1;
    if (n_pieces < early + 1u) return 0;
    const uint32_t W = pg_prep_band(n_pieces, early, piece_chunks * chunk_cols);
    if (out_cols) pg_prep_middle(n_columns, W, out_cols);
    if (out_vars) {
        if (!col_variant && n_columns) return -1;
        pg_prep_middle_variants(col_variant, n_columns, n_variants, W, out_vars);
    }
    return 1;
}
extern "C" uint32_t pg_prep_part_member(uint32_t part, uint32_t lo, uint32_t hi, uint32_t n, uint32_t u) {
    if ((part != 1u && part != 2u) || lo > hi || hi > n) return n;
    return pg_prep_part_item(part, lo, hi, n, u);
}
extern "C" int pg_sparse_chunk_segment(uint32_t n_columns, uint32_t chunk_cols, uint32_t chunk, uint32_t role, uint32_t j, uint32_t out[3]) {
    if (role > 1u || chunk_cols == 0u || chunk_cols % PG_LEAN_SPARSE != 0u || j >= chunk_cols / PG_LEAN_SPARSE) return -1;
    uint32_t seg[3];
    if (!pg_sparse2_segment(n_columns, role, (unsigned long long)chunk * (chunk_cols / PG_LEAN_SPARSE) + j, seg)) return 0;
    if (out) { out[0] = seg[0]; out[1] = seg[1]; out[2] = seg[2]; }
    return 1;
}
extern "C" int pg_sparse_chunk_stored_by_chain(uint32_t n_columns, uint32_t role, uint32_t column) {
    return role <= 1u && column < n_columns && pg_sparse2_stored(n_columns, role, column) ? 1 : 0;
}
extern "C" int pg_sparse_stored_by_chain(uint32_t n_columns, uint32_t role, uint32_t column) {
    return role <= 1u && column < n_columns && pg_sparse_stored(n_columns, role, column) ? 1 : 0;
}
extern "C" uint32_t pg_job_triangle_chains(const pg_job* job) {
    if (!job) return 0;
    uint32_t n = 0;
    for (const auto& ch : job->chains) n += ch.d.tri ? 1u : 0u;
    return n;
}

namespace {

int genotype_single(const pg_contig_batch* batch, const pg_table* table, const pg_hmm_params* params, int device,
                    pg_contig_result* out, char* err, size_t errlen) {
    std::vector<ChainSpec> specs(1);
    specs[0] = {0, batch->kmer_count, batch->coverage};
    pg_job* job = nullptr;
    int rc = job_build(device, 1, batch, specs, 1, false, table, params, true, &job, err, errlen);
    if (rc != PG_OK) return rc;
    rc = pg_job_run(job, nullptr, err, errlen);
    if (rc == PG_OK) rc = pg_job_fetch(job, 0, out, err, errlen);
    pg_job_destroy(job);
    return rc;
}

struct CoRequest {
    const pg_contig_batch* batch; pg_contig_result* out; char* err; size_t errlen;
    int rc = PG_OK; bool done = false;
};
struct CoBatch {
    int device; const pg_table* table; pg_hmm_params params;
    std::vector<CoRequest*> reqs;
    std::chrono::steady_clock::time_point last_arrival;
};
struct Coalescer {
    std::mutex mu;
    std::condition_variable cv;
    std::vector<std::shared_ptr<CoBatch>> open;
    int callers_inside = 0;
    int announced[PG_MAX_DEVICES_HOST] = {0};
    int inflight[PG_MAX_DEVICES_HOST] = {0};
    std::chrono::steady_clock::time_point last_concurrency = std::chrono::steady_clock::time_point::min();
    uint64_t stat_batches = 0, stat_requests = 0, stat_largest = 0;
} g_co;

long env_long(const char* name, long dflt) { const char* e = getenv(name); return e ? strtol(e, nullptr, 0) : dflt; }

bool same_params(const pg_hmm_params& a, const pg_hmm_params& b) {
    return a.effective_N == b.effective_N && a.recombrate == b.recombrate && (a.uniform != 0) == (b.uniform != 0) &&
           (a.run_genotyping != 0) == (b.run_genotyping != 0) && (a.run_phasing != 0) == (b.run_phasing != 0);
}

void run_merged(CoBatch& b) {
    const size_t n = b.reqs.size();
    pg_hmm_params prm = b.params;
    prm.reserved = 0;
    if (n > 1) {
        std::vector<pg_contig_batch> bs(n);
        std::vector<ChainSpec> specs(n);
        for (size_t i = 0; i < n; ++i) { bs[i] = *b.reqs[i]->batch; specs[i] = {(uint32_t)i, bs[i].kmer_count, bs[i].coverage}; }
        char err[512] = {0};
        pg_job* job = nullptr;
        int rc = job_build(b.device, (uint32_t)n, bs.data(), specs, 1, false, b.table, &prm, true, &job, err, sizeof(err));
        if (rc == PG_OK) rc = pg_job_run(job, nullptr, err, sizeof(err));
        if (rc == PG_OK) {
            std::vector<pg_contig_result> outs(n);
            for (size_t i = 0; i < n; ++i) outs[i] = *b.reqs[i]->out;
            rc = pg_job_fetch_all(job, outs.data(), err, sizeof(err));
            for (size_t i = 0; i < n; ++i) b.reqs[i]->out->n_columns = outs[i].n_columns;
        }
        if (job) pg_job_destroy(job);
        if (rc == PG_OK) { for (CoRequest* r : b.reqs) r->rc = PG_OK; return; }
    }
    for (CoRequest* r : b.reqs) r->rc = genotype_single(r->batch, b.table, &prm, b.device, r->out, r->err, r->errlen);
}

}

extern "C" void pg_hmm_announce(int device) {
    if (device < 0 || device >= PG_MAX_DEVICES_HOST) return;
    std::lock_guard<std::mutex> lock(g_co.mu);
    g_co.announced[device] += 1;
}
extern "C" void pg_hmm_retract(int device) {
    if (device < 0 || device >= PG_MAX_DEVICES_HOST) return;
    std::lock_guard<std::mutex> lock(g_co.mu);
    if (g_co.announced[device] > 0) g_co.announced[device] -= 1;
    g_co.cv.notify_all();
}
extern "C" int pg_hmm_coalesce_stats(uint64_t out3[3]) {
    if (!out3) return PG_ERR_INVALID;
    std::lock_guard<std::mutex> lock(g_co.mu);
    out3[0] = g_co.stat_batches; out3[1] = g_co.stat_requests; out3[2] = g_co.stat_largest;
    return PG_OK;
}

extern "C" int pg_hmm_genotype_contig(const pg_contig_batch* batch, const pg_table* table, const pg_hmm_params* params,
                                      int device, pg_contig_result* out, char* err, size_t errlen) {
    if (!batch || !table || !params || !out) { set_err(err, errlen, "null argument"); return PG_ERR_INVALID; }
    using clock = std::chrono::steady_clock;
    static const bool enabled = env_long("PG_COALESCE", 1) != 0;
    static const long wait_ms = env_long("PG_COALESCE_WAIT_MS", 250);
    const long window_us = 300, max_inflight = 2, max_batch = 256;
    const bool announced = (params->reserved & PG_CALL_ANNOUNCED) != 0;
    if (!enabled || device < 0 || device >= PG_MAX_DEVICES_HOST) {
        if (announced) pg_hmm_retract(device);
        return genotype_single(batch, table, params, device, out, err, errlen);
    }
    CoRequest req{batch, out, err, errlen};
    std::shared_ptr<CoBatch> mine;
    {
        std::unique_lock<std::mutex> lk(g_co.mu);
        if (announced && g_co.announced[device] > 0) g_co.announced[device] -= 1;
        g_co.callers_inside += 1;
        if (g_co.callers_inside > 1) g_co.last_concurrency = clock::now();
        for (auto& ob : g_co.open)
            if (ob->device == device && ob->table == table && same_params(ob->params, *params) && (long)ob->reqs.size() < max_batch) {
                ob->reqs.push_back(&req);
                ob->last_arrival = clock::now();
                g_co.cv.notify_all();
                g_co.cv.wait(lk, [&] { return req.done; });
                g_co.callers_inside -= 1;
                return req.rc;
            }
        mine = std::make_shared<CoBatch>();
        mine->device = device; mine->table = table; mine->params = *params;
        mine->reqs.push_back(&req);
        mine->last_arrival = clock::now();
        g_co.open.push_back(mine);
        g_co.cv.notify_all();
        const clock::time_point hard = clock::now() + std::chrono::milliseconds(wait_ms);
        for (;;) {
            const clock::time_point now = clock::now();
            const bool concurrent = g_co.callers_inside > 1 || (g_co.last_concurrency != clock::time_point::min() &&
                                                                now - g_co.last_concurrency < std::chrono::seconds(2));
            const clock::time_point quiet_until = mine->last_arrival + std::chrono::microseconds(concurrent ? window_us : 0);
            const bool slot = g_co.inflight[device] < max_inflight;
            const bool coming = g_co.announced[device] > 0 && now < hard;
            const bool full = (long)mine->reqs.size() >= max_batch;
            if (slot && (full || (!coming && now >= quiet_until))) break;
            clock::time_point until = now + std::chrono::milliseconds(50);
            if (slot && !coming && quiet_until < until) until = quiet_until;
            if (coming && hard < until) until = hard;
            g_co.cv.wait_until(lk, until);
        }
        for (size_t i = 0; i < g_co.open.size(); ++i)
            if (g_co.open[i] == mine) { g_co.open.erase(g_co.open.begin() + (long)i); break; }
        g_co.inflight[device] += 1;
        g_co.stat_batches += 1; g_co.stat_requests += mine->reqs.size();
        if (mine->reqs.size() > g_co.stat_largest) g_co.stat_largest = mine->reqs.size();
    }
    try {
        run_merged(*mine);
    } catch (...) {
        for (CoRequest* r : mine->reqs) {
            r->rc = PG_ERR_DEVICE;
            set_err(r->err, r->errlen, "merged one-shot job failed with a host exception");
        }
    }
    {
        std::lock_guard<std::mutex> lk(g_co.mu);
        g_co.inflight[device] -= 1;
        g_co.callers_inside -= 1;
        for (CoRequest* r : mine->reqs) r->done = true;
        g_co.cv.notify_all();
    }
    return req.rc;
}

extern "C" int pg_emission_table(const pg_contig_batch* batch, const pg_table* table, uint32_t v, int device,
                                 long double* out, int32_t* all_zeros_out, char* err, size_t errlen) {
    if (!batch || !table || !out || v >= batch->n_variants) { set_err(err, errlen, "bad argument"); return PG_ERR_INVALID; }
    pg_hmm_params p;
    memset(&p, 0, sizeof(p));
    p.effective_N = 25000.0L; p.recombrate = 1.26; p.run_genotyping = 1;
    pg_job* job = nullptr;
    int rc = pg_job_new(device, 1, batch, table, &p, &job, err, errlen);
    if (rc != PG_OK) return rc;
    const uint32_t A = batch->allele_off[v + 1] - batch->allele_off[v];
    double* dm = nullptr; int* de = nullptr;
    std::vector<double> m((size_t)A * A);
    std::vector<int> e((size_t)A * A);
    if (hipMalloc((void**)&dm, m.size() * 8 + 8) != hipSuccess || hipMalloc((void**)&de, e.size() * 4 + 8) != hipSuccess) {
        set_err(err, errlen, "hipMalloc failed"); rc = PG_ERR_NOMEM;
    } else {
        pgk_launch_emission_single(job->d_contigs, job->tab, v, dm, de, job->stream);
        if (hipStreamSynchronize(job->stream) != hipSuccess ||
            hipMemcpy(m.data(), dm, m.size() * 8, hipMemcpyDeviceToHost) != hipSuccess ||
            hipMemcpy(e.data(), de, e.size() * 4, hipMemcpyDeviceToHost) != hipSuccess) {
            set_err(err, errlen, "emission kernel failed: %s", hipGetErrorString(hipGetLastError())); rc = PG_ERR_DEVICE;
        }
    }
    if (dm) hipFree(dm);
    if (de) hipFree(de);
    pg_job_destroy(job);
    if (rc != PG_OK) return rc;
    bool all_zeros = true;
    for (size_t i = 0; i < m.size(); ++i) {
        out[i] = ldexpl((long double)m[i], e[i]);
        if (out[i] > 0) all_zeros = false;
    }
    if (all_zeros)
        for (size_t i = 0; i < m.size(); ++i) out[i] = 1.0L;
    if (all_zeros_out) *all_zeros_out = all_zeros ? 1 : 0;
    return PG_OK;
}

extern "C" int pg_transition_probs(uint64_t from_pos, uint64_t to_pos, double recombrate, uint32_t nr_paths, int uniform,
                                   long double effective_N, int device, double out3[3], char* err, size_t errlen) {
    if (!out3 || nr_paths == 0) { set_err(err, errlen, "bad argument"); return PG_ERR_INVALID; }
    int ndev = 0;
    if (hipGetDeviceCount(&ndev) != hipSuccess || ndev == 0) { set_err(err, errlen, "no HIP device available (no CPU fallback)"); return PG_ERR_DEVICE; }
    HIP_TRY(hipSetDevice(device));
    double* d = nullptr;
    HIP_TRY(hipMalloc((void**)&d, 3 * sizeof(double)));
    const long double dist = (to_pos - from_pos) * 0.000004L * ((long double)recombrate) * effective_N;
    pgk_launch_transition_single((double)dist, nr_paths, uniform, d, nullptr);
    hipError_t he = hipMemcpy(out3, d, 3 * sizeof(double), hipMemcpyDeviceToHost);
    hipFree(d);
    if (he != hipSuccess) { set_err(err, errlen, "transition kernel failed: %s", hipGetErrorString(he)); return PG_ERR_DEVICE; }
    return PG_OK;
}
```

Measured before the change: 24.21 million.

## Unify lean record LDS buffers into 256-byte ring images and align sparse upkeep

New measurement: 27.07 million (median of 6 runs). 1.12x the previous value.

```diff
diff --git a/include/pangenie_hmm.h b/include/pangenie_hmm.h
--- a/include/pangenie_hmm.h
+++ b/include/pangenie_hmm.h
@@ -97,6 +97,8 @@
 int pg_sparse_chunk_segment(uint32_t n_columns, uint32_t chunk_cols, uint32_t chunk, uint32_t role, uint32_t j, uint32_t out[3]);
 int pg_sparse_chunk_stored_by_chain(uint32_t n_columns, uint32_t role, uint32_t column);
 int pg_sparse_piece_range(uint32_t n_columns, uint32_t chunk_cols, uint32_t piece_chunks, uint32_t piece, uint32_t role, uint32_t out[2]);
+int pg_lean_ring_schedule(uint32_t n_columns, uint32_t chunk_cols, uint32_t piece_chunks, uint32_t role, uint32_t form, uint32_t arg, uint32_t out[6]);
+uint32_t pg_lean_ring_image_offset(uint32_t record);
 int pg_prep_parts(uint32_t n_columns, uint32_t chunk_cols, uint32_t piece_chunks, uint32_t n_pieces, uint32_t early,
                   const uint32_t* col_variant, uint32_t n_variants, uint32_t out_cols[2], uint32_t out_vars[2]);
 uint32_t pg_prep_part_member(uint32_t part, uint32_t lo, uint32_t hi, uint32_t n, uint32_t u);
diff --git a/pangenie_amd/_lib.py b/pangenie_amd/_lib.py
--- a/pangenie_amd/_lib.py
+++ b/pangenie_amd/_lib.py
@@ -148,6 +148,10 @@
     lib.pg_sparse_chunk_stored_by_chain.restype = C.c_int
     lib.pg_sparse_piece_range.argtypes = [C.c_uint32, C.c_uint32, C.c_uint32, C.c_uint32, C.c_uint32, u32p]
     lib.pg_sparse_piece_range.restype = C.c_int
+    lib.pg_lean_ring_schedule.argtypes = [C.c_uint32, C.c_uint32, C.c_uint32, C.c_uint32, C.c_uint32, C.c_uint32, u32p]
+    lib.pg_lean_ring_schedule.restype = C.c_int
+    lib.pg_lean_ring_image_offset.argtypes = [C.c_uint32]
+    lib.pg_lean_ring_image_offset.restype = C.c_uint32
     lib.pg_prep_parts.argtypes = [C.c_uint32, C.c_uint32, C.c_uint32, C.c_uint32, C.c_uint32, u32p, C.c_uint32, u32p, u32p]
     lib.pg_prep_parts.restype = C.c_int
     lib.pg_prep_part_member.argtypes = [C.c_uint32] * 5
@@ -300,7 +304,7 @@
     "pg_job_record_gl_ms", "pg_record_gl_from_bins", "pg_gl_from_values", "pg_gl_text",
     "pg_job_record_plan_strided", "pg_job_record_first", "pg_job_fetch_record_calls_packed", "pg_job_fetch_record_gl_packed",
     "pg_sparse_segment", "pg_sparse_stored_by_chain", "pg_sparse_chunk_segment", "pg_sparse_chunk_stored_by_chain", "pg_sparse_piece_range",
-    "pg_prep_parts", "pg_prep_part_member",
+    "pg_prep_parts", "pg_prep_part_member", "pg_lean_ring_schedule", "pg_lean_ring_image_offset",
 ]
 
 
diff --git a/pangenie_amd/csrc/pg_device.h b/pangenie_amd/csrc/pg_device.h
--- a/pangenie_amd/csrc/pg_device.h
+++ b/pangenie_amd/csrc/pg_device.h
@@ -205,6 +205,38 @@
     else { out[0] = (uint32_t)(mid + d0); out[1] = (uint32_t)(mid + d1 - 1u); }
     return true;
 }
+#define PG_LEAN_IMAGE 256u
+PG_HD inline uint32_t pg_lean_ring_image(uint32_t rel) { return (rel * PG_LEAN_IMAGE) & (2u * PG_LEAN_SPARSE * PG_LEAN_IMAGE - 1u); }
+#define PG_LEAN_RING_PARK (PG_LEAN_SPARSE - 4u)
+#define PG_LEAN_RING_EXPAND (PG_LEAN_SPARSE - 3u)
+PG_HD inline uint32_t pg_lean_ring_first(uint32_t lead) { return (PG_LEAN_SPARSE - lead % PG_LEAN_SPARSE) % PG_LEAN_SPARSE; }
+PG_HD inline uint32_t pg_lean_ring_lead(uint32_t C, uint32_t role, uint32_t phase, uint32_t c0, uint32_t end) {
+    if (phase != 1u) return 0u;
+    if (role == 0u) { const uint32_t ck0 = end ? (end - 1u) % PG_LEAN_SPARSE : 0u; return c0 <= ck0 ? ck0 - c0 + 1u : 0u; }
+    const unsigned long long ckh = (unsigned long long)(C / 2u) + (unsigned long long)pg_sparse_segments(C, 1u) * PG_LEAN_SPARSE;
+    return c0 >= ckh ? (uint32_t)(c0 - ckh) + 1u : 0u;
+}
+PG_HD inline bool pg_lean_ring_launch(uint32_t C, uint32_t role, uint32_t phase, uint32_t K, uint32_t chunk, uint32_t out[3]) {
+    const unsigned long long mid = C / 2u;
+    if (role == 0u) {
+        unsigned long long lo = phase == 1u ? 0u : mid, hi = phase == 1u ? mid : C;
+        if (phase == 3u) { lo = mid + (unsigned long long)chunk * K; if (lo >= C) return false; hi = C - lo > K ? lo + K : C; }
+        if (phase == 1u && chunk) { uint32_t pc[2]; if (!pg_sparse_piece(C, 0u, (chunk >> 16) * K, chunk & 0xFFFFu, pc)) return false; lo = pc[0]; hi = pc[1] + 1ull; }
+        const unsigned long long first = lo == 0u ? 1u : lo;
+        if (first >= hi) return false;
+        out[0] = (uint32_t)first; out[1] = (uint32_t)(hi - first); out[2] = pg_lean_ring_lead(C, 0u, phase, (uint32_t)first, (uint32_t)hi);
+        return true;
+    }
+    if (C == 0u) return false;
+    long long top = phase == 1u ? (long long)C - 1 : (long long)mid - 1, bot = phase == 1u ? (long long)mid : 0;
+    if (phase == 3u) { top = (long long)mid - 1 - (long long)chunk * K; if (top < 0) return false; bot = top - (long long)K + 1 > 0 ? top - (long long)K + 1 : 0; }
+    bool resumed = phase != 1u;
+    if (phase == 1u && chunk) { uint32_t pc[2]; if (!pg_sparse_piece(C, 1u, (chunk >> 16) * K, chunk & 0xFFFFu, pc)) return false; bot = pc[0]; top = pc[1]; resumed = top != (long long)C - 1; }
+    const long long t0 = resumed ? top : top - 1;
+    if (t0 < bot) return false;
+    out[0] = (uint32_t)t0; out[1] = (uint32_t)(t0 - bot + 1); out[2] = pg_lean_ring_lead(C, 1u, phase, (uint32_t)t0, (uint32_t)bot);
+    return true;
+}
 #define PG_PREP_EARLY_PIECES_DEFAULT 2u
 PG_HD inline uint32_t pg_prep_band(uint32_t n_pieces, uint32_t E, uint32_t piece_cols) {
     const unsigned long long W = (unsigned long long)(n_pieces - E) * piece_cols;
diff --git a/pangenie_amd/csrc/pg_experiments.h b/pangenie_amd/csrc/pg_experiments.h
--- a/pangenie_amd/csrc/pg_experiments.h
+++ b/pangenie_amd/csrc/pg_experiments.h
@@ -14,6 +14,10 @@
 #define PG_LEAN_EXP 0
 #endif
 static constexpr unsigned kLeanExp = PG_LEAN_EXP;
+#ifndef PG_LEAN_UPKEEP_EXP
+#define PG_LEAN_UPKEEP_EXP 0
+#endif
+static constexpr unsigned kLeanUpkeepExp = PG_LEAN_UPKEEP_EXP;
 #ifdef PG_LEAN_DPPSUM
 static constexpr bool kLeanDppSum = true;
 #else
diff --git a/pangenie_amd/csrc/pg_kernels.hip b/pangenie_amd/csrc/pg_kernels.hip
--- a/pangenie_amd/csrc/pg_kernels.hip
+++ b/pangenie_amd/csrc/pg_kernels.hip
@@ -2458,11 +2458,16 @@
     double psum[2][NW][64];
     double ptot[2][NW] __attribute__((aligned(32)));
     double u[NW][64] __attribute__((aligned(16)));
-    double rec[2][PG_LEAN_BLOCK][8] __attribute__((aligned(16)));
     double scal[2][64];
-    v2f64 tab[2][PG_LEAN_BLOCK][4][2];
-    unsigned char comb[2][PG_LEAN_BLOCK][NW][R / 2] __attribute__((aligned(8)));
+    double img[2 * PG_LEAN_BLOCK][PG_LEAN_IMAGE / 8] __attribute__((aligned(PG_LEAN_IMAGE)));
 };
+static_assert(PG_LEAN_IMAGE == 256 && (2 * PG_LEAN_BLOCK * PG_LEAN_IMAGE & (2 * PG_LEAN_BLOCK * PG_LEAN_IMAGE - 1)) == 0, "image(rel): a shift and a mask");
+constexpr uint32_t kLeanImgTab = 64u, kLeanImgComb = 192u;
+template <class SH>
+DEVI LAS const unsigned char* lean_image(const SH& sh, uint32_t rel ) {
+    static_assert(sizeof(sh.img) == 2u * PG_LEAN_SPARSE * PG_LEAN_IMAGE, "pg_lean_ring_image");
+    return (LAS const unsigned char*)&sh.img[0][0] + pg_lean_ring_image(rel);
+}
 struct FRec {
     double c0, c1, c2, kappa, E00, E01, E11;
     unsigned long long bits1;
@@ -2480,12 +2485,12 @@
     }
     template <class SH>
     DEVI void park(SH& sh, uint32_t block, v2f64 piece) const {
-        if (tid < 256u) ((v2f64*)&sh.rec[block & 1u][0][0])[tid] = piece;
+        if (tid < 256u) *(v2f64*)&sh.img[(block & 1u) * PG_LEAN_BLOCK + (tid >> 2)][(tid & 3u) * 2u] = piece;
     }
 };
 template <class SH>
 DEVI FRec read_frec(const SH& sh, uint32_t rel ) {
-    const double* q = sh.rec[(rel / PG_LEAN_BLOCK) & 1u][rel % PG_LEAN_BLOCK];
+    LAS const double* q = (LAS const double*)lean_image(sh, rel);
     FRec r;
     r.c0 = q[0]; r.c1 = q[1]; r.c2 = q[2]; r.kappa = q[3]; r.E00 = q[4]; r.E01 = q[5]; r.E11 = q[6];
     r.bits1 = (unsigned long long)__double_as_longlong(q[7]);
@@ -2566,34 +2571,34 @@
 }
 template <class SH>
 DEVI void lean_expand(SH& sh, uint32_t block , uint32_t tid) {
-    static_assert(sizeof(sh.comb[0][0]) == 32, "four waves of eight row pairs");
+    static_assert(sizeof(sh.img[0]) == PG_LEAN_IMAGE && kLeanImgComb + 4u * 8u <= PG_LEAN_IMAGE, "four waves of eight row pairs");
     if (tid >= 256u) return;
-    const uint32_t b = block & 1u;
+    double* im = sh.img[(block & 1u) * PG_LEAN_BLOCK + (tid >> 2)];
     {
-        const uint32_t r = tid >> 2, c = tid & 3u;
-        const double* rc = sh.rec[b][r];
-        const double E00 = rc[4], E01 = rc[5], E11 = rc[6];
-        sh.tab[b][r][c][0] = v2f64{(c & 1u) ? E01 : E00, (c & 2u) ? E01 : E00};
-        sh.tab[b][r][c][1] = v2f64{(c & 1u) ? E11 : E01, (c & 2u) ? E11 : E01};
+        const uint32_t c = tid & 3u;
+        const double E00 = im[4], E01 = im[5], E11 = im[6];
+        v2f64* tab = (v2f64*)((unsigned char*)im + kLeanImgTab);
+        tab[c * 2u + 0u] = v2f64{(c & 1u) ? E01 : E00, (c & 2u) ? E01 : E00};
+        tab[c * 2u + 1u] = v2f64{(c & 1u) ? E11 : E01, (c & 2u) ? E11 : E01};
     }
     {
-        const uint32_t r = tid >> 2, w = tid & 3u;
-        const unsigned long long bits = (unsigned long long)__double_as_longlong(sh.rec[b][r][7]);
+        const uint32_t w = tid & 3u;
+        const unsigned long long bits = (unsigned long long)__double_as_longlong(im[7]);
         const uint32_t b16 = (uint32_t)(bits >> (16u * w)) & 0xFFFFu;
         auto spread = [](uint32_t v8) { return ((v8 & 3u) | (((v8 >> 2) & 3u) << 8) | (((v8 >> 4) & 3u) << 16) | (((v8 >> 6) & 3u) << 24)) << 5; };
         typedef uint32_t u32x2 __attribute__((ext_vector_type(2)));
-        *(u32x2*)&sh.comb[b][r][w][0] = u32x2{spread(b16 & 0xFFu), spread(b16 >> 8)};
+        *(u32x2*)((unsigned char*)im + kLeanImgComb + w * 8u) = u32x2{spread(b16 & 0xFFu), spread(b16 >> 8)};
     }
 }
 struct LeanPairs { uint32_t tbase, cd0, cd1; };
 typedef uint32_t u32x2 __attribute__((ext_vector_type(2)));
 template <class SH>
 DEVI u32x2 lean_pair_bytes(const SH& sh, uint32_t rel , uint32_t wave ) {
-    return *(const u32x2*)&sh.comb[(rel / PG_LEAN_BLOCK) & 1u][rel % PG_LEAN_BLOCK][wave][0];
+    return *(LAS const u32x2*)(lean_image(sh, rel) + kLeanImgComb + wave * 8u);
 }
 template <class SH>
 DEVI LeanPairs lean_pairs(const SH& sh, uint32_t rel , u32x2 cd, uint32_t aj ) {
-    return LeanPairs{(uint32_t)(uintptr_t)(LAS const unsigned char*)&sh.tab[(rel / PG_LEAN_BLOCK) & 1u][rel % PG_LEAN_BLOCK][0][0] + aj * 16u, cd.x, cd.y};
+    return LeanPairs{(uint32_t)(uintptr_t)lean_image(sh, rel) + kLeanImgTab + aj * 16u, cd.x, cd.y};
 }
 template <class SH>
 DEVI LeanPairs lean_pairs(const SH& sh, uint32_t rel, uint32_t wave, uint32_t aj) { return lean_pairs(sh, rel, lean_pair_bytes(sh, rel, wave), aj); }
@@ -2604,6 +2609,42 @@
 template <int R>
 DEVI void lean_pairs_all(const LeanPairs& lp, double (&e)[R]) {
     static_for<0, R / 2>([&](auto pc) __attribute__((always_inline)) { constexpr int q = decltype(pc)::value; const v2f64 t = lean_pair<q>(lp); e[2 * q] = t.x; e[2 * q + 1] = t.y; });
+}
+template <class SH>
+DEVI v2f64 lean_ring_open(SH& sh, const LeanRecs& recs, uint32_t s0 , uint32_t tid) {
+    const bool two = s0 > PG_LEAN_RING_PARK;
+    recs.park(sh, 0, recs.fetch(0));
+    v2f64 piece = recs.fetch(1);
+    if (two) {
+        lds_barrier();
+        lean_expand(sh, 0, tid);
+        lds_barrier();
+        recs.park(sh, 1, piece);
+        piece = recs.fetch(2);
+    }
+    lds_barrier();
+    lean_expand(sh, two ? 1u : 0u, tid);
+    lds_barrier();
+    return piece;
+}
+constexpr int kUpkeepTested = -1, kUpkeepNone = 0, kUpkeepPark = 1, kUpkeepExpand = 2;
+template <int UPKEEP, class SH>
+DEVI void lean_ring_upkeep(SH& sh, const LeanRecs& recs, v2f64& piece, uint32_t n , uint32_t tid) {
+    if constexpr (UPKEEP == kUpkeepTested || (kLeanUpkeepExp & 1u)) {
+        if (((n + 4u) % PG_LEAN_BLOCK) == 0u) {
+            const uint32_t blk = (n + 4u) / PG_LEAN_BLOCK;
+            recs.park(sh, blk, piece);
+            piece = recs.fetch(blk + 1u);
+        } else if (((n + 3u) % PG_LEAN_BLOCK) == 0u) {
+            lean_expand(sh, (n + 3u) / PG_LEAN_BLOCK, tid);
+        }
+    } else if constexpr (UPKEEP == kUpkeepPark) {
+        const uint32_t blk = (n + 4u) / PG_LEAN_BLOCK;
+        recs.park(sh, blk, piece);
+        piece = recs.fetch(blk + 1u);
+    } else if constexpr (UPKEEP == kUpkeepExpand) {
+        lean_expand(sh, (n + 3u) / PG_LEAN_BLOCK, tid);
+    }
 }
 template <int R>
 DEVI double lean_colsum(const LeanShared<R>& sh, uint32_t pb, uint32_t lane) {
@@ -2703,12 +2744,9 @@
     const uint32_t i0 = wave * R;
     const size_t colsz = TRI ? (size_t)dc.col_stride : (size_t)HP * HP;
     const double unif = 1.0 / 4096.0;
-    LeanRecs recs{(const GAS char*)dc.frec, (int64_t)first - 1, (int64_t)C, +1, tid};
-    recs.park(sh, 0, recs.fetch(0));
-    v2f64 piece = recs.fetch(1);
-    lds_barrier();
-    lean_expand(sh, 0, tid);
-    lds_barrier();
+    const uint32_t s0 = SPARSE ? pg_lean_ring_first(pg_lean_ring_lead(C, 0u, (uint32_t)PHASE, first, hi)) : 0u;
+    LeanRecs recs{(const GAS char*)dc.frec, (int64_t)first - 1 - (int64_t)s0, (int64_t)C, +1, tid};
+    v2f64 piece = lean_ring_open(sh, recs, s0, tid);
     gdouble* fwd = (gdouble*)dc.fwd;
     gdouble* fscale = (gdouble*)dc.fscale;
     gu8* fallback = (gu8*)dc.fwd_fallback;
@@ -2788,7 +2826,7 @@
     ColScalars fsc{&sh.scal[0][0]};
     double x[R];
     {
-        const FRec r0 = read_frec(sh, 0);
+        const FRec r0 = read_frec(sh, s0);
         double eA, eB;
         emis(r0, eA, eB);
         const uint32_t rb = (uint32_t)__builtin_amdgcn_readfirstlane((int)((uint32_t)(r0.bits1 >> i0) & RMASK));
@@ -2819,29 +2857,33 @@
     }
     double ec[R];
     {
-        const FRec r1 = read_frec(sh, 1);
-        lean_pairs_all<R>(lean_pairs(sh, 1, wave, (uint32_t)((r1.bits1 >> lane) & 1ull)), ec);
+        const FRec r1 = read_frec(sh, s0 + 1u);
+        lean_pairs_all<R>(lean_pairs(sh, s0 + 1u, wave, (uint32_t)((r1.bits1 >> lane) & 1ull)), ec);
     }
     LeanTimeline tl;
     tl.init();
-    auto step = [&](auto store_c, uint32_t t, const FRec& cur, FRec& nxt) __attribute__((always_inline)) {
+    auto step = [&](auto store_c, auto upkeep_c, uint32_t t, const FRec& cur, FRec& nxt) __attribute__((always_inline)) {
         constexpr bool STORE = decltype(store_c)::value;
-        const uint32_t n = t - first;
+        constexpr int UPKEEP = decltype(upkeep_c)::value;
+        const uint32_t n = t - first + s0;
         tl.template mark<0>(0.0);
-        nxt = read_frec(sh, n + 2u);
-        const u32x2 cdn = lean_pair_bytes(sh, n + 2u, wave);
-        if (((n + 4u) % PG_LEAN_BLOCK) == 0u) {
-            const uint32_t blk = (n + 4u) / PG_LEAN_BLOCK;
-            recs.park(sh, blk, piece);
-            piece = recs.fetch(blk + 1u);
-        } else if (((n + 3u) % PG_LEAN_BLOCK) == 0u) {
-            lean_expand(sh, (n + 3u) / PG_LEAN_BLOCK, tid);
-        }
+        u32x2 cdn;
+        auto next_record = [&]() __attribute__((always_inline)) {
+            nxt = read_frec(sh, n + 2u);
+            cdn = lean_pair_bytes(sh, n + 2u, wave);
+            lean_ring_upkeep<UPKEEP>(sh, recs, piece, n, tid);
+        };
+        if constexpr (kLeanUpkeepExp & 2u) next_record();
         const uint32_t pb = (t - 1) & 1u;
         double pc[64 / R], pr[64 / R];
 #pragma unroll
         for (int q = 0; q < 64 / R; ++q) { pc[q] = sh.psum[pb][q][lane]; pr[q] = sh.psum[pb][q][i0 + (lane & 15u)]; }
         const double Spre = kLeanPreTotal ? lean_total<R>(sh, pb) : 0.0;
+        if constexpr (!(kLeanUpkeepExp & 2u)) {
+            lean_fence();
+            next_record();
+            lean_fence();
+        }
         const double Cj = (pc[0] + pc[1]) + (pc[2] + pc[3]);
         tl.template mark<1>(Cj);
         const v4f64 zz = {0.0, 0.0, 0.0, 0.0};
@@ -2901,9 +2943,13 @@
         tl.template mark<8>(0.0);
         tl.template fold<8>();
     };
-    FRec ra = read_frec(sh, 1), rb2;
+    FRec ra = read_frec(sh, s0 + 1u), rb2;
     constexpr std::true_type kStore{};
     constexpr std::false_type kNoStore{};
+    constexpr std::integral_constant<int, kUpkeepTested> kTested{};
+    constexpr std::integral_constant<int, kUpkeepNone> kNone{};
+    constexpr std::integral_constant<int, kUpkeepPark> kPark{};
+    constexpr std::integral_constant<int, kUpkeepExpand> kExpand{};
     __builtin_amdgcn_s_waitcnt(0x0F70);
     lds_barrier();
     uint32_t t = first;
@@ -2913,10 +2959,10 @@
         uint32_t q = 0, cend = hi - lo > K ? lo + K : hi;
         for (;;) {
             for (; t + 1 < cend; t += 2) {
-                step(kStore, t, ra, rb2);
-                step(kStore, t + 1, rb2, ra);
-            }
-            if (t < cend) { step(kStore, t, ra, rb2); ++t; }
+                step(kStore, kTested, t, ra, rb2);
+                step(kStore, kTested, t + 1, rb2, ra);
+            }
+            if (t < cend) { step(kStore, kTested, t, ra, rb2); ++t; }
             if (wave == 0 && fsc.valid) fsc.flush(fscale, lane, cend - 1);
             {
                 const double Cj = lean_colsum<R>(sh, (cend - 1) & 1u, lane);
@@ -2936,33 +2982,36 @@
         if constexpr (PHASE == 1) {
             const uint32_t ck0 = (hi - 1u) % PG_LEAN_SPARSE;
             for (; t + 1 <= ck0; t += 2) {
-                step(kStore, t, ra, rb2);
-                step(kStore, t + 1, rb2, ra);
-            }
-            if (t <= ck0) { step(kStore, t, ra, rb2); ra = rb2; ++t; }
-        }
+                step(kStore, kTested, t, ra, rb2);
+                step(kStore, kTested, t + 1, rb2, ra);
+            }
+            if (t <= ck0) { step(kStore, kTested, t, ra, rb2); ra = rb2; ++t; }
+        }
+        static_assert(PG_LEAN_SPARSE == PG_LEAN_BLOCK && PG_LEAN_RING_PARK % 2u == 0u && PG_LEAN_RING_EXPAND == PG_LEAN_RING_PARK + 1u && PG_LEAN_RING_PARK + 4u == PG_LEAN_SPARSE, "the group's last four steps: park, expand, plain, store");
         while (hi - t >= PG_LEAN_SPARSE) {
-            for (uint32_t g = 0; g + 1u < PG_LEAN_SPARSE / 2u; ++g, t += 2) {
-                step(kNoStore, t, ra, rb2);
-                step(kNoStore, t + 1, rb2, ra);
-            }
-            step(kNoStore, t, ra, rb2);
-            step(kStore, t + 1, rb2, ra);
-            t += 2;
+            for (uint32_t g = 0; g < PG_LEAN_RING_PARK / 2u; ++g, t += 2) {
+                step(kNoStore, kNone, t, ra, rb2);
+                step(kNoStore, kNone, t + 1, rb2, ra);
+            }
+            step(kNoStore, kPark, t, ra, rb2);
+            step(kNoStore, kExpand, t + 1, rb2, ra);
+            step(kNoStore, kNone, t + 2, ra, rb2);
+            step(kStore, kNone, t + 3, rb2, ra);
+            t += 4;
         }
         if constexpr (PHASE == 3) {
             for (; t + 1 < hi; t += 2) {
-                step(kNoStore, t, ra, rb2);
-                step(kNoStore, t + 1, rb2, ra);
-            }
-            if (t < hi) step(kNoStore, t, ra, rb2);
+                step(kNoStore, kTested, t, ra, rb2);
+                step(kNoStore, kTested, t + 1, rb2, ra);
+            }
+            if (t < hi) step(kNoStore, kTested, t, ra, rb2);
         }
     } else {
         for (; t + 1 < hi; t += 2) {
-            step(kStore, t, ra, rb2);
-            step(kStore, t + 1, rb2, ra);
-        }
-        if (t < hi) step(kStore, t, ra, rb2);
+            step(kStore, kTested, t, ra, rb2);
+            step(kStore, kTested, t + 1, rb2, ra);
+        }
+        if (t < hi) step(kStore, kTested, t, ra, rb2);
     }
     if constexpr (!SPARSE) if (wave == 0 && fsc.valid) fsc.flush(fscale, lane, hi - 1);
     if (kLeanTimeline && tid == 0) tl.write(dc.prof + 32);
@@ -3006,12 +3055,9 @@
     const uint32_t i0 = wave * R;
     const size_t colsz = TRI ? (size_t)dc.col_stride : (size_t)HP * HP;
     const double unif = 1.0 / 4096.0;
-    LeanRecs recs{(const GAS char*)dc.frec, t0 + 1, (int64_t)C, -1, tid};
-    recs.park(sh, 0, recs.fetch(0));
-    v2f64 piece = recs.fetch(1);
-    lds_barrier();
-    lean_expand(sh, 0, tid);
-    lds_barrier();
+    const uint32_t s0 = SPARSE && t0 >= bot ? pg_lean_ring_first(pg_lean_ring_lead(C, 1u, (uint32_t)PHASE, (uint32_t)t0, (uint32_t)bot)) : 0u;
+    LeanRecs recs{(const GAS char*)dc.frec, t0 + 1 + (int64_t)s0, (int64_t)C, -1, tid};
+    v2f64 piece = lean_ring_open(sh, recs, s0, tid);
     gdouble* cols = (gdouble*)dc.fwd;
     gdouble* bscale = (gdouble*)dc.bscale;
     gdouble* bsum = (gdouble*)dc.bsum;
@@ -3081,7 +3127,7 @@
     if constexpr (PHASE == 5) if (seg2 && pg_sparse2_stored(C, 1u, (uint32_t)bot)) noscal = bot;
     ColScalars bsc{&sh.scal[0][0]}, bsm{&sh.scal[1][0]};
     double w[R], Sy;
-    FRec cur = read_frec(sh, 0);
+    FRec cur = read_frec(sh, s0);
     {
         double y[R];
         if (!resumed) {
@@ -3112,24 +3158,19 @@
     }
     double ec[R];
     {
-        const FRec r1 = read_frec(sh, 1);
-        lean_pairs_all<R>(lean_pairs(sh, 1, wave, (uint32_t)((r1.bits1 >> lane) & 1ull)), ec);
+        const FRec r1 = read_frec(sh, s0 + 1u);
+        lean_pairs_all<R>(lean_pairs(sh, s0 + 1u, wave, (uint32_t)((r1.bits1 >> lane) & 1ull)), ec);
     }
     double one = 1.0;
     asm volatile("" : "+v"(one));
     LeanTimeline tl;
     tl.init();
-    auto step = [&](auto store_c, int64_t t, const FRec& cur, FRec& nxt) __attribute__((always_inline)) {
+    auto step = [&](auto store_c, auto upkeep_c, int64_t t, const FRec& cur, FRec& nxt) __attribute__((always_inline)) {
         constexpr bool STORE = decltype(store_c)::value;
-        const uint32_t n = (uint32_t)(t0 - t);
+        constexpr int UPKEEP = decltype(upkeep_c)::value;
+        const uint32_t n = (uint32_t)(t0 - t) + s0;
         tl.template mark<0>(0.0);
-        if (((n + 4u) % PG_LEAN_BLOCK) == 0u) {
-            const uint32_t blk = (n + 4u) / PG_LEAN_BLOCK;
-            recs.park(sh, blk, piece);
-            piece = recs.fetch(blk + 1u);
-        } else if (((n + 3u) % PG_LEAN_BLOCK) == 0u) {
-            lean_expand(sh, (n + 3u) / PG_LEAN_BLOCK, tid);
-        }
+        lean_ring_upkeep<UPKEEP>(sh, recs, piece, n, tid);
         int es = exponent_of(Sy) - PG_BIAS_B;
         es = es < -900 ? -900 : es;
         const double m = ldexp(Sy, -es - PG_BIAS_B);
@@ -3148,7 +3189,7 @@
         const double Spre = kLeanPreTotal ? lean_total<R>(sh, pb) : 0.0;
         lean_fence();
         nxt = read_frec(sh, n + 1u);
-        const unsigned long long bits_n = (unsigned long long)__double_as_longlong(sh.rec[((n + 2u) / PG_LEAN_BLOCK) & 1u][(n + 2u) % PG_LEAN_BLOCK][7]);
+        const unsigned long long bits_n = (unsigned long long)__double_as_longlong(((LAS const double*)lean_image(sh, n + 2u))[7]);
         const u32x2 cdn = lean_pair_bytes(sh, n + 2u, wave);
         lean_fence();
         const double Cj = (pc[0] + pc[1]) + (pc[2] + pc[3]);
@@ -3214,6 +3255,10 @@
     FRec rb2;
     constexpr std::true_type kStore{};
     constexpr std::false_type kNoStore{};
+    constexpr std::integral_constant<int, kUpkeepTested> kTested{};
+    constexpr std::integral_constant<int, kUpkeepNone> kNone{};
+    constexpr std::integral_constant<int, kUpkeepPark> kPark{};
+    constexpr std::integral_constant<int, kUpkeepExpand> kExpand{};
     int64_t t = t0;
     __builtin_amdgcn_s_waitcnt(0x0F70);
     if constexpr (PHASE == 4) {
@@ -3222,10 +3267,10 @@
         uint32_t q = 0;
         for (;;) {
             for (; t - 1 >= cbot; t -= 2) {
-                step(kStore, t, cur, rb2);
-                step(kStore, t - 1, rb2, cur);
-            }
-            if (t >= cbot) { step(kStore, t, cur, rb2); --t; }
+                step(kStore, kTested, t, cur, rb2);
+                step(kStore, kTested, t - 1, rb2, cur);
+            }
+            if (t >= cbot) { step(kStore, kTested, t, cur, rb2); --t; }
             if (wave == 1 && bsc.valid) bsc.flush(bscale, lane, (uint64_t)cbot);
             if (wave == 2 && bsm.valid) bsm.flush(bsum, lane, (uint64_t)cbot);
             chunk_publish(dc.sync + 1, q + 1u);
@@ -3242,33 +3287,35 @@
         if constexpr (PHASE == 1) {
             const int64_t ckh = mid + (int64_t)pg_sparse_segments(C, 1u) * (int64_t)PG_LEAN_SPARSE;
             for (; t - 1 >= ckh; t -= 2) {
-                step(kStore, t, cur, rb2);
-                step(kStore, t - 1, rb2, cur);
-            }
-            if (t >= ckh) { step(kStore, t, cur, rb2); cur = rb2; --t; }
+                step(kStore, kTested, t, cur, rb2);
+                step(kStore, kTested, t - 1, rb2, cur);
+            }
+            if (t >= ckh) { step(kStore, kTested, t, cur, rb2); cur = rb2; --t; }
         }
         while (t - bot >= (int64_t)PG_LEAN_SPARSE - 1) {
-            for (uint32_t g = 0; g + 1u < PG_LEAN_SPARSE / 2u; ++g, t -= 2) {
-                step(kNoStore, t, cur, rb2);
-                step(kNoStore, t - 1, rb2, cur);
-            }
-            step(kNoStore, t, cur, rb2);
-            step(kStore, t - 1, rb2, cur);
-            t -= 2;
+            for (uint32_t g = 0; g < PG_LEAN_RING_PARK / 2u; ++g, t -= 2) {
+                step(kNoStore, kNone, t, cur, rb2);
+                step(kNoStore, kNone, t - 1, rb2, cur);
+            }
+            step(kNoStore, kPark, t, cur, rb2);
+            step(kNoStore, kExpand, t - 1, rb2, cur);
+            step(kNoStore, kNone, t - 2, cur, rb2);
+            step(kStore, kNone, t - 3, rb2, cur);
+            t -= 4;
         }
         if constexpr (PHASE == 3) {
             for (; t - 1 >= bot; t -= 2) {
-                step(kNoStore, t, cur, rb2);
-                step(kNoStore, t - 1, rb2, cur);
-            }
-            if (t >= bot) step(kNoStore, t, cur, rb2);
+                step(kNoStore, kTested, t, cur, rb2);
+                step(kNoStore, kTested, t - 1, rb2, cur);
+            }
+            if (t >= bot) step(kNoStore, kTested, t, cur, rb2);
         }
     } else {
         for (; t - 1 >= bot; t -= 2) {
-            step(kStore, t, cur, rb2);
-            step(kStore, t - 1, rb2, cur);
-        }
-        if (t >= bot) step(kStore, t, cur, rb2);
+            step(kStore, kTested, t, cur, rb2);
+            step(kStore, kTested, t - 1, rb2, cur);
+        }
+        if (t >= bot) step(kStore, kTested, t, cur, rb2);
     }
     if constexpr (!SPARSE) {
         if (wave == 1 && bsc.valid) bsc.flush(bscale, lane, (uint64_t)bot);
@@ -3384,9 +3431,9 @@
     u32x2 ccd = lean_pair_bytes(sh, 1, wave);
     auto step = [&](uint32_t t, const double (&ba)[R], double (&bc)[R]) __attribute__((always_inline)) {
         const uint32_t n = t - first;
-        const double* rq = sh.rec[((n + 1u) / PG_LEAN_BLOCK) & 1u][(n + 1u) % PG_LEAN_BLOCK];
+        LAS const double* rq = (LAS const double*)lean_image(sh, n + 1u);
         const double rc0 = rq[0], rc1 = rq[1], rc2 = rq[2];
-        const unsigned long long nbits = (unsigned long long)__double_as_longlong(sh.rec[((n + 2u) / PG_LEAN_BLOCK) & 1u][(n + 2u) % PG_LEAN_BLOCK][7]);
+        const unsigned long long nbits = (unsigned long long)__double_as_longlong(((LAS const double*)lean_image(sh, n + 2u))[7]);
         const u32x2 ncd = lean_pair_bytes(sh, n + 2u, wave);
         if (((n + 4u) % PG_LEAN_BLOCK) == 0u) {
             const uint32_t blk = (n + 4u) / PG_LEAN_BLOCK;
@@ -3541,9 +3588,9 @@
         if (wave == 0) bsc.put(lane, (uint64_t)t, m);
         const double k0 = ldexp(kc0, -es), k1 = ldexp(kc1, -es), k2 = ldexp(kc2, -es), kap = ldexp(kck, -es);
         lds_barrier();
-        const double* rq = sh.rec[((n + 1u) / PG_LEAN_BLOCK) & 1u][(n + 1u) % PG_LEAN_BLOCK];
+        LAS const double* rq = (LAS const double*)lean_image(sh, n + 1u);
         const double nc0 = rq[0], nc1 = rq[1], nc2 = rq[2], nck = rq[3];
-        const unsigned long long nbits = (unsigned long long)__double_as_longlong(sh.rec[((n + 2u) / PG_LEAN_BLOCK) & 1u][(n + 2u) % PG_LEAN_BLOCK][7]);
+        const unsigned long long nbits = (unsigned long long)__double_as_longlong(((LAS const double*)lean_image(sh, n + 2u))[7]);
         const u32x2 ncd = lean_pair_bytes(sh, n + 2u, wave);
         if (t < t0) lean2_flush_partials<R>(sh2, (uint32_t)(t + 1) & 1u, part, (size_t)(t + 1), wave, lane, pbits);
         const double Cj = lean_colsum<R>(sh, (uint32_t)t & 1u, lane);
diff --git a/pangenie_amd/csrc/pg_shim.cpp b/pangenie_amd/csrc/pg_shim.cpp
--- a/pangenie_amd/csrc/pg_shim.cpp
+++ b/pangenie_amd/csrc/pg_shim.cpp
@@ -1743,6 +1743,16 @@
     if (out) { out[0] = r[0]; out[1] = r[1]; }
     return 1;
 }
+extern "C" int pg_lean_ring_schedule(uint32_t n_columns, uint32_t chunk_cols, uint32_t piece_chunks, uint32_t role, uint32_t form, uint32_t arg, uint32_t out[6]) {
+    if (role > 1u || form > 2u || chunk_cols == 0u || chunk_cols % PG_LEAN_SPARSE != 0u) return -1;
+    if (form == 1u && (piece_chunks == 0u || piece_chunks > 0xFFFFu || arg > 0xFFFFu || (unsigned long long)piece_chunks * chunk_cols > 0xFFFFFFFFull)) return -1;
+    uint32_t r[3];
+    const uint32_t chunk = form == 0u ? 0u : (form == 1u ? (piece_chunks << 16 | arg) : arg);
+    if (!pg_lean_ring_launch(n_columns, role, form == 2u ? 3u : 1u, chunk_cols, chunk, r)) return 0;
+    if (out) { out[0] = r[0]; out[1] = r[1]; out[2] = r[2]; out[3] = pg_lean_ring_first(r[2]); out[4] = PG_LEAN_RING_PARK; out[5] = PG_LEAN_RING_EXPAND; }
+    return 1;
+}
+extern "C" uint32_t pg_lean_ring_image_offset(uint32_t record) { return pg_lean_ring_image(record); }
 extern "C" int pg_prep_parts(uint32_t n_columns, uint32_t chunk_cols, uint32_t piece_chunks, uint32_t n_pieces, uint32_t early,
                              const uint32_t* col_variant, uint32_t n_variants, uint32_t out_cols[2], uint32_t out_vars[2]) {
     if (chunk_cols == 0u || chunk_cols % PG_LEAN_SPARSE != 0u || piece_chunks == 0u || (unsigned long long)piece_chunks * chunk_cols > 0xFFFFFFFFull) return -1;
```
